# jdeschut/tunempc

Hardware: AMD Instinct MI355X
Metric: stage-Hessian convexifications/sec at (nx+nu)=32, p=64 (higher is better)
Workload: dtype f64

## Files before the change

### include/tunempc_hip.h

```cpp
#ifndef TUNEMPC_HIP_H
#define TUNEMPC_HIP_H

#include <stdint.h>

#ifdef __cplusplus
extern "C" {
#endif

#define TMPC_OK 0
#define TMPC_E_ARG (-1)
#define TMPC_E_UNSUPPORTED (-2)
#define TMPC_E_NOMEM (-3)
#define TMPC_E_HIP (-4)
#define TMPC_E_NODEVICE (-5)
#define TMPC_E_NOCONV (-6)

#define TMPC_STATUS_OPTIMAL 0
#define TMPC_STATUS_FEASIBLE 1
#define TMPC_STATUS_INFEASIBLE 2

#define TMPC_FLAG_NO_MFMA 1
#define TMPC_FLAG_PROFILE 2
#define TMPC_FLAG_FAST_EXIT 4

#define TMPC_INFO_STRIDE 16

typedef struct tmpc_handle tmpc_handle;

int tmpc_device_count(void);

uint64_t tmpc_workspace_bytes(int chunk, int p, int nx, int mb);

int tmpc_create(tmpc_handle** out, int chunk, int p, int nx, int mb);
#define TMPC_MAX_ROWS 31
#define TMPC_ARROW_LD 32
uint64_t tmpc_workspace_bytes_eq(int chunk, int p, int nx, int mb, int ng);
int tmpc_create_eq(tmpc_handle** out, int chunk, int p, int nx, int mb, int ng);
uint64_t tmpc_workspace_bytes_con(int chunk, int p, int nx, int mb, int ng, int nc);
int tmpc_create_con(tmpc_handle** out, int chunk, int p, int nx, int mb, int ng, int nc);
int tmpc_destroy(tmpc_handle* h);
int tmpc_get_chunk(tmpc_handle* h);

int tmpc_set_options(tmpc_handle* h, double tol, double center_tol, int max_iter, int center_iter, int flags);

#define TMPC_TUNE_CHORD_STEP 1
#define TMPC_TUNE_SMALL_BLOCKS 2
#define TMPC_TUNE_EIG_PRETEST 3
#define TMPC_TUNE_FUSE_FWD 4
#define TMPC_TUNE_GRAPH 5
#define TMPC_TUNE_PERSISTENT 7
#define TMPC_TUNE_LOWP_SWITCH 8
#define TMPC_LOWP_SWITCH_DEFAULT 1e-5
#define TMPC_TUNE_LOWP_TRSM 9
int tmpc_set_tuning(tmpc_handle* h, int key, double value);
int tmpc_create_ex(tmpc_handle** out, int chunk, int p, int nx, int mb, int ng, int nc, int step3, int lanes);

int tmpc_set_tight(tmpc_handle* h, int enable, double tight_tol);

int tmpc_convexify_batch_host(tmpc_handle* h, int nb, const double* A, const double* B, const double* H,
                              double* Hc, double* dHc, double* P, double* alpha, double* beta, double* kappa,
                              int32_t* status, int32_t* iters, double* info);
int tmpc_convexify_batch_device(tmpc_handle* h, int nb, const double* dA, const double* dB, const double* dH,
                                double* dHc_out, double* ddHc_out, double* dP_out, double* d_alpha, double* d_beta,
                                double* d_kappa, int32_t* d_status, int32_t* d_iters, double* d_info, void* stream);

int tmpc_convexify_eq_batch_host(tmpc_handle* h, int nb, const double* A, const double* B, const double* H, const double* G,
                                 double* Hc, double* dHc, double* P, double* Fg, double* alpha, double* beta, double* kappa,
                                 int32_t* status, int32_t* iters, double* info);

int tmpc_convexify_step2_batch_host(tmpc_handle* h, int nb, const double* A, const double* B, const double* H, const double* J,
                                    const int32_t* ncnt, double rho, double* Hc, double* dHc, double* P, double* FgF, double* alpha,
                                    double* beta, double* kappa, int32_t* status, int32_t* iters, double* info);

uint64_t tmpc_workspace_bytes_step3(int chunk, int p, int nx, int mb);
int tmpc_create_step3(tmpc_handle** out, int chunk, int p, int nx, int mb);
int tmpc_convexify_step3_batch_host(tmpc_handle* h, int nb, const double* A, const double* B, const double* H, double rho,
                                    double* Hc, double* dHc, double* P, double* T, double* alpha, double* beta, double* kappa,
                                    int32_t* status, int32_t* iters, double* info);

uint64_t tmpc_workspace_bytes_step3_con(int chunk, int p, int nx, int mb, int ng, int nc);
int tmpc_create_step3_con(tmpc_handle** out, int chunk, int p, int nx, int mb, int ng, int nc);
int tmpc_convexify_step3_con_batch_host(tmpc_handle* h, int nb, const double* A, const double* B, const double* H, const double* J,
                                        const int32_t* ncnt, double rho, double* Hc, double* dHc, double* P, double* FgF, double* T,
                                        double* alpha, double* beta, double* kappa, int32_t* status, int32_t* iters, double* info);
int tmpc_convexify_step3_batch_device(tmpc_handle* h, int nb, const double* dA, const double* dB, const double* dH, double rho, double* Hc, double* dHc,
                                      double* P, double* T, double* alpha, double* beta, double* kappa, int32_t* status, int32_t* iters, double* info, void* stream);
int tmpc_convexify_step3_con_batch_device(tmpc_handle* h, int nb, const double* dA, const double* dB, const double* dH, const double* dJ, const int32_t* d_ncnt,
                                          double rho, double* Hc, double* dHc, double* P, double* FgF, double* T, double* alpha, double* beta, double* kappa,
                                          int32_t* status, int32_t* iters, double* info, void* stream);

int tmpc_convexify_con_batch_device(tmpc_handle* h, int nb, const double* dA, const double* dB, const double* dH, const double* dJ,
                                    const int32_t* d_ncnt, double rho, double* dHc_out, double* ddHc_out, double* dP_out, double* dFgF,
                                    double* d_alpha, double* d_beta, double* d_kappa, int32_t* d_status, int32_t* d_iters,
                                    double* d_info, void* stream);

int tmpc_supplement_batch_host(tmpc_handle* h, int nb, const double* A, const double* B, const double* P, double* dHc);
int tmpc_supplement_terms_batch_host(tmpc_handle* h, int nb, const double* A, const double* B, const double* P, int nr,
                                     const double* J, const double* wts, const double* T, double* dHc);

int tmpc_pack_sensitivities_host(tmpc_handle* h, int nb, int nh, const double* C, const double* mu, const double* Hbig, double thr, int ncmax,
                                 double* C_As, int32_t* ncnt, int32_t* idx, double* q, double* Hst);

int tmpc_tracking_reference_host(tmpc_handle* h, int nstage, const double* Hc, const double* q, const double* wref,
                                 double ts, double* W, double* yref, int32_t* info);

int tmpc_eig_scan_host(tmpc_handle* h, int nb, const double* H, double* out);

int tmpc_eig_clip_host(int nb, int n, const double* A, double tol, double* out, double* evals, double* reg, int32_t* sweeps);

#define TMPC_LQR_NMAX 64
int tmpc_periodic_lqr_batch_host(int nb, int p, int nx, int mb, const double* A, const double* B, const double* H, const double* Pi0, double tol,
                                 int max_sweeps, double* K, double* Pi, double* Phi, double* info);
int tmpc_periodic_lqr_batch_device(int nb, int p, int nx, int mb, const double* A, const double* B, const double* H, const double* Pi0, double tol,
                                   int max_sweeps, double* K, double* Pi, double* Phi, double* info);

int tmpc_periodic_lqr_rows_batch_host(int nb, int p, int nx, int mb, int nr, int ng, const double* A, const double* B, const double* H, const double* J,
                                      const int32_t* ncnt, const double* Pi0, double tol, int max_sweeps, double* K, double* Pi, double* Phi, double* Lam,
                                      double* info);
int tmpc_periodic_lqr_rows_batch_device(int nb, int p, int nx, int mb, int nr, int ng, const double* A, const double* B, const double* H, const double* J,
                                        const int32_t* ncnt, const double* Pi0, double tol, int max_sweeps, double* K, double* Pi, double* Phi, double* Lam,
                                        double* info);

#define TMPC_LQR_CTG_INFO 12
int tmpc_periodic_lqr_ctg_batch_host(int nb, int p, int nx, int mb, int nr, int ng, const double* A, const double* B, const double* H, const double* J,
                                     const int32_t* ncnt, const double* Pi0, double tol, double rank_tol, int max_sweeps, double* K, double* Pi, double* Phi,
                                     double* Hn, int32_t* cnt, double* info);
int tmpc_periodic_lqr_ctg_batch_device(int nb, int p, int nx, int mb, int nr, int ng, const double* A, const double* B, const double* H, const double* J,
                                       const int32_t* ncnt, const double* Pi0, double tol, double rank_tol, int max_sweeps, double* K, double* Pi, double* Phi,
                                       double* Hn, int32_t* cnt, double* info);

int tmpc_horizon_lqr_batch_host(int nb, int p, int nx, int mb, int nr, int ng, int N, int nph, const int32_t* phases, int terminal, const double* A,
                                const double* B, const double* H, const double* J, const int32_t* ncnt, const double* Pf, double rank_tol, double* K0,
                                double* Pi0, double* Hn0, int32_t* cnt0, double* Kall, int32_t* cntall, double* info);
int tmpc_horizon_lqr_batch_device(int nb, int p, int nx, int mb, int nr, int ng, int N, int nph, const int32_t* phases, int terminal, const double* A,
                                  const double* B, const double* H, const double* J, const int32_t* ncnt, const double* Pf, double rank_tol, double* K0,
                                  double* Pi0, double* Hn0, int32_t* cnt0, double* Kall, int32_t* cntall, double* info);
// ... 67 lines not shown
```

### include/tunempc_hip_debug.h

```cpp
#ifndef TUNEMPC_HIP_DEBUG_H
#define TUNEMPC_HIP_DEBUG_H

#include "tunempc_hip.h"

#ifdef __cplusplus
extern "C" {
#endif

#define TMPC_DEBUG_FLAG_STOP_ASSEMBLED 8
#define TMPC_DEBUG_FLAG_NO_LIFT 16
#define TMPC_DEBUG_FLAG_NO_DMA 32
#define TMPC_DEBUG_FLAG_GENERIC_STAGE 64

int tmpc_debug_gemm_nt(tmpc_handle* h, double* C, const double* A, const double* B, int M, int N, int K, int mode, int lower);

int tmpc_debug_block_solve(tmpc_handle* h, int p, int d, const double* D, const double* Ccpl, const double* rhs, double* x, int32_t* nshift);

#define TMPC_DEBUG_FACTOR_PASS1 1
#define TMPC_DEBUG_FACTOR_FUSE_FWD1 2
#define TMPC_DEBUG_FACTOR_LOWP_TRSM 4
#define TMPC_DEBUG_FACTOR_DD 8
typedef struct {
  const double *D, *Ccpl, *Dlo, *Clo, *rhs;
  const int32_t *list, *lowp;
  double *oD, *oO, *oF, *oDdiag, *oX;
  float* oO32;
  double *oDl, *oOl, *oFl, *oXl;
  int32_t *nshift, *dims, *orient;
} tmpc_debug_factor_io;
int tmpc_debug_block_factor(tmpc_handle* h, int nb, int p, int d, int count, int mode, const tmpc_debug_factor_io* io);

int tmpc_debug_cr_schedule(int p, int32_t* out, int cap);

int tmpc_debug_get_multipliers(tmpc_handle* h, int nb, int nr, double* phi, double* z, double* dphi, double* dz);

int tmpc_debug_get_array(tmpc_handle* h, int which, uint64_t offset, uint64_t count, double* out);

int tmpc_debug_min_eig(tmpc_handle* h, int nmat, int n, const double* W, double* out);
int tmpc_debug_min_eig_lane(tmpc_handle* h, int nmat, int n, const double* W, double* out);

int tmpc_debug_factor_bench(tmpc_handle* h, int nb, int p, int d, int reps, double* ms_out2);

#ifdef __cplusplus
}
#endif
#endif
```

### tunempc_amd/_lib.py

```python
import ctypes as C
import os

import numpy as np

_HERE = os.path.dirname(os.path.abspath(__file__))
_LIB = None

INFO_STRIDE = 16
FLAG_NO_MFMA = 1
FLAG_PROFILE = 2
FLAG_FAST_EXIT = 4
STATUS_NAMES = {0: 'Optimal', 1: 'Feasible', 2: 'Infeasible'}

ARROW_LD = 32
EXPORTS = [
    'tmpc_device_count', 'tmpc_workspace_bytes', 'tmpc_workspace_bytes_eq', 'tmpc_workspace_bytes_con',
    'tmpc_create', 'tmpc_create_eq', 'tmpc_create_con', 'tmpc_destroy', 'tmpc_get_chunk', 'tmpc_set_options', 'tmpc_set_tight', 'tmpc_set_tuning', 'tmpc_create_ex',
    'tmpc_convexify_batch_host', 'tmpc_convexify_batch_device', 'tmpc_convexify_eq_batch_host', 'tmpc_convexify_step2_batch_host',
    'tmpc_convexify_con_batch_device', 'tmpc_workspace_bytes_step3', 'tmpc_create_step3', 'tmpc_convexify_step3_batch_host', 'tmpc_workspace_bytes_step3_con', 'tmpc_create_step3_con', 'tmpc_convexify_step3_con_batch_host', 'tmpc_convexify_step3_batch_device', 'tmpc_convexify_step3_con_batch_device', 'tmpc_supplement_batch_host', 'tmpc_supplement_terms_batch_host',
    'tmpc_tracking_reference_host', 'tmpc_eig_scan_host', 'tmpc_get_profile', 'tmpc_get_trace', 'tmpc_get_dual_host', 'tmpc_get_dual_con_host', 'tmpc_pack_sensitivities_host', 'tmpc_eig_clip_host',
    'tmpc_periodic_lqr_batch_host', 'tmpc_periodic_lqr_batch_device', 'tmpc_periodic_lqr_rows_batch_host', 'tmpc_periodic_lqr_rows_batch_device',
    'tmpc_periodic_lqr_ctg_batch_host', 'tmpc_periodic_lqr_ctg_batch_device', 'tmpc_horizon_lqr_batch_host', 'tmpc_horizon_lqr_batch_device',
    'tmpc_closed_loop_batch_host', 'tmpc_closed_loop_batch_device', 'tmpc_mpc_qp_batch_host', 'tmpc_mpc_qp_batch_device',
    'tmpc_mpc_qp_soft_batch_host', 'tmpc_mpc_qp_soft_batch_device', 'tmpc_mpc_qp_eq_batch_host', 'tmpc_mpc_qp_eq_batch_device',
    'tmpc_mpc_qp_aff_batch_host', 'tmpc_mpc_qp_aff_batch_device',
    'tmpc_last_error', 'tmpc_version',
]
DEBUG_EXPORTS = [
    'tmpc_debug_gemm_nt', 'tmpc_debug_block_solve', 'tmpc_debug_cr_schedule', 'tmpc_debug_get_multipliers', 'tmpc_debug_get_array',
    'tmpc_debug_min_eig', 'tmpc_debug_min_eig_lane', 'tmpc_debug_factor_bench', 'tmpc_debug_block_factor',
]
FLAG_DEBUG_NO_DMA = 32
FACTOR_PASS1, FACTOR_FUSE_FWD1, FACTOR_LOWP_TRSM, FACTOR_DD = 1, 2, 4, 8


class _FactorIO(C.Structure):
    _fields_ = ([(n, C.POINTER(C.c_double)) for n in ('D', 'Ccpl', 'Dlo', 'Clo', 'rhs')] + [(n, C.POINTER(C.c_int32)) for n in ('list', 'lowp')] +
                [(n, C.POINTER(C.c_double)) for n in ('oD', 'oO', 'oF', 'oDdiag', 'oX')] + [('oO32', C.POINTER(C.c_float))] +
                [(n, C.POINTER(C.c_double)) for n in ('oDl', 'oOl', 'oFl', 'oXl')] + [(n, C.POINTER(C.c_int32)) for n in ('nshift', 'dims', 'orient')])


def library_path():
    return os.environ.get('TMPC_LIB') or os.path.join(_HERE, 'lib', 'libtunempc_hip.so')


def load_library():
    global _LIB
    if _LIB is not None:
        return _LIB
    path = library_path()
    if not os.path.exists(path):
        raise RuntimeError(
            f"tunempc_amd: HIP library not built ({path}); run `python -c 'import __graft_entry__ as g; g.build()'`"
            " -- there is no CPU fallback for the convexify hot path")
    lib = C.CDLL(path)
    dp = C.POINTER(C.c_double)
    ip = C.POINTER(C.c_int32)
    vp = C.c_void_p
    lib.tmpc_device_count.restype = C.c_int
    lib.tmpc_workspace_bytes.restype = C.c_uint64
    lib.tmpc_workspace_bytes.argtypes = [C.c_int] * 4
    lib.tmpc_workspace_bytes_eq.restype = C.c_uint64
    lib.tmpc_workspace_bytes_eq.argtypes = [C.c_int] * 5
    lib.tmpc_create_eq.restype = C.c_int
    lib.tmpc_create_eq.argtypes = [C.POINTER(vp), C.c_int, C.c_int, C.c_int, C.c_int, C.c_int]
    lib.tmpc_convexify_eq_batch_host.restype = C.c_int
    lib.tmpc_convexify_eq_batch_host.argtypes = [vp, C.c_int, dp, dp, dp, dp, dp, dp, dp, dp, dp, dp, dp, ip, ip, dp]
    lib.tmpc_workspace_bytes_con.restype = C.c_uint64
    lib.tmpc_workspace_bytes_con.argtypes = [C.c_int] * 6
    lib.tmpc_create_con.restype = C.c_int
    lib.tmpc_create_con.argtypes = [C.POINTER(vp), C.c_int, C.c_int, C.c_int, C.c_int, C.c_int, C.c_int]
    lib.tmpc_convexify_step2_batch_host.restype = C.c_int
    lib.tmpc_convexify_step2_batch_host.argtypes = [vp, C.c_int, dp, dp, dp, dp, ip, C.c_double, dp, dp, dp, dp, dp, dp, dp, ip, ip, dp]
    lib.tmpc_workspace_bytes_step3.restype = C.c_uint64
    lib.tmpc_workspace_bytes_step3.argtypes = [C.c_int] * 4
    lib.tmpc_create_step3.restype = C.c_int
    lib.tmpc_create_step3.argtypes = [C.POINTER(vp), C.c_int, C.c_int, C.c_int, C.c_int]
    lib.tmpc_workspace_bytes_step3_con.restype = C.c_uint64
    lib.tmpc_workspace_bytes_step3_con.argtypes = [C.c_int] * 6
    lib.tmpc_create_step3_con.restype = C.c_int
    lib.tmpc_create_step3_con.argtypes = [C.POINTER(vp), C.c_int, C.c_int, C.c_int, C.c_int, C.c_int, C.c_int]
    lib.tmpc_convexify_step3_con_batch_host.restype = C.c_int
    lib.tmpc_convexify_step3_con_batch_host.argtypes = [vp, C.c_int, dp, dp, dp, dp, ip, C.c_double, dp, dp, dp, dp, dp, dp, dp, dp, ip, ip, dp]
    lib.tmpc_convexify_step3_batch_host.restype = C.c_int
    lib.tmpc_convexify_step3_batch_host.argtypes = [vp, C.c_int, dp, dp, dp, C.c_double, dp, dp, dp, dp, dp, dp, dp, ip, ip, dp]
    lib.tmpc_debug_get_multipliers.restype = C.c_int
    lib.tmpc_debug_get_multipliers.argtypes = [vp, C.c_int, C.c_int, dp, dp, dp, dp]
    lib.tmpc_debug_get_array.restype = C.c_int
    lib.tmpc_debug_get_array.argtypes = [vp, C.c_int, C.c_uint64, C.c_uint64, dp]
    lib.tmpc_convexify_con_batch_device.restype = C.c_int
    lib.tmpc_convexify_con_batch_device.argtypes = [vp, C.c_int, vp, vp, vp, vp, vp, C.c_double] + [vp] * 10 + [vp]
    lib.tmpc_convexify_step3_batch_device.restype = C.c_int
    lib.tmpc_convexify_step3_batch_device.argtypes = [vp, C.c_int, vp, vp, vp, C.c_double] + [vp] * 10 + [vp]
    lib.tmpc_convexify_step3_con_batch_device.restype = C.c_int
    lib.tmpc_convexify_step3_con_batch_device.argtypes = [vp, C.c_int, vp, vp, vp, vp, vp, C.c_double] + [vp] * 11 + [vp]
    lib.tmpc_get_dual_con_host.restype = C.c_int
    lib.tmpc_get_dual_con_host.argtypes = [vp, C.c_int, dp, dp, dp, dp]
    lib.tmpc_create.restype = C.c_int
    lib.tmpc_create.argtypes = [C.POINTER(vp), C.c_int, C.c_int, C.c_int, C.c_int]
    lib.tmpc_destroy.restype = C.c_int
    lib.tmpc_destroy.argtypes = [vp]
    lib.tmpc_get_chunk.restype = C.c_int
    lib.tmpc_get_chunk.argtypes = [vp]
    lib.tmpc_set_tuning.restype = C.c_int
    lib.tmpc_set_tuning.argtypes = [vp, C.c_int, C.c_double]
    lib.tmpc_create_ex.restype = C.c_int
    lib.tmpc_create_ex.argtypes = [C.POINTER(C.c_void_p)] + [C.c_int] * 8
    lib.tmpc_set_tight.restype = C.c_int
    lib.tmpc_set_tight.argtypes = [vp, C.c_int, C.c_double]
    lib.tmpc_set_options.restype = C.c_int
    lib.tmpc_set_options.argtypes = [vp, C.c_double, C.c_double, C.c_int, C.c_int, C.c_int]
    lib.tmpc_convexify_batch_host.restype = C.c_int
    lib.tmpc_convexify_batch_host.argtypes = [vp, C.c_int, dp, dp, dp, dp, dp, dp, dp, dp, dp, ip, ip, dp]
    lib.tmpc_convexify_batch_device.restype = C.c_int
    lib.tmpc_convexify_batch_device.argtypes = [vp, C.c_int] + [vp] * 12 + [vp]
    lib.tmpc_supplement_batch_host.restype = C.c_int
    lib.tmpc_supplement_batch_host.argtypes = [vp, C.c_int, dp, dp, dp, dp]
    lib.tmpc_eig_scan_host.restype = C.c_int
    lib.tmpc_eig_scan_host.argtypes = [vp, C.c_int, dp, dp]
    lib.tmpc_eig_clip_host.restype = C.c_int
    lib.tmpc_eig_clip_host.argtypes = [C.c_int, C.c_int, dp, C.c_double, dp, dp, dp, C.POINTER(C.c_int32)]
    lib.tmpc_periodic_lqr_batch_host.restype = C.c_int
    lib.tmpc_periodic_lqr_batch_host.argtypes = [C.c_int] * 4 + [dp] * 4 + [C.c_double, C.c_int] + [dp] * 4
    lib.tmpc_periodic_lqr_batch_device.restype = C.c_int
    lib.tmpc_periodic_lqr_batch_device.argtypes = [C.c_int] * 4 + [vp] * 4 + [C.c_double, C.c_int] + [vp] * 4
    lib.tmpc_periodic_lqr_rows_batch_host.restype = C.c_int
    lib.tmpc_periodic_lqr_rows_batch_host.argtypes = [C.c_int] * 6 + [dp] * 4 + [ip, dp, C.c_double, C.c_int] + [dp] * 5
    lib.tmpc_periodic_lqr_rows_batch_device.restype = C.c_int
    lib.tmpc_periodic_lqr_rows_batch_device.argtypes = [C.c_int] * 6 + [vp] * 6 + [C.c_double, C.c_int] + [vp] * 5
    lib.tmpc_periodic_lqr_ctg_batch_host.restype = C.c_int
    lib.tmpc_periodic_lqr_ctg_batch_host.argtypes = [C.c_int] * 6 + [dp] * 4 + [ip, dp, C.c_double, C.c_double, C.c_int] + [dp] * 4 + [ip, dp]
    lib.tmpc_periodic_lqr_ctg_batch_device.restype = C.c_int
    lib.tmpc_periodic_lqr_ctg_batch_device.argtypes = [C.c_int] * 6 + [vp] * 6 + [C.c_double, C.c_double, C.c_int] + [vp] * 6
    lib.tmpc_horizon_lqr_batch_host.restype = C.c_int
    lib.tmpc_horizon_lqr_batch_host.argtypes = [C.c_int] * 8 + [ip, C.c_int] + [dp] * 4 + [ip, dp, C.c_double] + [dp] * 3 + [ip, dp, ip, dp]
    lib.tmpc_horizon_lqr_batch_device.restype = C.c_int
    lib.tmpc_horizon_lqr_batch_device.argtypes = [C.c_int] * 8 + [ip, C.c_int] + [vp] * 6 + [C.c_double] + [vp] * 7
    lib.tmpc_closed_loop_batch_host.restype = C.c_int
    lib.tmpc_closed_loop_batch_host.argtypes = [C.c_int] * 9 + [dp] * 7 + [ip] + [dp] * 10
    lib.tmpc_closed_loop_batch_device.restype = C.c_int
    lib.tmpc_closed_loop_batch_device.argtypes = [C.c_int] * 9 + [vp] * 18
    lib.tmpc_mpc_qp_batch_host.restype = C.c_int
    lib.tmpc_mpc_qp_batch_host.argtypes = [C.c_int] * 9 + [dp] * 6 + [ip, dp, dp, C.c_double, C.c_int] + [dp] * 5 + [ip, ip] + [dp] * 4
    lib.tmpc_mpc_qp_batch_device.restype = C.c_int
    lib.tmpc_mpc_qp_batch_device.argtypes = [C.c_int] * 9 + [vp] * 9 + [C.c_double, C.c_int] + [vp] * 11
    lib.tmpc_mpc_qp_soft_batch_host.restype = C.c_int
    lib.tmpc_mpc_qp_soft_batch_host.argtypes = lib.tmpc_mpc_qp_batch_host.argtypes + [dp, dp, ip]
    lib.tmpc_mpc_qp_soft_batch_device.restype = C.c_int
    lib.tmpc_mpc_qp_soft_batch_device.argtypes = lib.tmpc_mpc_qp_batch_device.argtypes + [vp] * 3
    lib.tmpc_mpc_qp_eq_batch_host.restype = C.c_int
    lib.tmpc_mpc_qp_eq_batch_host.argtypes = lib.tmpc_mpc_qp_soft_batch_host.argtypes + [C.c_int, dp, dp, ip, C.c_int, dp, dp, dp, dp]
    lib.tmpc_mpc_qp_eq_batch_device.restype = C.c_int
    lib.tmpc_mpc_qp_eq_batch_device.argtypes = lib.tmpc_mpc_qp_soft_batch_device.argtypes + [C.c_int, vp, vp, vp, C.c_int, vp, vp, vp, vp]
    lib.tmpc_mpc_qp_aff_batch_host.restype = C.c_int
    lib.tmpc_mpc_qp_aff_batch_host.argtypes = lib.tmpc_mpc_qp_eq_batch_host.argtypes + [dp] * 7
    lib.tmpc_mpc_qp_aff_batch_device.restype = C.c_int
    lib.tmpc_mpc_qp_aff_batch_device.argtypes = lib.tmpc_mpc_qp_eq_batch_device.argtypes + [vp] * 7
    lib.tmpc_get_profile.restype = C.c_int
    lib.tmpc_get_profile.argtypes = [vp, dp]
    lib.tmpc_get_trace.restype = C.c_int
    lib.tmpc_get_trace.argtypes = [vp, C.c_int, dp]
    lib.tmpc_pack_sensitivities_host.restype = C.c_int
    lib.tmpc_pack_sensitivities_host.argtypes = [vp, C.c_int, C.c_int, dp, dp, dp, C.c_double, C.c_int, dp, ip, ip, dp, dp]
    lib.tmpc_get_dual_host.restype = C.c_int
    lib.tmpc_get_dual_host.argtypes = [vp, C.c_int, dp, dp, dp]
    lib.tmpc_debug_gemm_nt.restype = C.c_int
    lib.tmpc_debug_gemm_nt.argtypes = [vp, dp, dp, dp, C.c_int, C.c_int, C.c_int, C.c_int, C.c_int]
    lib.tmpc_debug_block_solve.restype = C.c_int
    lib.tmpc_debug_block_solve.argtypes = [vp, C.c_int, C.c_int, dp, dp, dp, dp, ip]
    lib.tmpc_supplement_terms_batch_host.restype = C.c_int
    lib.tmpc_supplement_terms_batch_host.argtypes = [vp, C.c_int, dp, dp, dp, C.c_int, dp, dp, dp, dp]
    lib.tmpc_tracking_reference_host.restype = C.c_int
    lib.tmpc_tracking_reference_host.argtypes = [vp, C.c_int, dp, dp, dp, C.c_double, dp, dp, ip]
    lib.tmpc_debug_cr_schedule.restype = C.c_int
    lib.tmpc_debug_cr_schedule.argtypes = [C.c_int, ip, C.c_int]
    lib.tmpc_debug_block_factor.restype = C.c_int
    lib.tmpc_debug_block_factor.argtypes = [vp, C.c_int, C.c_int, C.c_int, C.c_int, C.c_int, C.POINTER(_FactorIO)]
    lib.tmpc_debug_factor_bench.restype = C.c_int
    lib.tmpc_debug_factor_bench.argtypes = [vp, C.c_int, C.c_int, C.c_int, C.c_int, dp]
    lib.tmpc_debug_min_eig.restype = C.c_int
    lib.tmpc_debug_min_eig.argtypes = [vp, C.c_int, C.c_int, dp, dp]
    lib.tmpc_debug_min_eig_lane.restype = C.c_int
    lib.tmpc_debug_min_eig_lane.argtypes = [vp, C.c_int, C.c_int, dp, dp]
    lib.tmpc_last_error.restype = C.c_char_p
    lib.tmpc_version.restype = C.c_char_p
    _LIB = lib
    return lib


def _dptr(a):
    return a.ctypes.data_as(C.POINTER(C.c_double)) if a is not None else None


def _iptr(a):
    return a.ctypes.data_as(C.POINTER(C.c_int32)) if a is not None else None


class EigNotConverged(RuntimeError):
    """tmpc_eig_clip_host returned TMPC_E_NOCONV: the Jacobi sweeps were exhausted; `.partial` holds the last iterate."""


E_NOCONV = -6
E_UNSUPPORTED = -2
LQR_INFO_STRIDE = 8
LQR_CTG_INFO_STRIDE = 12
CLOSED_LOOP_INFO_STRIDE = 4
MPC_QP_INFO_STRIDE = 8


def _check(lib, rc, what):
    if rc != 0:
        raise RuntimeError(f"tunempc_amd: {what} failed with code {rc}: {lib.tmpc_last_error().decode()}")


class HipConvexifier:

    def __init__(self, p, nx, mb, chunk=0, tol=None, center_tol=None, max_iter=None, center_iter=None, flags=0, ng=0, nc=0, step3=False, lanes=0):
        self.lib = load_library()
        if self.lib.tmpc_device_count() < 1:
            raise RuntimeError("tunempc_amd: no HIP device visible; the convexify hot path has no CPU fallback")
        self.p, self.nx, self.mb, self.n = int(p), int(nx), int(mb), int(nx) + int(mb)
        self._h = C.c_void_p()
        self.ng = int(ng)
        self.nc = int(nc)
        self.step3 = bool(step3)
        if lanes:
            _check(self.lib, self.lib.tmpc_create_ex(C.byref(self._h), int(chunk), self.p, self.nx, self.mb, self.ng, self.nc, int(self.step3), int(lanes)), 'tmpc_create_ex')
        elif self.step3 and (self.ng or self.nc):
            _check(self.lib, self.lib.tmpc_create_step3_con(C.byref(self._h), int(chunk), self.p, self.nx, self.mb, self.ng, self.nc), 'tmpc_create_step3_con')
        elif self.step3:
            _check(self.lib, self.lib.tmpc_create_step3(C.byref(self._h), int(chunk), self.p, self.nx, self.mb), 'tmpc_create_step3')
        else:
            _check(self.lib, self.lib.tmpc_create_con(C.byref(self._h), int(chunk), self.p, self.nx, self.mb, self.ng, self.nc), 'tmpc_create_con')
        self.chunk = int(self.lib.tmpc_get_chunk(self._h))
        self.flags = int(flags)
        self.set_options(tol, center_tol, max_iter, center_iter, flags)

    def set_options(self, tol=None, center_tol=None, max_iter=None, center_iter=None, flags=None):
        if flags is not None:
            self.flags = int(flags)
        _check(self.lib, self.lib.tmpc_set_options(self._h, float(tol or 0.0), float(center_tol or 0.0),
                                                   int(max_iter or 0), int(center_iter or 0), self.flags), 'tmpc_set_options')

    def set_tuning(self, chord_step=None, small_blocks=None, eig_pretest=None, fuse_fwd=None, graph=None, persistent=None, lowp_switch=None, lowp_trsm=None):
        for key, v in ((1, chord_step), (2, small_blocks), (3, eig_pretest), (4, fuse_fwd), (5, graph), (7, persistent), (8, lowp_switch), (9, lowp_trsm)):
            if v is not None:
                _check(self.lib, self.lib.tmpc_set_tuning(self._h, key, float(v)), 'tmpc_set_tuning')

    def set_tight(self, enable=True, tight_tol=None):
        _check(self.lib, self.lib.tmpc_set_tight(self._h, 1 if enable else 0, float(tight_tol or 0.0)), 'tmpc_set_tight')

    def close(self):
        if getattr(self, '_h', None) is not None and self._h.value:
            self.lib.tmpc_destroy(self._h)
            self._h = C.c_void_p()

    def __del__(self):
        try:
            self.close()
        except Exception:
            pass

    def convexify_batch(self, A, B, H):
        A = np.ascontiguousarray(A, dtype=np.float64); B = np.ascontiguousarray(B, dtype=np.float64)
        H = np.ascontiguousarray(H, dtype=np.float64)
        nb = A.shape[0]
        assert A.shape == (nb, self.p, self.nx, self.nx), A.shape
        assert B.shape == (nb, self.p, self.nx, self.mb), B.shape
        assert H.shape == (nb, self.p, self.n, self.n), H.shape
        out = dict(Hc=np.empty_like(H), dHc=np.empty_like(H), P=np.empty_like(A), alpha=np.empty(nb), beta=np.empty(nb),
                   kappa=np.empty(nb), status=np.empty(nb, np.int32), iters=np.empty(nb, np.int32),
                   info=np.empty((nb, INFO_STRIDE)))
        if nb == 0:
            return out
        rc = self.lib.tmpc_convexify_batch_host(self._h, nb, _dptr(A), _dptr(B), _dptr(H), _dptr(out['Hc']), _dptr(out['dHc']),
                                                _dptr(out['P']), _dptr(out['alpha']), _dptr(out['beta']), _dptr(out['kappa']),
                                                _iptr(out['status']), _iptr(out['iters']), _dptr(out['info']))
        _check(self.lib, rc, 'tmpc_convexify_batch_host')
        return out

    def convexify_eq_batch(self, A, B, H, G):
        A = np.ascontiguousarray(A, dtype=np.float64); B = np.ascontiguousarray(B, dtype=np.float64)
        H = np.ascontiguousarray(H, dtype=np.float64); G = np.ascontiguousarray(G, dtype=np.float64)
        nb = A.shape[0]
        assert A.shape == (nb, self.p, self.nx, self.nx), A.shape
        assert B.shape == (nb, self.p, self.nx, self.mb), B.shape
        assert H.shape == (nb, self.p, self.n, self.n), H.shape
        assert self.ng > 0 and G.shape == (nb, self.p, self.ng, self.n), (G.shape, self.ng)
        out = dict(Hc=np.empty_like(H), dHc=np.empty_like(H), P=np.empty_like(A), Fg=np.empty((nb, self.p, self.ng)),
                   alpha=np.empty(nb), beta=np.empty(nb), kappa=np.empty(nb), status=np.empty(nb, np.int32),
                   iters=np.empty(nb, np.int32), info=np.empty((nb, INFO_STRIDE)))
        if nb == 0:
            return out
        rc = self.lib.tmpc_convexify_eq_batch_host(self._h, nb, _dptr(A), _dptr(B), _dptr(H), _dptr(G), _dptr(out['Hc']),
                                                   _dptr(out['dHc']), _dptr(out['P']), _dptr(out['Fg']), _dptr(out['alpha']),
                                                   _dptr(out['beta']), _dptr(out['kappa']), _iptr(out['status']),
                                                   _iptr(out['iters']), _dptr(out['info']))
        _check(self.lib, rc, 'tmpc_convexify_eq_batch_host')
        return out

    def debug_array(self, which, offset, count):
        out = np.empty(int(count))
        _check(self.lib, self.lib.tmpc_debug_get_array(self._h, int(which), int(offset), int(count), _dptr(out)), 'tmpc_debug_get_array')
        return out

    def debug_multipliers(self, nb, nr):
        out = [np.empty((nb, self.p, nr)) for _ in range(4)]
        _check(self.lib, self.lib.tmpc_debug_get_multipliers(self._h, nb, nr, *[_dptr(o) for o in out]), 'tmpc_debug_get_multipliers')
        return dict(phi=out[0], z=out[1], dphi=out[2], dz=out[3])

    def convexify_step2_batch(self, A, B, H, J, ncnt, rho):
        A = np.ascontiguousarray(A, dtype=np.float64); B = np.ascontiguousarray(B, dtype=np.float64)
        H = np.ascontiguousarray(H, dtype=np.float64); J = np.ascontiguousarray(J, dtype=np.float64)
        ncnt = np.ascontiguousarray(ncnt, dtype=np.int32)
        nb = A.shape[0]
        nr = self.ng + self.nc
        assert A.shape == (nb, self.p, self.nx, self.nx), A.shape
        assert B.shape == (nb, self.p, self.nx, self.mb), B.shape
        assert H.shape == (nb, self.p, self.n, self.n), H.shape
        assert self.nc > 0 and J.shape == (nb, self.p, nr, self.n) and ncnt.shape == (nb, self.p), (J.shape, ncnt.shape, nr)
        out = dict(Hc=np.empty_like(H), dHc=np.empty_like(H), P=np.empty_like(A), FgF=np.empty((nb, self.p, nr)),
                   alpha=np.empty(nb), beta=np.empty(nb), kappa=np.empty(nb), status=np.empty(nb, np.int32),
                   iters=np.empty(nb, np.int32), info=np.empty((nb, INFO_STRIDE)))
        if nb == 0:
            return out
        rc = self.lib.tmpc_convexify_step2_batch_host(self._h, nb, _dptr(A), _dptr(B), _dptr(H), _dptr(J), _iptr(ncnt), float(rho),
                                                      _dptr(out['Hc']), _dptr(out['dHc']), _dptr(out['P']), _dptr(out['FgF']),
                                                      _dptr(out['alpha']), _dptr(out['beta']), _dptr(out['kappa']),
# ... 141 lines not shown

    def profile(self):
        out = np.zeros(16)
        _check(self.lib, self.lib.tmpc_get_profile(self._h, _dptr(out)), 'tmpc_get_profile')
        keys = ['pre_ms', 'schur_ms', 'factor_ms', 'pass1_ms', 'pass2_ms', 'factor_launches', 'total_ms', 'ipm_iters',
                'problem_factorisations', 'potrf_ms', 'trsm_ms', 'update_ms', 'lanes', 'lowp_factorisations', 'update_f32_ms', 'persistent_problems']
        return dict(zip(keys, out.tolist()))

    def pack_sensitivities(self, C=None, mu=None, Hbig=None, thr=1e-15, ncmax=None, nb=None):
        out = {}
        p, n = self.p, self.n
        if C is not None:
            C = np.ascontiguousarray(C, dtype=np.float64); mu = np.ascontiguousarray(mu, dtype=np.float64)
            nb, nh = C.shape[0], C.shape[2]
            assert C.shape == (nb, p, nh, n) and mu.shape == (nb, p, nh), (C.shape, mu.shape)
            ncmax = int(ncmax or nh)
            out.update(C_As=np.empty((nb, p, ncmax, n)), nc=np.empty((nb, p), np.int32), idx=np.empty((nb, p, nh), np.int32))
        else:
            nh, ncmax = 0, 0
            nb = int(nb if nb is not None else Hbig.shape[0])
        out['q'] = np.empty((nb, p, n))
        if Hbig is not None:
            Hbig = np.ascontiguousarray(Hbig, dtype=np.float64)
            assert Hbig.shape == (nb, p * n, p * n), Hbig.shape
            out['H'] = np.empty((nb, p, n, n))
        _check(self.lib, self.lib.tmpc_pack_sensitivities_host(self._h, nb, nh, _dptr(C), _dptr(mu), _dptr(Hbig), float(thr), ncmax,
                                                               _dptr(out.get('C_As')), _iptr(out.get('nc')), _iptr(out.get('idx')),
                                                               _dptr(out['q']), _dptr(out.get('H'))), 'tmpc_pack_sensitivities_host')
        if 'nc' in out and (out['nc'] > ncmax).any():
            raise ValueError('pack_sensitivities: a stage has %d active rows, more than ncmax = %d' % (int(out['nc'].max()), ncmax))
        return out

    def dual(self, nb):
        X1 = np.empty((nb, self.p, self.n, self.n)); X2 = np.empty_like(X1); sc = np.empty((nb, 4))
        _check(self.lib, self.lib.tmpc_get_dual_host(self._h, int(nb), _dptr(X1), _dptr(X2), _dptr(sc)), 'tmpc_get_dual_host')
        return dict(X1=X1, X2=X2, x0=sc[:, 0].copy(), tau=sc[:, 1].copy(), alpha=sc[:, 2].copy(), mu_target=sc[:, 3].copy())

    def dual_con(self, nb, arrows=False):
        nr = self.ng + self.nc
        phi = np.zeros((nb, self.p, nr)); z = np.zeros_like(phi)
        aX = np.zeros((nb, self.p, 2, ARROW_LD, ARROW_LD)) if arrows else None; at = np.zeros((nb, self.p, 2)) if arrows else None
        _check(self.lib, self.lib.tmpc_get_dual_con_host(self._h, int(nb), _dptr(phi), _dptr(z), _dptr(aX) if arrows else None, _dptr(at) if arrows else None), 'tmpc_get_dual_con_host')
        out = dict(phi=phi, z=z)
        if arrows:
            out.update(aX=aX, at=at)
        return out

    def trace(self, nb):
        out = np.zeros((nb, 80, 10))
        _check(self.lib, self.lib.tmpc_get_trace(self._h, nb, _dptr(out)), 'tmpc_get_trace')
        return out

    def debug_gemm_nt(self, Cm, A, B, mode=0, lower=False):
        Cm = np.ascontiguousarray(Cm, dtype=np.float64).copy(); A = np.ascontiguousarray(A, dtype=np.float64)
        B = np.ascontiguousarray(B, dtype=np.float64)
        M, N = Cm.shape; K = A.shape[1]
        _check(self.lib, self.lib.tmpc_debug_gemm_nt(self._h, _dptr(Cm), _dptr(A), _dptr(B), M, N, K, int(mode), int(lower)), 'tmpc_debug_gemm_nt')
        return Cm

    def debug_min_eig(self, W, lane=False):
        W = np.ascontiguousarray(W, dtype=np.float64)
        nmat, n, _ = W.shape
        out = np.empty(nmat)
        fn = self.lib.tmpc_debug_min_eig_lane if lane else self.lib.tmpc_debug_min_eig
        _check(self.lib, fn(self._h, nmat, n, _dptr(W), _dptr(out)), 'tmpc_debug_min_eig')
        return out

    def tracking_reference(self, Hc, q, wref, ts):
        Hc = np.ascontiguousarray(Hc, dtype=np.float64); q = np.ascontiguousarray(q, dtype=np.float64)
        wref = np.ascontiguousarray(wref, dtype=np.float64)
        n = self.nx + self.mb
        if Hc.shape[-2:] != (n, n) or q.shape != Hc.shape[:-1] or wref.shape != q.shape:
            raise ValueError('tracking_reference: expected Hc [..., %d, %d] and q, wref [..., %d]' % (n, n, n))
        ns = int(np.prod(Hc.shape[:-2], dtype=np.int64))
        W = np.empty_like(Hc); yref = np.empty_like(q); info = np.zeros(Hc.shape[:-2], dtype=np.int32)
        _check(self.lib, self.lib.tmpc_tracking_reference_host(self._h, ns, _dptr(Hc), _dptr(q), _dptr(wref), float(ts), _dptr(W), _dptr(yref),
                                                              info.ctypes.data_as(C.POINTER(C.c_int32))), 'tmpc_tracking_reference_host')
        return W, yref, info

    def debug_factor_bench(self, nb, p, d, reps=3):
        out = np.zeros(2)
        _check(self.lib, self.lib.tmpc_debug_factor_bench(self._h, nb, p, d, reps, _dptr(out)), 'tmpc_debug_factor_bench')
        return out

    def debug_block_solve(self, D, Ccpl, rhs):
        D = np.ascontiguousarray(D, dtype=np.float64); Ccpl = np.ascontiguousarray(Ccpl, dtype=np.float64)
        rhs = np.ascontiguousarray(rhs, dtype=np.float64)
        p, d, _ = D.shape
        x = np.empty((p, d)); ns = np.zeros(1, np.int32)
        _check(self.lib, self.lib.tmpc_debug_block_solve(self._h, p, d, _dptr(D), _dptr(Ccpl), _dptr(rhs), _dptr(x), _iptr(ns)), 'tmpc_debug_block_solve')
        return x, int(ns[0])

    def debug_block_factor(self, D, Ccpl, rhs, plist=None, lowp=None, pass1=False, fuse_fwd1=False, lowp_trsm=False, dd=False, Dlo=None, Clo=None):
        f64 = lambda a: None if a is None else np.ascontiguousarray(a, dtype=np.float64)
        D, Ccpl, rhs, Dlo, Clo = f64(D), f64(Ccpl), f64(rhs), f64(Dlo), f64(Clo)
        nb, p, d, _ = D.shape
        nc = 3 if pass1 else 1
        if Ccpl.shape != D.shape or rhs.shape != ((nb, p, d, 3) if pass1 else (nb, p, d)):
            raise ValueError('debug_block_factor: D, Ccpl [nb, p, d, d] and rhs [nb, p, d] (pass 2) / [nb, p, d, 3] (pass 1) expected')
        plist = np.ascontiguousarray(np.arange(nb) if plist is None else plist, dtype=np.int32)
        lowp = None if lowp is None else np.ascontiguousarray(lowp, dtype=np.int32)
        if lowp is not None and lowp.shape != (nb,):
            raise ValueError('debug_block_factor: lowp [nb] expected')
        mode = (FACTOR_PASS1 if pass1 else 0) | (FACTOR_FUSE_FWD1 if fuse_fwd1 else 0) | (FACTOR_LOWP_TRSM if lowp_trsm else 0) | (FACTOR_DD if dd else 0)
        dp = (d + 15) // 16 * 16; ld32 = (dp + 31) // 32 * 32
        has32 = bool(lowp_trsm or (lowp is not None and lowp.any()))
        raw = dict(D=np.empty((nb, p, dp, dp)), O=np.empty((nb, p, dp, dp)), F=np.empty((nb, p, dp, dp)), Ddiag=np.empty((nb, p, dp)), X=np.empty((nb, p, dp, nc)),
                   O32=np.empty((nb, 2 * p, dp, ld32), np.float32) if has32 else None)
        if dd:
            raw.update(Dl=np.empty((nb, p, dp, dp)), Ol=np.empty((nb, p, dp, dp)), Fl=np.empty((nb, p, dp, dp)), Xl=np.empty((nb, p, dp, nc)))
        nshift = np.zeros(nb, np.int32); dims = np.zeros(4, np.int32); orient = np.zeros(p, np.int32)
        io = _FactorIO(D=_dptr(D), Ccpl=_dptr(Ccpl), Dlo=_dptr(Dlo), Clo=_dptr(Clo), rhs=_dptr(rhs), list=_iptr(plist), lowp=_iptr(lowp),
                       oD=_dptr(raw['D']), oO=_dptr(raw['O']), oF=_dptr(raw['F']), oDdiag=_dptr(raw['Ddiag']), oX=_dptr(raw['X']),
                       oO32=raw['O32'].ctypes.data_as(C.POINTER(C.c_float)) if has32 else None,
                       oDl=_dptr(raw.get('Dl')), oOl=_dptr(raw.get('Ol')), oFl=_dptr(raw.get('Fl')), oXl=_dptr(raw.get('Xl')),
                       nshift=_iptr(nshift), dims=_iptr(dims), orient=_iptr(orient))
        _check(self.lib, self.lib.tmpc_debug_block_factor(self._h, nb, p, d, len(plist), mode, C.byref(io)), 'tmpc_debug_block_factor')
        assert (int(dims[0]), int(dims[1]), int(dims[2]), bool(dims[3])) == (dp, ld32, nc, has32), dims
        raw.update(dp=dp, ld32=ld32)
        cut = lambda a: None if a is None else a[:, :, :d, :d].copy()
        vec = lambda a: None if a is None else (a[:, :, :d, :].copy() if pass1 else a[:, :, :d, 0].copy())
        out = dict(raw=raw, orient=orient, nshift=nshift, D=cut(raw['D']), L=np.tril(cut(raw['D'])), O=cut(raw['O']), F=cut(raw['F']), O32=cut(raw['O32']),
                   Ddiag=raw['Ddiag'][:, :, :d].copy(), x=vec(raw['X']))
        if dd:
            out.update(Dl=cut(raw['Dl']), Ll=np.tril(cut(raw['Dl'])), Ol=cut(raw['Ol']), Fl=cut(raw['Fl']), xl=vec(raw['Xl']))
        return out


def eig_clip(A, tol):
    lib = load_library()
    A = np.ascontiguousarray(A, dtype=np.float64)
    single = A.ndim == 2
    A3 = A[None] if single else A
    nb, n, n2 = A3.shape
    if n != n2:
        raise ValueError('square matrices expected')
    out = np.empty_like(A3); ev = np.empty((nb, n)); reg = np.empty(nb); sw = np.zeros(nb, dtype=np.int32)
    rc = lib.tmpc_eig_clip_host(nb, n, _dptr(A3), float(tol), _dptr(out), _dptr(ev), _dptr(reg), _iptr(sw))
    if rc == E_NOCONV:
        err = EigNotConverged(f"tunempc_amd: tmpc_eig_clip_host did not converge: {lib.tmpc_last_error().decode()}")
        err.partial = dict(out=out, evals=ev, reg=reg, sweeps=sw)
        raise err
    _check(lib, rc, 'tmpc_eig_clip_host')
    if single:
        return dict(out=out[0], evals=ev[0], reg=float(reg[0]), sweeps=int(sw[0]))
    return dict(out=out, evals=ev, reg=reg, sweeps=sw)


def _check_lqr(lib, rc, what):
    if rc == E_UNSUPPORTED:
        raise NotImplementedError(lib.tmpc_last_error().decode())
    _check(lib, rc, what)


def periodic_lqr_batch_host(A, B, H, Pi0, tol, max_sweeps):
    lib = load_library()
    nb, p, nx, mb = B.shape
    K = np.empty((nb, p, mb, nx)); Pi = np.empty((nb, p, nx, nx)); Phi = np.empty((nb, nx, nx)); info = np.zeros((nb, LQR_INFO_STRIDE))
    rc = lib.tmpc_periodic_lqr_batch_host(nb, p, nx, mb, _dptr(A), _dptr(B), _dptr(H), _dptr(Pi0), float(tol), int(max_sweeps),
                                          _dptr(K), _dptr(Pi), _dptr(Phi), _dptr(info))
    _check_lqr(lib, rc, 'tmpc_periodic_lqr_batch_host')
    return K, Pi, Phi, info


def periodic_lqr_batch_device(A, B, H, Pi0, tol, max_sweeps):
    import torch
# ... 335 lines not shown
```

### tunempc_amd/csrc/tmpc_api.hip

```cpp
#include <hip/hip_runtime.h>
#include <stdio.h>
#include <stdlib.h>
#include <new>
#include <string.h>
#include <algorithm>
#include <chrono>
#include <thread>
#include <mutex>
#include <condition_variable>
#include <functional>
#include <unistd.h>
#include <vector>

#include <string>
#include <unordered_map>

#include "../../include/tunempc_hip.h"
#include "../../include/tunempc_hip_debug.h"
#include "tmpc_common.h"
#include "tmpc_small.h"
#include "tmpc_stage.h"
#include "tmpc_schur.h"
#include "tmpc_factor.h"
#include "tmpc_cr.h"
// ... 27 lines not shown
struct DevBuf {
  void* p = nullptr;
  ~DevBuf() { if (p) hipFree(p); }
  hipError_t alloc(size_t bytes) { return hipMalloc(&p, bytes ? bytes : 8); }
  template <typename T> T* as() const { return (T*)p; }
};

constexpr int MAXL = 4;
struct LaneWorker {
  std::thread th;
  std::mutex m;
  std::condition_variable cv;
  std::function<void()> job;
  bool has_job = false, done = true, stop = false;
  pid_t pid = 0;
  void start() {
    pid = getpid();
    th = std::thread([this] {
      std::unique_lock<std::mutex> lk(m);
      for (;;) {
        cv.wait(lk, [&] { return has_job || stop; });
        if (stop) return;
        std::function<void()> j = std::move(job);
        has_job = false;
        lk.unlock();
        j();
        lk.lock();
        done = true;
        cv.notify_all();
      }
    });
  }
  void submit(std::function<void()> j) {
    { std::lock_guard<std::mutex> lk(m); job = std::move(j); has_job = true; done = false; }
    cv.notify_all();
  }
  void wait() { std::unique_lock<std::mutex> lk(m); cv.wait(lk, [&] { return done; }); }
  void shutdown() {
    { std::lock_guard<std::mutex> lk(m); stop = true; }
    cv.notify_all();
    if (th.joinable()) th.join();
  }
  static void retire(LaneWorker*& wk) {
    if (!wk) return;
    if (wk->pid == getpid()) { wk->shutdown(); delete wk; }
    wk = nullptr;
  }
};

struct Lane {
  LaneWorker* worker;
  WS ws;
  double *dA, *dB, *dH;
  double* dG;
  int32_t* dncnt;
  double* d_info;
  double* d_abk;
  void* big_scr;
  int32_t* d_si;
  hipStream_t st;
  hipEvent_t ev[8];
  double prof[16];
  std::vector<hipEvent_t> kev;
  int last_nb;
  int o32_dp;
  std::unordered_map<std::string, hipGraphExec_t>* graphs;
  char err[512];
};

struct tmpc_handle {
  Dims dm;
  int chunk;
  int nlanes;
  Opts opt;
  int flags;
  Lane lane[MAXL];
  void* slab;
  size_t slab_bytes;
  hipEvent_t ev_in;
  int device;
  CrSched sched;
  int* d_sched;
  int rs, mt;
  int tune_small, tune_pretest, tune_fuse, tune_graph, tune_persist, tune_lowp_trsm;
  void* dd_slab;
  size_t dd_bytes;
  int tight;
  double tight_tol;
};

static int cr_upload(const CrSched& sc, int** out) {
  std::vector<int> flat(sc.elim);
  flat.insert(flat.end(), sc.upd.begin(), sc.upd.end());
  flat.insert(flat.end(), sc.orient.begin(), sc.orient.end());
  *out = nullptr;
  if (hipMalloc(out, flat.size() * sizeof(int)) != hipSuccess) return TMPC_E_NOMEM;
  if (hipMemcpy(*out, flat.data(), flat.size() * sizeof(int), hipMemcpyHostToDevice) != hipSuccess) { hipFree(*out); *out = nullptr; return TMPC_E_HIP; }
  return TMPC_OK;
}
static CrDev cr_dev(const CrSched& sc, const int* d_sched, const int* alist) {
  CrDev c; c.elim = d_sched; c.upd = d_sched + sc.elim.size(); c.orient = d_sched + sc.elim.size() + sc.upd.size(); c.alist = alist;
  return c;
}

static bool dims_ok(int p, int nx, int mb) { return p >= 1 && nx >= 1 && mb >= 0 && nx + mb <= NB && nx + mb >= 1; }

static Dims make_dims(int chunk, int p, int nx, int mb, int ng = 0, int nc = 0, int step3 = 0) {
  Dims d;
  d.ng = ng; d.nr = ng + nc; d.constr = 0;
  d.nT = step3 ? (nx + mb) * (nx + mb + 1) / 2 : 0;
  d.nz = d.nr + (nc > 0 ? 2 : 0);
  d.B = chunk; d.p = p; d.nx = nx; d.mb = mb; d.n = nx + mb;
  d.d = nx * (nx + 1) / 2;
  d.dp = (d.d + d.nz + (d.nT ? d.nT + 1 : 0) + 15) / 16 * 16;
  d.nt = (d.dp + TB - 1) / TB;
  d.flags = 0;
  return d;
}

static bool schur_in_lds(const Dims& dm) { return (size_t)sch_rec<0>() * dm.nx * dm.nx * sizeof(double) + (size_t)dm.d * sizeof(unsigned) + 64 <= 158 * 1024; }
struct Carver {
  char* base; size_t off;
  template <typename T> T* take(size_t count) {
    off = (off + 255) & ~(size_t)255;
    T* p = base ? (T*)(base + off) : nullptr;
    off += count * sizeof(T);
    return p;
  }
};

static size_t carve(WS& w, const Dims& dm, char* base, Lane* h) {
  Carver c{base, 0};
  const size_t BP = (size_t)dm.B * dm.p, nn = (size_t)dm.n * dm.n, nxx = (size_t)dm.nx * dm.nx;
  const size_t bs = (size_t)dm.dp * dm.dp;
  w.Hb = c.take<double>(BP * nn); w.V = c.take<double>(BP * dm.nx * dm.n);
  w.P = c.take<double>(BP * nxx);
  w.X1 = c.take<double>(BP * nn); w.X2 = c.take<double>(BP * nn); w.S1 = c.take<double>(BP * nn); w.S2 = c.take<double>(BP * nn);
  w.S1i = c.take<double>(BP * nn); w.S2i = c.take<double>(BP * nn); w.L1i = c.take<double>(BP * nn); w.L2i = c.take<double>(BP * nn);
  w.LX1i = c.take<double>(BP * nn); w.LX2i = c.take<double>(BP * nn);
  w.Rd1 = c.take<double>(BP * nn); w.Rd2 = c.take<double>(BP * nn); w.T1 = c.take<double>(BP * nn); w.T2 = c.take<double>(BP * nn);
  w.dS1 = c.take<double>(BP * nn); w.dS2 = c.take<double>(BP * nn); w.dX1 = c.take<double>(BP * nn); w.dX2 = c.take<double>(BP * nn);
  w.c1 = c.take<double>(BP * nn); w.c2 = c.take<double>(BP * nn);
  w.dP = c.take<double>(BP * nxx);
  w.Wm = c.take<double>(BP * 4 * nn); w.eigmin = c.take<double>(BP * 4);
  w.KF = c.take<double>(BP * 12 * nxx); w.adjV = c.take<double>(BP * NADJ * nxx); w.adjE = c.take<double>(BP * NADJ * nxx);
  w.part = c.take<double>(BP * NPART); w.prob = c.take<double>((size_t)dm.B * PS); w.iprob = c.take<int>((size_t)dm.B * IS);
  w.D = c.take<double>(BP * bs); w.O = c.take<double>(BP * bs); w.F = c.take<double>(BP * bs);
  w.O32 = (dm.nT == 0 && dm.n <= NMAX && dm.dp > 64 && dm.nt <= TRR_NT) ? c.take<float>(2 * BP * (size_t)dm.dp * ((dm.dp + 31) & ~31)) : nullptr;
  w.Linv = c.take<double>(BP * dm.nt * TB * TB); w.Ddiag = c.take<double>(BP * dm.dp);
  w.W3 = c.take<double>(BP * dm.dp * 3); w.U = c.take<double>(BP * dm.dp * 2); w.TU = c.take<double>(BP * dm.dp * 2);
  w.Z = c.take<double>(BP * dm.dp);
  w.active = c.take<int>(64);
  w.alist = c.take<int>((size_t)dm.B);
  w.flist = c.take<int>((size_t)dm.B);
  w.cr_orient = nullptr;
  w.trace = c.take<double>((size_t)dm.B * TRACE_LEN * TRACE_W);
  w.Hc = c.take<double>(BP * nn); w.dHc = c.take<double>(BP * nn); w.Pout = c.take<double>(BP * nxx);
  w.bscr = (dm.n > NMAX) ? c.take<double>(BP * BIG_SCR * nn) : nullptr;
  w.sscr = schur_in_lds(dm) ? nullptr : c.take<double>(BP * 10 * nxx);
  w.Dl = w.Ol = w.Fl = w.Linvl = w.KFl = w.adjVl = w.adjEl = w.W3l = w.Zl = w.Pprev = w.Pdef = w.phidef = w.Zdd = w.TUl = w.atdef = w.ddscr = nullptr; w.plist = w.pnext = nullptr;
  w.G = nullptr; w.ncnt = nullptr; w.rho = 0.0;
  w.phi = w.zph = w.dphi = w.dzph = w.corrp = w.pvec = w.psm = w.prs = w.Fg = nullptr;
  w.at = w.adt = w.aX = w.adX = w.acor = w.aSi = w.aLi = w.aLXi = w.asum = nullptr;
  if (dm.nr > 0) {
    const size_t g = dm.nr, z = dm.nz;
    w.phi = c.take<double>(BP * g); w.zph = c.take<double>(BP * g); w.dphi = c.take<double>(BP * g); w.dzph = c.take<double>(BP * g);
    w.corrp = c.take<double>(BP * g); w.Fg = c.take<double>(BP * g);
// ... 208 lines not shown
  const double* A0 = A + (size_t)m0 * K; const double* B0 = B + (size_t)n0 * K;
  if (k1 > 0 && k1 < K && 2 * k1 == K)
    wg_tile_dma<UPD_DMA_DEPTH>(C + (size_t)m0 * N + n0, N, A0, B0, A0 + k1, B0 + k1, K, Mt, Nt, k1, mode, (lower && tm == tn) ? 0 : GM_NOTRI, blockIdx.x, lds);
  else
    wg_tile_dma<UPD_DMA_DEPTH>(C + (size_t)m0 * N + n0, N, A0, B0, nullptr, nullptr, K, Mt, Nt, K, mode, (lower && tm == tn) ? 0 : GM_NOTRI, blockIdx.x, lds);
}
static size_t slots_bytes(int s) { return (size_t)s * MS * sizeof(double); }
template <int PART> static size_t schur_lds(const Dims& dm) {
  if (!schur_in_lds(dm)) return (size_t)dm.d * sizeof(unsigned) + 64;
 return (size_t)sch_rec<PART>() * dm.nx * dm.nx * sizeof(double) + (size_t)dm.d * sizeof(unsigned) + 64; }
static size_t factor_lds() { return (size_t)FACT_LDS_DOUBLES * sizeof(double); }
static size_t solve_lds(const Dims& dm) { return (size_t)cr_solve_lds_doubles(dm.dp) * sizeof(double); }

static int set_lds_attrs(int device) {
  static bool done[64] = {false};
  if (device >= 0 && device < 64 && done[device]) return TMPC_OK;
  const int big = 160 * 1024;
  HIPCHK(hipFuncSetAttribute((const void*)k_stage_pre<256>, hipFuncAttributeMaxDynamicSharedMemorySize, big - 4096));
  HIPCHK(hipFuncSetAttribute((const void*)k_stage_rhs<256>, hipFuncAttributeMaxDynamicSharedMemorySize, big - 4096));
  HIPCHK(hipFuncSetAttribute((const void*)k_stage_dir<256>, hipFuncAttributeMaxDynamicSharedMemorySize, big - 4096));
  HIPCHK(hipFuncSetAttribute((const void*)k_final_stage, hipFuncAttributeMaxDynamicSharedMemorySize, big));
  HIPCHK(hipFuncSetAttribute((const void*)k_schur<0>, hipFuncAttributeMaxDynamicSharedMemorySize, big));
  HIPCHK(hipFuncSetAttribute((const void*)k_schur<1>, hipFuncAttributeMaxDynamicSharedMemorySize, big));
  HIPCHK(hipFuncSetAttribute((const void*)k_cr_potrf<true>, hipFuncAttributeMaxDynamicSharedMemorySize, big));
  HIPCHK(hipFuncSetAttribute((const void*)k_cr_potrf<false>, hipFuncAttributeMaxDynamicSharedMemorySize, big));
  HIPCHK(hipFuncSetAttribute((const void*)k_cr_trsm<true, 2>, hipFuncAttributeMaxDynamicSharedMemorySize, big));
  HIPCHK(hipFuncSetAttribute((const void*)k_cr_trsm<false, 2>, hipFuncAttributeMaxDynamicSharedMemorySize, big));
  HIPCHK(hipFuncSetAttribute((const void*)k_cr_trsm_dma, hipFuncAttributeMaxDynamicSharedMemorySize, big));
  HIPCHK(hipFuncSetAttribute((const void*)k_cr_trsm_dma_f32, hipFuncAttributeMaxDynamicSharedMemorySize, big));
  HIPCHK(hipFuncSetAttribute((const void*)k_cr_potrf_dma, hipFuncAttributeMaxDynamicSharedMemorySize, big));
  HIPCHK(hipFuncSetAttribute((const void*)k_cr_update<true, 2>, hipFuncAttributeMaxDynamicSharedMemorySize, big));
  HIPCHK(hipFuncSetAttribute((const void*)k_cr_update<false, 2>, hipFuncAttributeMaxDynamicSharedMemorySize, big));
  HIPCHK(hipFuncSetAttribute((const void*)k_cr_fwd_diag, hipFuncAttributeMaxDynamicSharedMemorySize, big));
  HIPCHK(hipFuncSetAttribute((const void*)k_cr_fwd_off, hipFuncAttributeMaxDynamicSharedMemorySize, big));
  HIPCHK(hipFuncSetAttribute((const void*)k_cr_bwd, hipFuncAttributeMaxDynamicSharedMemorySize, big));
  HIPCHK(hipFuncSetAttribute((const void*)k_cr_small_solve, hipFuncAttributeMaxDynamicSharedMemorySize, big));
  HIPCHK(hipFuncSetAttribute((const void*)k_cr_small_factor, hipFuncAttributeMaxDynamicSharedMemorySize, big));
  HIPCHK(hipFuncSetAttribute((const void*)k_ipm_small, hipFuncAttributeMaxDynamicSharedMemorySize, big));
  HIPCHK(hipFuncSetAttribute((const void*)k_debug_gemm<true>, hipFuncAttributeMaxDynamicSharedMemorySize, big));
  HIPCHK(hipFuncSetAttribute((const void*)k_debug_gemm<false>, hipFuncAttributeMaxDynamicSharedMemorySize, big));
  HIPCHK(hipFuncSetAttribute((const void*)k_supplement, hipFuncAttributeMaxDynamicSharedMemorySize, big));
  HIPCHK(hipFuncSetAttribute((const void*)k_phi_pre<false, false>, hipFuncAttributeMaxDynamicSharedMemorySize, big));
  HIPCHK(hipFuncSetAttribute((const void*)k_phi_pre<false, true>, hipFuncAttributeMaxDynamicSharedMemorySize, big));
  HIPCHK(hipFuncSetAttribute((const void*)k_phi_pre<true, false>, hipFuncAttributeMaxDynamicSharedMemorySize, big));
  HIPCHK(hipFuncSetAttribute((const void*)k_phi_pre<true, true>, hipFuncAttributeMaxDynamicSharedMemorySize, big));
  HIPCHK(hipFuncSetAttribute((const void*)k_phi_rhs<false>, hipFuncAttributeMaxDynamicSharedMemorySize, big));
  HIPCHK(hipFuncSetAttribute((const void*)k_phi_dir<false>, hipFuncAttributeMaxDynamicSharedMemorySize, big));
  HIPCHK(hipFuncSetAttribute((const void*)k_phi_rhs<true>, hipFuncAttributeMaxDynamicSharedMemorySize, big));
  HIPCHK(hipFuncSetAttribute((const void*)k_phi_dir<true>, hipFuncAttributeMaxDynamicSharedMemorySize, big));
  HIPCHK(hipFuncSetAttribute((const void*)k_t3_schur<false>, hipFuncAttributeMaxDynamicSharedMemorySize, big));
  HIPCHK(hipFuncSetAttribute((const void*)k_t3_schur<true>, hipFuncAttributeMaxDynamicSharedMemorySize, big));
  HIPCHK(hipFuncSetAttribute((const void*)k_dd_potrf, hipFuncAttributeMaxDynamicSharedMemorySize, big));
  HIPCHK(hipFuncSetAttribute((const void*)k_dd_aug_fill, hipFuncAttributeMaxDynamicSharedMemorySize, big));
  HIPCHK(hipFuncSetAttribute((const void*)k_dd_trsm, hipFuncAttributeMaxDynamicSharedMemorySize, big));
  HIPCHK(hipFuncSetAttribute((const void*)k_dd_update, hipFuncAttributeMaxDynamicSharedMemorySize, big));
  HIPCHK(hipFuncSetAttribute((const void*)k_dd_fwd_diag, hipFuncAttributeMaxDynamicSharedMemorySize, big));
  HIPCHK(hipFuncSetAttribute((const void*)k_dd_fwd_off, hipFuncAttributeMaxDynamicSharedMemorySize, big));
  HIPCHK(hipFuncSetAttribute((const void*)k_dd_bwd, hipFuncAttributeMaxDynamicSharedMemorySize, big));
  HIPCHK(hipFuncSetAttribute((const void*)k_dd_images, hipFuncAttributeMaxDynamicSharedMemorySize, big));
  HIPCHK(hipFuncSetAttribute((const void*)k_dd_schur<0>, hipFuncAttributeMaxDynamicSharedMemorySize, big));
  HIPCHK(hipFuncSetAttribute((const void*)k_dd_schur<1>, hipFuncAttributeMaxDynamicSharedMemorySize, big));
  HIPCHK(hipFuncSetAttribute((const void*)k_dd_schur<0, true>, hipFuncAttributeMaxDynamicSharedMemorySize, big));
  HIPCHK(hipFuncSetAttribute((const void*)k_dd_schur<1, true>, hipFuncAttributeMaxDynamicSharedMemorySize, big));
  HIPCHK(hipFuncSetAttribute((const void*)k_dd_polish_pre, hipFuncAttributeMaxDynamicSharedMemorySize, big - 4096));
  HIPCHK(hipFuncSetAttribute((const void*)k_polish_step, hipFuncAttributeMaxDynamicSharedMemorySize, big - 4096));
  if (device >= 0 && device < 64) done[device] = true;
  return TMPC_OK;
}

static unsigned cr_grid(long items) { return (unsigned)((items + 7) / 8 * 8); }
constexpr int DF_NO_SMALL = 2;
constexpr int DF_NO_DMA = 4;

static bool cr_small_levels(const Dims& dm, const CrSched& sc, CrLevs* out) {
  if ((dm.flags & DF_NO_SMALL) || dm.dp != 16 || (dm.flags & 1) || dm.p > CRS_PMAX || (int)sc.lev.size() > CRS_MAXLEV) return false;
  if (out) {
    out->n = (int)sc.lev.size();
    for (int l = 0; l < out->n; ++l) { out->v[4 * l] = sc.lev[l].eoff; out->v[4 * l + 1] = sc.lev[l].nelim; out->v[4 * l + 2] = sc.lev[l].uoff; out->v[4 * l + 3] = sc.lev[l].nupd; }
  }
  return true;
}

static void cr_factor(const WS& w, const Dims& dm, const CrSched& sc, const int* d_sched, const int* alist, int count, hipStream_t st,
                      int rs_opt, int mt_opt, std::vector<hipEvent_t>* kev = nullptr, int* nkev = nullptr, int fuse_fwd1 = 0, int nlowp = 0) {
  const CrDev cd = cr_dev(sc, d_sched, alist);
  int ke = 0;
  auto mark = [&](int cls) {
#ifdef TMPC_CYCLE_PROF
    { static int cls_ids[4] = {0, 1, 2, 3}; hipMemcpyToSymbolAsync(HIP_SYMBOL(tmpc::g_prof_cls), &cls_ids[cls + 1], sizeof(int), 0, hipMemcpyHostToDevice, st); }
#endif
    if (!kev) return;
    while ((int)kev->size() <= ke) { hipEvent_t e; if (hipEventCreate(&e) != hipSuccess) return; kev->push_back(e); }
    (void)cls;
    hipEventRecord((*kev)[ke++], st);
  };
  const bool mf = !(dm.flags & 1);
  if (sc.prep) hipLaunchKernelGGL(k_cr_prep, dim3(count), dim3(256), 0, st, w, dm, cd, sc.prep);
  {
    CrLevs lv;
    if (!fuse_fwd1 && cr_small_levels(dm, sc, &lv)) {
      mark(0);
      hipLaunchKernelGGL(k_cr_small_factor, dim3(count), dim3(CRS_NT), (size_t)crs_factor_lds_doubles() * sizeof(double), st, w, dm, cd, lv);
      mark(0);
      if (nkev) *nkev = ke;
      return;
    }
  }
  const int nt64 = (dm.dp + 63) / 64;
  for (const CrLevel& lv : sc.lev) {
    const bool use_dma = !(dm.flags & DF_NO_DMA), potrf_dma = use_dma;
    mark(0);
    if (mf && use_dma && potrf_dma && dm.nt <= TRR_NT)
      hipLaunchKernelGGL(k_cr_potrf_dma, dim3(cr_grid((long)count * lv.nelim)), dim3(256), (size_t)potrf_dma_lds_doubles() * sizeof(double), st, w, dm, cd, lv.eoff, lv.nelim, count);
    else if (mf) hipLaunchKernelGGL(k_cr_potrf<true>, dim3(cr_grid((long)count * lv.nelim)), dim3(256), factor_lds(), st, w, dm, cd, lv.eoff, lv.nelim, count);
    else hipLaunchKernelGGL(k_cr_potrf<false>, dim3(cr_grid((long)count * lv.nelim)), dim3(256), factor_lds(), st, w, dm, cd, lv.eoff, lv.nelim, count);
    mark(0);
    if (fuse_fwd1) hipLaunchKernelGGL(k_cr_fwd_diag, dim3(cr_grid((long)count * lv.nelim)), dim3(256), solve_lds(dm), st, w, dm, cd, lv.eoff, lv.nelim, count, 1);
    if (lv.nupd == 0) { mark(1); mark(1); mark(2); mark(2); mark(3); mark(3); continue; }
    const long work64 = (long)count * lv.nelim * 2 * nt64;
    const int rs = rs_opt > 0 ? rs_opt : (work64 >= 16384 ? 128 : 64);
    const int mt = mt_opt > 0 ? mt_opt : 64;
    const int nstrip = (dm.dp + rs - 1) / rs, nm = (dm.dp + mt - 1) / mt;
    const long it_trsm = (long)count * lv.nelim * 2 * nstrip;
    const long it_upd = (long)count * ((long)lv.nupd * (nm * (nm + 1) / 2) + (long)lv.nelim * nm * nm);
    mark(1);
    if (mf && use_dma && dm.nt <= TRR_NT) {
      const size_t trsm_lds = (size_t)trd_lds_doubles() * sizeof(double);
      const bool trsm32 = (dm.flags & DF_LOWP_TRSM) != 0;
      if (!trsm32 || nlowp < count)
        hipLaunchKernelGGL(k_cr_trsm_dma, dim3(cr_grid((long)count * lv.nelim * 2 * nt64)), dim3(256), trsm_lds, st, w, dm, cd, lv.eoff, lv.nelim, count);
      if (trsm32 && nlowp > 0)
        hipLaunchKernelGGL(k_cr_trsm_dma_f32, dim3(cr_grid((long)count * lv.nelim * 2 * nt64)), dim3(256), (size_t)trf_lds_doubles() * sizeof(double), st, w, dm, cd, lv.eoff, lv.nelim, count);
    }
    else if (mf) hipLaunchKernelGGL((k_cr_trsm<true, 2>), dim3(cr_grid(it_trsm)), dim3(256), factor_lds(), st, w, dm, cd, lv.eoff, lv.nelim, count, rs);
    else hipLaunchKernelGGL((k_cr_trsm<false, 2>), dim3(cr_grid(it_trsm)), dim3(256), factor_lds(), st, w, dm, cd, lv.eoff, lv.nelim, count, rs);
    mark(1); mark(2);
    if (mf && use_dma) {
      const int nm64 = (dm.dp + 63) / 64;
      const long it_dma = (long)count * ((long)lv.nupd * (nm64 * (nm64 + 1) / 2) + (long)lv.nelim * nm64 * nm64);
      if (nlowp < count)
        hipLaunchKernelGGL(k_cr_update_dma, dim3(cr_grid(it_dma)), dim3(256), (size_t)dma_lds_doubles<UPD_DMA_DEPTH>() * sizeof(double), st, w, dm, cd, lv.eoff, lv.nelim, lv.uoff, lv.nupd, count, fuse_fwd1);
      mark(2); mark(3);
      if (nlowp > 0)
        hipLaunchKernelGGL(k_cr_update_dma_f32, dim3(cr_grid(it_dma)), dim3(256), (size_t)UPD_DMA_DEPTH * DMA_SLAB * sizeof(double), st, w, dm, cd, lv.eoff, lv.nelim, lv.uoff, lv.nupd, count);
      mark(3);
    }
    else if (mf) { hipLaunchKernelGGL((k_cr_update<true, 2>), dim3(cr_grid(it_upd)), dim3(256), factor_lds(), st, w, dm, cd, lv.eoff, lv.nelim, lv.uoff, lv.nupd, count, mt); mark(2); mark(3); mark(3); }
    else { hipLaunchKernelGGL((k_cr_update<false, 2>), dim3(cr_grid(it_upd)), dim3(256), factor_lds(), st, w, dm, cd, lv.eoff, lv.nelim, lv.uoff, lv.nupd, count, mt); mark(2); mark(3); mark(3); }
    if (fuse_fwd1 && nlowp > 0 && mf && use_dma && lv.nupd)
      hipLaunchKernelGGL(k_cr_fwd_off, dim3(cr_grid((long)count * lv.nupd)), dim3(256), solve_lds(dm), st, w, dm, cd, lv.uoff, lv.nupd, count, 1, 1);
  }
  if (nkev) *nkev = ke;
}

static void cr_solve(const WS& w, const Dims& dm, const CrSched& sc, const int* d_sched, const int* alist, int count, hipStream_t st, int pass, bool skip_fwd = false) {
  const CrDev cd = cr_dev(sc, d_sched, alist);
  {
    CrLevs lv;
    if (!skip_fwd && cr_small_levels(dm, sc, &lv)) {
      hipLaunchKernelGGL(k_cr_small_solve, dim3(count), dim3(CRS_NT), (size_t)crs_solve_lds_doubles(dm.p) * sizeof(double), st, w, dm, cd, lv, pass);
      return;
    }
  }
  const size_t lds = solve_lds(dm);
  for (const CrLevel& lv : sc.lev) {
    if (skip_fwd) break;
    hipLaunchKernelGGL(k_cr_fwd_diag, dim3(cr_grid((long)count * lv.nelim)), dim3(256), lds, st, w, dm, cd, lv.eoff, lv.nelim, count, pass);
    if (lv.nupd) hipLaunchKernelGGL(k_cr_fwd_off, dim3(cr_grid((long)count * lv.nupd)), dim3(256), lds, st, w, dm, cd, lv.uoff, lv.nupd, count, pass, 0);
  }
  for (size_t l = sc.lev.size(); l-- > 0;) {
    const CrLevel& lv = sc.lev[l];
    hipLaunchKernelGGL(k_cr_bwd, dim3(cr_grid((long)count * lv.nelim)), dim3(256), lds, st, w, dm, cd, lv.eoff, lv.nelim, count, pass);
  }
}

static bool ddschur_in_lds(const Dims& dm) { return (size_t)2 * ddsch_mats<0>() * dm.nx * dm.nx * sizeof(double) + (size_t)dm.d * sizeof(unsigned) + 64 <= 158 * 1024; }
template <int PART> static size_t ddschur_lds(const Dims& dm) {
  if (!ddschur_in_lds(dm)) return (size_t)dm.d * sizeof(unsigned) + 64;
  return (size_t)2 * ddsch_mats<PART>() * dm.nx * dm.nx * sizeof(double) + (size_t)dm.d * sizeof(unsigned) + 64;
}
static void dd_schur_launch(const WS& w, const Dims& dm, int grid_stages, hipStream_t st) {
  if (ddschur_in_lds(dm)) {
    hipLaunchKernelGGL(k_dd_schur<0>, dim3(grid_stages), dim3(256), ddschur_lds<0>(dm), st, w, dm);
    hipLaunchKernelGGL(k_dd_schur<1>, dim3(grid_stages), dim3(256), ddschur_lds<1>(dm), st, w, dm);
  } else {
    hipLaunchKernelGGL((k_dd_schur<0, true>), dim3(grid_stages), dim3(256), ddschur_lds<0>(dm), st, w, dm);
    hipLaunchKernelGGL((k_dd_schur<1, true>), dim3(grid_stages), dim3(256), ddschur_lds<1>(dm), st, w, dm);
  }
}
static size_t dd_stage_lds(const Dims& dm, int slots) { return dm.n > NMAX ? 64 : slots_bytes(slots); }
static void dd_factor(const WS& w, const Dims& dm, const CrSched& sc, const int* d_sched, const int* alist, int count, hipStream_t st) {
  const CrDev cd = cr_dev(sc, d_sched, alist);
  const size_t lds = (size_t)DD_FACT_LDS * sizeof(double);
  if (sc.prep) hipLaunchKernelGGL(k_dd_prep, dim3(count), dim3(256), 0, st, w, dm, cd, sc.prep);
  const int nm = (dm.dp + 63) / 64;
  for (const CrLevel& lv : sc.lev) {
    hipLaunchKernelGGL(k_dd_potrf, dim3(cr_grid((long)count * lv.nelim)), dim3(256), lds, st, w, dm, cd, lv.eoff, lv.nelim, count);
    if (lv.nupd == 0) continue;
    hipLaunchKernelGGL(k_dd_trsm, dim3(cr_grid((long)count * lv.nelim * 2 * nm)), dim3(256), lds, st, w, dm, cd, lv.eoff, lv.nelim, count);
    const long items = (long)count * ((long)lv.nupd * (nm * (nm + 1) / 2) + (long)lv.nelim * nm * nm);
    hipLaunchKernelGGL(k_dd_update, dim3(cr_grid(items)), dim3(256), lds, st, w, dm, cd, lv.eoff, lv.nelim, lv.uoff, lv.nupd, count);
  }
}
static int dd_solve(const WS& w, const Dims& dm, const CrSched& sc, const int* d_sched, const int* alist, int count, hipStream_t st, int pass, int nb_all) {
  const CrDev cd = cr_dev(sc, d_sched, alist);
  const size_t lds = (size_t)dd_solve_lds_doubles(dm.dp) * sizeof(double);
  HIPCHK(hipMemsetAsync(w.W3l, 0, (size_t)nb_all * dm.p * dm.dp * 3 * sizeof(double), st));
  HIPCHK(hipMemsetAsync(w.Zl, 0, (size_t)nb_all * dm.p * dm.dp * sizeof(double), st));
  for (const CrLevel& lv : sc.lev) {
    hipLaunchKernelGGL(k_dd_fwd_diag, dim3(cr_grid((long)count * lv.nelim)), dim3(256), lds, st, w, dm, cd, lv.eoff, lv.nelim, count, pass);
    if (lv.nupd) hipLaunchKernelGGL(k_dd_fwd_off, dim3(cr_grid((long)count * lv.nupd)), dim3(256), lds, st, w, dm, cd, lv.uoff, lv.nupd, count, pass);
  }
  for (size_t l = sc.lev.size(); l-- > 0;) {
    const CrLevel& lv = sc.lev[l];
    hipLaunchKernelGGL(k_dd_bwd, dim3(cr_grid((long)count * lv.nelim)), dim3(256), lds, st, w, dm, cd, lv.eoff, lv.nelim, count, pass);
  }
  return TMPC_OK;
}

#define TMPC_STAGE_LAUNCH(K, LDSB, ST, ...)                                                          \
  do {                                                                                               \
    hipLaunchKernelGGL((K<256>), dim3(BP), dim3(256), LDSB, ST, __VA_ARGS__);                        \
  } while (0)

static int run_chunk(tmpc_handle* h, Lane* ln, int nb, const double* dA, const double* dB, const double* dH, hipStream_t st,
                     const double* dG = nullptr, const int32_t* dncnt = nullptr, double rho = 0.0, bool step3 = false) {
  Dims dm = h->dm;
  dm.B = nb;
  if (!step3) dm.nT = 0;
  if (!dG) { dm.ng = 0; dm.nr = 0; dm.nz = 0; }
  dm.constr = (dG && dncnt && rho > 0.0) ? 1 : 0;
  if (dG && !dncnt) { dm.nr = dm.ng; dm.nz = dm.ng; }
  if (dG && dncnt && !dm.constr) dm.nz = dm.nr;
  const bool eq = dm.nr > 0;
  const bool t3 = dm.nT > 0;
  dm.dp = (dm.d + (eq ? dm.nz : 0) + (t3 ? dm.nT + 1 : 0) + 15) / 16 * 16;
  dm.nt = (dm.dp + TB - 1) / TB;
  dm.flags = (h->flags & TMPC_FLAG_NO_MFMA) | (h->tune_small ? 0 : DF_NO_SMALL) | ((h->flags & TMPC_DEBUG_FLAG_NO_DMA) ? DF_NO_DMA : 0);
  const size_t t3_lds = (size_t)(3 * (dm.nT + 1) + 8) * sizeof(double);
  const bool big = dm.n > NMAX || (h->flags & TMPC_DEBUG_FLAG_GENERIC_STAGE);
  const size_t t3_schur_lds = (size_t)((big ? 0 : 9 * 32 * T3_LD) + 2 * (dm.nT + 1)) * sizeof(double) + (size_t)(2 * (dm.nT + 1) + 2 * (dm.d + 1)) * sizeof(short) + 64;
  if (big && !ln->ws.bscr) {
    if (hipMalloc(&ln->big_scr, (size_t)h->dm.B * dm.p * BIG_SCR * dm.n * dm.n * sizeof(double)) != hipSuccess) { snprintf(g_err, sizeof(g_err), "hipMalloc of the generic-stage scratch failed"); return TMPC_E_NOMEM; }
    ln->ws.bscr = (double*)ln->big_scr;
  }
  WS wall = ln->ws;
  wall.A = dA; wall.Bm = dB; wall.H = dH; wall.G = dG; wall.ncnt = dncnt; wall.rho = rho;
  wall.cr_orient = h->d_sched + h->sched.elim.size() + h->sched.upd.size();
  WS w = wall;
  w.A = nullptr; w.Bm = nullptr; w.H = nullptr;
  int* alist = wall.alist;
  int* flist = wall.flist;
  wall.alist = nullptr;
  Opts o = h->opt;
  o.tight = 0; o.tight_tol = 0.0;
  o.fast_exit = (h->flags & TMPC_FLAG_FAST_EXIT) ? 1 : 0;
  if ((h->flags & (TMPC_FLAG_NO_MFMA | TMPC_DEBUG_FLAG_NO_DMA)) || !w.O32 || t3 || dm.dp <= 64 || dm.nt > TRR_NT) o.lowp_switch = 0.0;
  if (o.lowp_switch > 0.0) o.lowp_switch = fmax(o.lowp_switch, 16.0 * o.tol);
  if (o.lowp_switch > 0.0) {
    dm.flags |= DF_LOWP | (h->tune_lowp_trsm ? DF_LOWP_TRSM : 0);
    if (ln->o32_dp != 0 && ln->o32_dp != dm.dp) HIPCHK(hipMemsetAsync(w.O32, 0, 2 * (size_t)h->dm.B * h->dm.p * h->dm.dp * ((h->dm.dp + 31) & ~31) * sizeof(float), st));
    ln->o32_dp = dm.dp;
  }
  WS wf = w; wf.alist = flist;
  const int BPall = nb * dm.p;
  const bool prof = (h->flags & TMPC_FLAG_PROFILE) != 0;
  bool use_graph = h->tune_graph && dm.dp <= 64 && !(h->flags & (TMPC_FLAG_PROFILE | TMPC_DEBUG_FLAG_STOP_ASSEMBLED)) && st == ln->st;
  const int reg_max = (h->flags & TMPC_DEBUG_FLAG_NO_LIFT) ? 0 : REG_MAX;
  HIPCHK(hipMemsetAsync(w.active, 0, 5 * sizeof(int), st));
  HIPCHK(hipMemsetAsync(w.trace, 0, (size_t)nb * TRACE_LEN * TRACE_W * sizeof(double), st));
  const size_t big_lds = (size_t)BIG_EIG_LDS * sizeof(double);
  if (big) hipLaunchKernelGGL(kb_init_stage, dim3(BPall), dim3(256), big_lds, st, wall, dm);
  else hipLaunchKernelGGL(k_init_stage, dim3(BPall), dim3(64), slots_bytes(2), st, wall, dm);
  {
    WS wi = wall; wi.alist = alist;
    hipLaunchKernelGGL(k_init_prob, dim3(nb), dim3(64), 0, st, wi, dm, o.lowp_switch);
  }
  hipLaunchKernelGGL(k_init_state, dim3(BPall), dim3(64), 0, st, wall, dm);
  if (eq) hipLaunchKernelGGL(k_phi_init, dim3(BPall), dim3(64), 0, st, wall, dm);
  if (t3) hipLaunchKernelGGL(k_t3_init, dim3(BPall), dim3(64), 0, st, wall, dm);
  int cnt[5] = {0, 0, 0, 0, 0};
  HIPCHK(hipMemcpyAsync(cnt, w.active, 5 * sizeof(int), hipMemcpyDeviceToHost, st));
  HIPCHK(hipStreamSynchronize(st));
  int active = cnt[0], nfac = cnt[0], nlowp = cnt[4];
  const int cap = o.max_iter + o.center_iter * (MUT_BACKOFF_MAX + 1) + 2;
  int it = 0;
  {
    CrLevs plv;
    const bool pays = h->tune_persist >= 2 || dm.p <= 8 || active * h->nlanes >= 96;
    const bool persist = h->tune_persist && pays && !eq && !t3 && !big && dm.dp == 16 && dm.n <= PK_NMAX && !h->tight && !prof &&
                         !(h->flags & TMPC_DEBUG_FLAG_STOP_ASSEMBLED) && cr_small_levels(dm, h->sched, &plv);
    if (persist && active > 0) {
      const CrDev cd = cr_dev(h->sched, h->d_sched, alist);
      hipLaunchKernelGGL(k_ipm_small, dim3(active), dim3(CRS_NT), (size_t)pk_lds_doubles(dm.p) * sizeof(double), st, w, dm, o, cd, plv, h->sched.prep, reg_max,
                         h->tune_pretest ? o.chord_step : -1.0, cap);
      HIPCHK(hipGetLastError());
      ln->prof[15] += (double)active;
      active = 0; nfac = 0;
    }
  }
  auto ipm_loop = [&](const Opts& o, bool ddm, int cap) -> int {
  while (active > 0 && it < cap) {
    const int BP = active * dm.p;
    hipGraphExec_t gexec = nullptr;
    std::string gkey;
    bool capturing = false;
    struct CaptureGuard {
      hipStream_t st; bool* on;
      ~CaptureGuard() { if (*on) { hipGraph_t g_ = nullptr; (void)hipStreamEndCapture(st, &g_); if (g_) hipGraphDestroy(g_); (void)hipGetLastError(); } }
    } capture_guard{st, &capturing};
    int nkev = 0;
    if (use_graph && !ddm) {
      gkey.assign((const char*)&w, sizeof(WS)); gkey.append((const char*)&dm, sizeof(Dims)); gkey.append((const char*)&o, sizeof(Opts));
      const int ks[6] = {active, nfac, nb, reg_max, (int)h->flags, h->tune_pretest | (h->tune_fuse << 1) | (h->tune_small << 2)};
      gkey.append((const char*)ks, sizeof(ks));
      if (!ln->graphs) ln->graphs = new std::unordered_map<std::string, hipGraphExec_t>();
      auto f = ln->graphs->find(gkey);
      if (f == ln->graphs->end()) {
        if (ln->graphs->size() >= 256) { for (auto& kv : *ln->graphs) if (kv.second) hipGraphExecDestroy(kv.second); ln->graphs->clear(); }
        (*ln->graphs)[gkey] = nullptr;
      } else if (f->second) gexec = f->second;
      else if (hipStreamBeginCapture(st, hipStreamCaptureModeThreadLocal) == hipSuccess) capturing = true;
    }
    if (!gexec) {
    if (prof) HIPCHK(hipEventRecord(ln->ev[0], st));
    if (big) hipLaunchKernelGGL(kb_stage_pre, dim3(BP), dim3(256), 0, st, w, dm);
    else TMPC_STAGE_LAUNCH(k_stage_pre, slots_bytes(PRE_SLOTS), st, w, dm);
    if (eq) {
      const bool bigr = dm.nr > NRS;
      if (big && bigr) hipLaunchKernelGGL((k_phi_pre<true, true>), dim3(BP), dim3(64), (size_t)phi_pre_lds(true, true) * sizeof(double), st, w, dm, 1);
      else if (big) hipLaunchKernelGGL((k_phi_pre<true, false>), dim3(BP), dim3(64), (size_t)phi_pre_lds(true, false) * sizeof(double), st, w, dm, 1);
      else if (bigr) hipLaunchKernelGGL((k_phi_pre<false, true>), dim3(BP), dim3(64), (size_t)phi_pre_lds(false, true) * sizeof(double), st, w, dm, 1);
      else hipLaunchKernelGGL((k_phi_pre<false, false>), dim3(BP), dim3(64), (size_t)phi_pre_lds(false, false) * sizeof(double), st, w, dm, 1);
    }
    if (t3) hipLaunchKernelGGL(k_t3_pre, dim3(BP), dim3(64), t3_lds, st, w, dm);
    hipLaunchKernelGGL(k_ctrl_a, dim3(active), dim3(64), 0, st, w, dm, o);
    if (prof) HIPCHK(hipEventRecord(ln->ev[1], st));
    if (ddm) {
      if (nfac > 0) {
        hipLaunchKernelGGL(k_dd_images, dim3(nfac * dm.p), dim3(256), dd_stage_lds(dm, DD_IMG_SLOTS), st, wf, dm);
        dd_schur_launch(wf, dm, nfac * dm.p, st);
      }
    } else if (nfac > 0) {
// ... 189 lines not shown
const char* tmpc_version(void) { return "tunempc_amd 0.2 (gfx950, fp64 MFMA, cyclic-reduction block factorisation)"; }

int tmpc_device_count(void) {
  int n = 0;
  if (hipGetDeviceCount(&n) != hipSuccess) return 0;
  return n;
}

static bool rows_ok(int nx, int ng, int nc) {
  (void)nx;
  return ng >= 0 && ng <= NGM && nc >= 0 && nc <= NCM;
}
static bool model_dims_ok(int nx, int mb, int ng, int nc, int step3) { return nx + mb <= NBM || (ng == 0 && nc == 0 && !step3); }
static_assert(AEL == TMPC_ARROW_LD, "tunempc_hip.h: leading dimension of the exported arrow blocks");
static_assert(LQR_NMAX == TMPC_LQR_NMAX, "tunempc_hip.h: largest stage block of the periodic LQR recursion");
static_assert(NGM == TMPC_MAX_ROWS && NCM == TMPC_MAX_ROWS, "tunempc_hip.h: row limits");
static uint64_t workspace_bytes(int chunk, int p, int nx, int mb, int ng, int nc, int step3) {
  if (chunk < 1 || !dims_ok(p, nx, mb) || !rows_ok(nx, ng, nc) || !model_dims_ok(nx, mb, ng, nc, step3)) return 0;
  WS w;
  Dims dm = make_dims(chunk, p, nx, mb, ng, nc, step3);
  if (solve_lds(dm) > 160 * 1024) return 0;
  return (uint64_t)carve(w, dm, nullptr, nullptr);
}
uint64_t tmpc_workspace_bytes_con(int chunk, int p, int nx, int mb, int ng, int nc) { return workspace_bytes(chunk, p, nx, mb, ng, nc, 0); }
uint64_t tmpc_workspace_bytes_step3(int chunk, int p, int nx, int mb) { return workspace_bytes(chunk, p, nx, mb, 0, 0, 1); }
uint64_t tmpc_workspace_bytes_step3_con(int chunk, int p, int nx, int mb, int ng, int nc) { return workspace_bytes(chunk, p, nx, mb, ng, nc, 1); }
uint64_t tmpc_workspace_bytes_eq(int chunk, int p, int nx, int mb, int ng) { return tmpc_workspace_bytes_con(chunk, p, nx, mb, ng, 0); }
uint64_t tmpc_workspace_bytes(int chunk, int p, int nx, int mb) { return tmpc_workspace_bytes_eq(chunk, p, nx, mb, 0); }

int tmpc_create(tmpc_handle** out, int chunk, int p, int nx, int mb) { return tmpc_create_eq(out, chunk, p, nx, mb, 0); }

int tmpc_create_eq(tmpc_handle** out, int chunk, int p, int nx, int mb, int ng) { return tmpc_create_con(out, chunk, p, nx, mb, ng, 0); }

static int create_handle(tmpc_handle** out, int chunk, int p, int nx, int mb, int ng, int nc, int step3, int lanes = 0);
int tmpc_create_con(tmpc_handle** out, int chunk, int p, int nx, int mb, int ng, int nc) { return create_handle(out, chunk, p, nx, mb, ng, nc, 0); }
int tmpc_create_step3(tmpc_handle** out, int chunk, int p, int nx, int mb) { return create_handle(out, chunk, p, nx, mb, 0, 0, 1); }
int tmpc_create_step3_con(tmpc_handle** out, int chunk, int p, int nx, int mb, int ng, int nc) { return create_handle(out, chunk, p, nx, mb, ng, nc, 1); }
int tmpc_create_ex(tmpc_handle** out, int chunk, int p, int nx, int mb, int ng, int nc, int step3, int lanes) {
  if (lanes < 0 || lanes > MAXL) { snprintf(g_err, sizeof(g_err), "tmpc_create_ex: lanes = %d outside 0..%d", lanes, MAXL); return TMPC_E_ARG; }
  return create_handle(out, chunk, p, nx, mb, ng, nc, step3 ? 1 : 0, lanes);
}

static int create_handle(tmpc_handle** out, int chunk, int p, int nx, int mb, int ng, int nc, int step3, int lanes) {
  if (!out) return TMPC_E_ARG;
  *out = nullptr;
  if (!dims_ok(p, nx, mb)) { snprintf(g_err, sizeof(g_err), "unsupported dims p=%d nx=%d mb=%d (need nx+mb<=%d)", p, nx, mb, NB); return TMPC_E_UNSUPPORTED; }
  if (!rows_ok(nx, ng, nc)) {
    snprintf(g_err, sizeof(g_err), "unsupported constraint rows ng=%d nc=%d (need 0<=ng<=%d, 0<=nc<=%d)", ng, nc, NGM, NCM);
    return TMPC_E_UNSUPPORTED;
  }
  if (!model_dims_ok(nx, mb, ng, nc, step3)) {
    snprintf(g_err, sizeof(g_err), "nx+mb = %d > %d is supported for the plain model only (no G / C rows, no Step 3)", nx + mb, NBM);
    return TMPC_E_UNSUPPORTED;
  }
  {
    const Dims db = make_dims(1, p, nx, mb, ng, nc, step3);
    if (solve_lds(db) > 160 * 1024) {
      snprintf(g_err, sizeof(g_err), "nx=%d ng=%d nc=%d step3=%d: Schur blocks of %d (svec(P) + multipliers + entries of T_k) do not fit the LDS image of the substitution kernels (limit 3168)", nx, ng, nc, step3, db.dp);
      return TMPC_E_UNSUPPORTED;
    }
  }
  int ndev = 0;
  if (hipGetDeviceCount(&ndev) != hipSuccess || ndev < 1) { snprintf(g_err, sizeof(g_err), "no HIP device"); return TMPC_E_NODEVICE; }
  if (chunk <= 0) {
    size_t fr = 0, tot = 0;
    HIPCHK(hipMemGetInfo(&fr, &tot));
    const uint64_t per = workspace_bytes(1, p, nx, mb, ng, nc, step3);
    uint64_t fit = (uint64_t)(0.6 * (double)fr) / std::max<uint64_t>(per, 1);
    chunk = (int)std::max<uint64_t>(1, std::min<uint64_t>(512, fit));
  }
  tmpc_handle* h = new (std::nothrow) tmpc_handle();
  if (!h) return TMPC_E_NOMEM;
  h->slab = nullptr; h->d_sched = nullptr; h->ev_in = nullptr; h->dd_slab = nullptr; h->dd_bytes = 0; h->tight = 0; h->tight_tol = 0x1p-37;
  if (hipGetDevice(&h->device) != hipSuccess) { delete h; return TMPC_E_HIP; }
  int nl = (make_dims(1, p, nx, mb, ng, nc, step3).dp <= 64 && chunk >= 2) ? 2 : 1;
  if (lanes >= 1) nl = std::min(lanes, MAXL);
  nl = std::max(1, std::min(nl, chunk));
  h->nlanes = nl;
  const int cap = (chunk + nl - 1) / nl;
  h->chunk = cap * nl;
  h->dm = make_dims(cap, p, nx, mb, ng, nc, step3);
  h->sched = cr_build(p);
  h->rs = 0; h->mt = 0;
  h->tune_small = 1; h->tune_pretest = 1; h->tune_fuse = 1; h->tune_graph = 1; h->tune_persist = 1; h->tune_lowp_trsm = 1;
  h->opt.tol = 0x1p-25; h->opt.center_tol = 1e-9; h->opt.max_iter = 50; h->opt.center_iter = 12;
  h->opt.fast_exit = 0;
  h->opt.lowp_switch = TMPC_LOWP_SWITCH_DEFAULT;
  h->opt.chord_step = 10.0;
  h->flags = 0;
  WS tmp;
  const size_t lane_bytes = carve(tmp, h->dm, nullptr, nullptr);
  h->slab_bytes = lane_bytes * nl;
  if (hipMalloc(&h->slab, h->slab_bytes) != hipSuccess) {
    snprintf(g_err, sizeof(g_err), "hipMalloc(%zu bytes) failed", h->slab_bytes);
    delete h;
    return TMPC_E_NOMEM;
  }
  int rc = cr_upload(h->sched, &h->d_sched);
  bool ok = (rc == TMPC_OK) && hipEventCreateWithFlags(&h->ev_in, hipEventDisableTiming) == hipSuccess;
  for (int l = 0; l < MAXL; ++l) { Lane& ln = h->lane[l]; ln.big_scr = nullptr; ln.o32_dp = 0; ln.graphs = nullptr; ln.st = nullptr; for (int i = 0; i < 8; ++i) ln.ev[i] = nullptr; memset(ln.prof, 0, sizeof(ln.prof)); ln.last_nb = 0; ln.err[0] = 0; }
  for (int l = 0; l < nl && ok; ++l) {
    Lane& ln = h->lane[l];
    carve(ln.ws, h->dm, (char*)h->slab + (size_t)l * lane_bytes, &ln);
    if (ln.ws.O32) ok = hipMemset(ln.ws.O32, 0, 2 * (size_t)h->dm.B * h->dm.p * h->dm.dp * ((h->dm.dp + 31) & ~31) * sizeof(float)) == hipSuccess;
    ok = ok && hipStreamCreateWithFlags(&ln.st, hipStreamNonBlocking) == hipSuccess;
    for (int i = 0; i < 8 && ok; ++i) ok = hipEventCreate(&ln.ev[i]) == hipSuccess;
  }
  if (ok) { rc = set_lds_attrs(h->device); ok = (rc == TMPC_OK); }
  if (!ok) { tmpc_destroy(h); return rc != TMPC_OK ? rc : TMPC_E_HIP; }
  *out = h;
  return TMPC_OK;
}

int tmpc_destroy(tmpc_handle* h) {
  if (!h) return TMPC_E_ARG;
#ifdef TMPC_EIG_DEBUG
  { int c[4]; double v[8]; hipDeviceSynchronize(); hipMemcpyFromSymbol(c, HIP_SYMBOL(g_eig_dbg), sizeof c); hipMemcpyFromSymbol(v, HIP_SYMBOL(g_eig_dbgv), sizeof v);
    fprintf(stderr, "eig pretest: passed %d (wrong %d: lambda %.6e theta %.6f pass %g phase %g)  failed %d (wrong %d: lambda %.6e theta %.6f pass %g phase %g)\n",
            c[0], c[1], v[0], v[1], v[2], v[3], c[2], c[3], v[4], v[5], v[6], v[7]); }
#endif
  for (int l = 0; l < MAXL; ++l) {
    Lane& ln = h->lane[l];
    for (int i = 0; i < 8; ++i) if (ln.ev[i]) hipEventDestroy(ln.ev[i]);
    for (hipEvent_t e : ln.kev) hipEventDestroy(e);
    if (ln.st) hipStreamDestroy(ln.st);
    if (ln.big_scr) hipFree(ln.big_scr);
    if (ln.graphs) { for (auto& kv : *ln.graphs) if (kv.second) hipGraphExecDestroy(kv.second); delete ln.graphs; }
    LaneWorker::retire(ln.worker);
  }
  if (h->ev_in) hipEventDestroy(h->ev_in);
  if (h->slab) hipFree(h->slab);
  if (h->dd_slab) hipFree(h->dd_slab);
  if (h->d_sched) hipFree(h->d_sched);
  delete h;
  return TMPC_OK;
}

int tmpc_get_chunk(tmpc_handle* h) { return h ? h->chunk : TMPC_E_ARG; }

int tmpc_set_options(tmpc_handle* h, double tol, double center_tol, int max_iter, int center_iter, int flags) {
  if (!h) return TMPC_E_ARG;
  if (flags & ~(TMPC_FLAG_NO_MFMA | TMPC_FLAG_PROFILE | TMPC_FLAG_FAST_EXIT | TMPC_DEBUG_FLAG_STOP_ASSEMBLED | TMPC_DEBUG_FLAG_NO_LIFT | TMPC_DEBUG_FLAG_NO_DMA | TMPC_DEBUG_FLAG_GENERIC_STAGE)) {
    snprintf(g_err, sizeof(g_err), "tmpc_set_options: unknown flag bits 0x%x (TMPC_FLAG_NO_MFMA = 1, TMPC_FLAG_PROFILE = 2, TMPC_FLAG_FAST_EXIT = 4)", flags);
    return TMPC_E_ARG;
  }
  if (tol > 0) h->opt.tol = tol;
  if (center_tol > 0) h->opt.center_tol = center_tol;
  if (max_iter > 0) h->opt.max_iter = max_iter;
  if (center_iter > 0) h->opt.center_iter = center_iter;
  h->flags = flags;
  return TMPC_OK;
}


int tmpc_set_tuning(tmpc_handle* h, int key, double value) {
  if (!h) return TMPC_E_ARG;
  switch (key) {
    case TMPC_TUNE_CHORD_STEP: if (!(value >= 0.0)) return TMPC_E_ARG; h->opt.chord_step = value; return TMPC_OK;
    case TMPC_TUNE_LOWP_SWITCH: if (!(value >= 0.0)) return TMPC_E_ARG; h->opt.lowp_switch = value; return TMPC_OK;
    case TMPC_TUNE_SMALL_BLOCKS: h->tune_small = value != 0.0; return TMPC_OK;
    case TMPC_TUNE_EIG_PRETEST: h->tune_pretest = value != 0.0; return TMPC_OK;
    case TMPC_TUNE_FUSE_FWD: h->tune_fuse = value != 0.0; return TMPC_OK;
    case TMPC_TUNE_GRAPH: h->tune_graph = value != 0.0; return TMPC_OK;
    case TMPC_TUNE_PERSISTENT: if (!(value >= 0.0 && value <= 2.0)) return TMPC_E_ARG; h->tune_persist = (int)value; return TMPC_OK;
    case TMPC_TUNE_LOWP_TRSM: h->tune_lowp_trsm = value != 0.0; return TMPC_OK;
    default: snprintf(g_err, sizeof(g_err), "tmpc_set_tuning: unknown key %d", key); return TMPC_E_ARG;
  }
}

int tmpc_set_tight(tmpc_handle* h, int enable, double tight_tol) {
  if (!h) return TMPC_E_ARG;
  if (!enable) { h->tight = 0; return TMPC_OK; }
  if (h->dm.nT > 0) { snprintf(g_err, sizeof(g_err), "tmpc_set_tight: Steps 1 and 2 only (no Step 3 handles)"); return TMPC_E_UNSUPPORTED; }
  if (h->dm.nr > 0 && (size_t)dd_aug_lds_doubles(h->dm.nr, h->dm.n, h->dm.nx) * sizeof(double) > 160 * 1024) {
    snprintf(g_err, sizeof(g_err), "tmpc_set_tight: %d rows per stage at nx = %d, nx + mb = %d: their double-double vectors do not fit the LDS (rows * (2 n + 2 nx) <= 4040)", h->dm.nr, h->dm.nx, h->dm.n);
    return TMPC_E_UNSUPPORTED;
  }
  if ((size_t)dd_solve_lds_doubles(h->dm.dp) * sizeof(double) > 160 * 1024) {
    snprintf(g_err, sizeof(g_err), "tmpc_set_tight: Schur blocks of %d do not fit the LDS image of the double-double substitution kernels (nx <= 51)", h->dm.dp);
    return TMPC_E_UNSUPPORTED;
  }
  if (tight_tol > 0.0 && !(tight_tol >= 0x1p-42 && tight_tol < 1.0)) { snprintf(g_err, sizeof(g_err), "tmpc_set_tight: tolerance %g outside [2^-42, 1)", tight_tol); return TMPC_E_ARG; }
  ON_DEVICE(h);
  if (!h->dd_slab) {
    WS tmp;
    const size_t lane_bytes = carve_dd(tmp, h->dm, nullptr);
    if (hipMalloc(&h->dd_slab, lane_bytes * h->nlanes) != hipSuccess) {
      h->dd_slab = nullptr;
      snprintf(g_err, sizeof(g_err), "tmpc_set_tight: hipMalloc(%zu bytes) failed", lane_bytes * h->nlanes);
      return TMPC_E_NOMEM;
    }
    h->dd_bytes = lane_bytes * h->nlanes;
    for (int l = 0; l < h->nlanes; ++l) carve_dd(h->lane[l].ws, h->dm, (char*)h->dd_slab + (size_t)l * lane_bytes);
  }
  if (tight_tol > 0.0) h->tight_tol = tight_tol;
  h->tight = 1;
  return TMPC_OK;
}

}

template <typename F> static int for_last_wave(tmpc_handle* h, int nb, F&& f) {
  int done = 0;
  for (int l = 0; l < h->nlanes && done < nb; ++l) {
    const int m = std::min(h->lane[l].last_nb, nb - done);
    if (m > 0) { int rc = f(h->lane[l], done, m); if (rc != TMPC_OK) return rc; }
    done += m;
  }
  return done == nb ? TMPC_OK : TMPC_E_ARG;
}

extern "C" {

int tmpc_get_trace(tmpc_handle* h, int nb, double* out) {
  if (!h || !out || nb < 1 || nb > h->chunk) return TMPC_E_ARG;
  ON_DEVICE(h);
  const size_t row = (size_t)TRACE_LEN * TRACE_W;
  return for_last_wave(h, nb, [&](Lane& ln, int o, int m) {
    HIPCHK(hipMemcpy(out + (size_t)o * row, ln.ws.trace, (size_t)m * row * sizeof(double), hipMemcpyDeviceToHost));
    return TMPC_OK;
  });
}

__global__ void k_dual_scalars(WS w, int nb, double* out) {
  const int b = blockIdx.x * blockDim.x + threadIdx.x;
  if (b >= nb) return;
  const double* pr = w.prob + (size_t)b * PS;
  double* o = out + (size_t)b * 4;
  o[0] = pr[P_X0]; o[1] = pr[P_TAU]; o[2] = pr[P_ALPHA]; o[3] = pr[P_MUT];
}

int tmpc_get_dual_host(tmpc_handle* h, int nb, double* X1, double* X2, double* scal) {
  if (!h || nb < 1 || nb > h->chunk) return TMPC_E_ARG;
  ON_DEVICE(h);
  const size_t row = (size_t)h->dm.p * h->dm.n * h->dm.n;
  return for_last_wave(h, nb, [&](Lane& ln, int o, int m) {
    if (X1) HIPCHK(hipMemcpy(X1 + (size_t)o * row, ln.ws.X1, (size_t)m * row * sizeof(double), hipMemcpyDeviceToHost));
    if (X2) HIPCHK(hipMemcpy(X2 + (size_t)o * row, ln.ws.X2, (size_t)m * row * sizeof(double), hipMemcpyDeviceToHost));
    if (scal) {
      hipLaunchKernelGGL(k_dual_scalars, dim3((m + 63) / 64), dim3(64), 0, 0, ln.ws, m, ln.d_info);
      HIPCHK(hipMemcpy(scal + (size_t)o * 4, ln.d_info, (size_t)m * 4 * sizeof(double), hipMemcpyDeviceToHost));
    }
    return TMPC_OK;
  });
}

int tmpc_get_dual_con_host(tmpc_handle* h, int nb, double* phi, double* z, double* aX, double* at) {
  if (!h || nb < 1 || nb > h->chunk || h->dm.nr < 1 || !h->lane[0].ws.phi) return TMPC_E_ARG;
// ... 1197 lines not shown

struct CrBench {
  WS w; Dims dm; CrSched sc; int* d_sched = nullptr; DevBuf D, O, F, Li, dd, Z, W3, ip, pr, al;
  DevBuf O32b; int ablate = 0;
  int init(int nb, int p, int d, int flags, bool lowp = false) {
    memset(&w, 0, sizeof(w)); memset(&dm, 0, sizeof(dm));
    dm.B = nb; dm.p = p; dm.d = d; dm.dp = (d + 15) / 16 * 16; dm.nt = (dm.dp + TB - 1) / TB; dm.flags = flags & TMPC_FLAG_NO_MFMA;
    const size_t bs = (size_t)dm.dp * dm.dp, per = (size_t)p * bs;
    sc = cr_build(p);
    int rc = cr_upload(sc, &d_sched);
    if (rc != TMPC_OK) return rc;
    if (D.alloc(nb * per * 8) != hipSuccess || O.alloc(nb * per * 8) != hipSuccess || F.alloc(nb * per * 8) != hipSuccess ||
        Li.alloc((size_t)nb * p * dm.nt * TB * TB * 8) != hipSuccess || dd.alloc((size_t)nb * p * dm.dp * 8) != hipSuccess ||
        Z.alloc((size_t)nb * p * dm.dp * 8) != hipSuccess || W3.alloc((size_t)nb * p * dm.dp * 3 * 8) != hipSuccess ||
        ip.alloc((size_t)nb * IS * sizeof(int)) != hipSuccess || pr.alloc((size_t)nb * PS * 8) != hipSuccess || al.alloc((size_t)nb * sizeof(int)) != hipSuccess)
      return TMPC_E_NOMEM;
    w.D = D.as<double>(); w.O = O.as<double>(); w.F = F.as<double>(); w.Linv = Li.as<double>(); w.Ddiag = dd.as<double>();
    w.Z = Z.as<double>(); w.W3 = W3.as<double>(); w.iprob = ip.as<int>(); w.prob = pr.as<double>(); w.alist = al.as<int>();
    std::vector<int> ids(nb); for (int i = 0; i < nb; ++i) ids[i] = i;
    std::vector<double> one((size_t)nb * PS, 1.0);
    if (hipMemcpy(w.alist, ids.data(), nb * sizeof(int), hipMemcpyHostToDevice) != hipSuccess) return TMPC_E_HIP;
    if (hipMemset(w.iprob, 0, (size_t)nb * IS * sizeof(int)) != hipSuccess) return TMPC_E_HIP;
    if (hipMemcpy(w.prob, one.data(), one.size() * 8, hipMemcpyHostToDevice) != hipSuccess) return TMPC_E_HIP;
    if (lowp && dm.dp > 64 && dm.nt <= TRR_NT) {
      dm.flags |= DF_LOWP;
      const size_t n32 = 2 * (size_t)nb * p * dm.dp * ((dm.dp + 31) & ~31);
      if (O32b.alloc(n32 * sizeof(float)) != hipSuccess || hipMemset(O32b.as<float>(), 0, n32 * sizeof(float)) != hipSuccess) return TMPC_E_NOMEM;
      w.O32 = O32b.as<float>();
#ifdef TMPC_ABLATE
      dm.flags |= ablate << 24;
#endif
      std::vector<int> hi((size_t)nb * IS, 0);
      for (int b = 0; b < nb; ++b) hi[(size_t)b * IS + I_LOWP] = 1;
      if (hipMemcpy(w.iprob, hi.data(), hi.size() * sizeof(int), hipMemcpyHostToDevice) != hipSuccess) return TMPC_E_HIP;
    }
    return TMPC_OK;
  }
  ~CrBench() { if (d_sched) hipFree(d_sched); }
};

static void cr_pack(const CrSched& sc, int p, int d, int dp, const double* D, const double* Ccpl, std::vector<double>& hD, std::vector<double>& hO,
                    std::vector<double>& hdd) {
  const size_t bs = (size_t)dp * dp;
  hD.assign(p * bs, 0.0); hO.assign(p * bs, 0.0); hdd.assign((size_t)p * dp, 1.0);
  for (int k = 0; k < p; ++k) {
    for (int i = 0; i < dp; ++i)
      for (int j = 0; j < dp; ++j) {
        double dv = (i == j) ? 1.0 : 0.0, cv = 0.0;
        if (i < d && j < d) { dv = D[((size_t)k * d + i) * d + j]; cv = Ccpl[((size_t)k * d + i) * d + j]; }
        hD[k * bs + (size_t)i * dp + j] = dv;
        if (sc.orient[k]) hO[k * bs + (size_t)i * dp + j] = cv; else hO[k * bs + (size_t)j * dp + i] = cv;
      }
    for (int i = 0; i < d; ++i) hdd[(size_t)k * dp + i] = D[((size_t)k * d + i) * d + i];
  }
}

int tmpc_debug_block_solve(tmpc_handle* h, int p, int d, const double* D, const double* Ccpl, const double* rhs, double* x, int32_t* nshift) {
  if (!h || p < 1 || d < 1 || !D || !Ccpl || !rhs || !x) return TMPC_E_ARG;
  ON_DEVICE(h);
  CrBench cb;
  int rc = cb.init(1, p, d, h->flags, h->opt.lowp_switch >= 1.0);
  if (rc != TMPC_OK) return rc;
  const int dp = cb.dm.dp;
  const size_t bs = (size_t)dp * dp;
  std::vector<double> hD, hO, hdd, hz((size_t)p * dp, 0.0);
  cr_pack(cb.sc, p, d, dp, D, Ccpl, hD, hO, hdd);
  for (int k = 0; k < p; ++k) for (int i = 0; i < d; ++i) hz[(size_t)k * dp + i] = rhs[(size_t)k * d + i];
  HIPCHK(hipMemcpy(cb.w.D, hD.data(), p * bs * 8, hipMemcpyHostToDevice));
  HIPCHK(hipMemcpy(cb.w.O, hO.data(), p * bs * 8, hipMemcpyHostToDevice));
  HIPCHK(hipMemcpy(cb.w.Ddiag, hdd.data(), (size_t)p * dp * 8, hipMemcpyHostToDevice));
  HIPCHK(hipMemcpy(cb.w.Z, hz.data(), (size_t)p * dp * 8, hipMemcpyHostToDevice));
  cr_factor(cb.w, cb.dm, cb.sc, cb.d_sched, cb.w.alist, 1, 0, h->rs, h->mt, nullptr, nullptr, 0, cb.w.O32 ? 1 : 0);
  cr_solve(cb.w, cb.dm, cb.sc, cb.d_sched, cb.w.alist, 1, 0, 2);
  HIPCHK(hipDeviceSynchronize());
  HIPCHK(hipGetLastError());
  int hip_[IS];
  HIPCHK(hipMemcpy(hz.data(), cb.w.Z, (size_t)p * dp * 8, hipMemcpyDeviceToHost));
  HIPCHK(hipMemcpy(hip_, cb.w.iprob, sizeof(hip_), hipMemcpyDeviceToHost));
  for (int k = 0; k < p; ++k) for (int i = 0; i < d; ++i) x[(size_t)k * d + i] = hz[(size_t)k * dp + i];
  if (nshift) *nshift = hip_[I_NSHIFT];
  return TMPC_OK;
}

int tmpc_debug_block_factor(tmpc_handle* h, int nb, int p, int d, int count, int mode, const tmpc_debug_factor_io* io) {
  if (!h || !io || nb < 1 || p < 1 || d < 1 || count < 0 || count > nb || !io->D || !io->Ccpl || !io->rhs || (count > 0 && !io->list)) return TMPC_E_ARG;
  if (mode & ~(TMPC_DEBUG_FACTOR_PASS1 | TMPC_DEBUG_FACTOR_FUSE_FWD1 | TMPC_DEBUG_FACTOR_LOWP_TRSM | TMPC_DEBUG_FACTOR_DD)) return TMPC_E_ARG;
  const bool pass1 = (mode & TMPC_DEBUG_FACTOR_PASS1) != 0, fuse = (mode & TMPC_DEBUG_FACTOR_FUSE_FWD1) != 0, ddm = (mode & TMPC_DEBUG_FACTOR_DD) != 0;
  std::vector<char> seen(nb, 0);
  int nlowp = 0, anylowp = 0;
  for (int i = 0; i < count; ++i) {
    const int b = io->list[i];
    if (b < 0 || b >= nb || seen[b]) { snprintf(g_err, sizeof(g_err), "tmpc_debug_block_factor: list entry %d is out of range or repeated", i); return TMPC_E_ARG; }
    seen[b] = 1;
    if (io->lowp && io->lowp[b]) ++nlowp;
  }
  for (int b = 0; b < nb && io->lowp; ++b) anylowp |= io->lowp[b] != 0;
  ON_DEVICE(h);
  CrBench cb;
  int rc = cb.init(nb, p, d, h->flags, false);
  if (rc != TMPC_OK) return rc;
  Dims& dm = cb.dm; WS& w = cb.w;
  if (h->flags & TMPC_DEBUG_FLAG_NO_DMA) dm.flags |= DF_NO_DMA;
  if (!h->tune_small) dm.flags |= DF_NO_SMALL;
  const int dp = dm.dp, ld32 = (dp + 31) & ~31, nc = pass1 ? 3 : 1;
  const size_t bs = (size_t)dp * dp, per = (size_t)p * bs, vl = (size_t)p * dp;
  if (solve_lds(dm) > 160 * 1024) return TMPC_E_UNSUPPORTED;
  const bool lowp_ok = !(dm.flags & (1 | DF_NO_DMA)) && dp > 64 && dm.nt <= TRR_NT;
  const bool fuse_ok = pass1 && !(dm.flags & (1 | DF_NO_DMA)) && p > 1 && dm.nt <= TRR_NT && !cr_small_levels(dm, cb.sc, nullptr);
  if ((anylowp || (mode & TMPC_DEBUG_FACTOR_LOWP_TRSM)) && (!lowp_ok || ddm)) { snprintf(g_err, sizeof(g_err), "tmpc_debug_block_factor: no float32 path at dp = %d with these flags", dp); return TMPC_E_ARG; }
  if (fuse && (!fuse_ok || ddm)) { snprintf(g_err, sizeof(g_err), "tmpc_debug_block_factor: no fused forward sweep at p = %d, dp = %d with these flags", p, dp); return TMPC_E_ARG; }
  DevBuf O32b, Dlb, Olb, Flb, Lilb, W3lb, Zlb;
  const size_t n32 = 2 * (size_t)nb * p * dp * ld32;
  if (anylowp || (mode & TMPC_DEBUG_FACTOR_LOWP_TRSM)) {
    if (O32b.alloc(n32 * sizeof(float)) != hipSuccess) return TMPC_E_NOMEM;
    HIPCHK(hipMemset(O32b.p, 0, n32 * sizeof(float)));
    w.O32 = O32b.as<float>();
    dm.flags |= DF_LOWP | ((mode & TMPC_DEBUG_FACTOR_LOWP_TRSM) ? DF_LOWP_TRSM : 0);
  }
  if (ddm) {
    if (Dlb.alloc(nb * per * 8) != hipSuccess || Olb.alloc(nb * per * 8) != hipSuccess || Flb.alloc(nb * per * 8) != hipSuccess ||
        Lilb.alloc((size_t)nb * p * dm.nt * TB * TB * 8) != hipSuccess || W3lb.alloc((size_t)nb * vl * 3 * 8) != hipSuccess || Zlb.alloc((size_t)nb * vl * 8) != hipSuccess)
      return TMPC_E_NOMEM;
    w.Dl = Dlb.as<double>(); w.Ol = Olb.as<double>(); w.Fl = Flb.as<double>(); w.Linvl = Lilb.as<double>(); w.W3l = W3lb.as<double>(); w.Zl = Zlb.as<double>();
    HIPCHK(hipMemset(w.Fl, 0, nb * per * 8)); HIPCHK(hipMemset(w.Linvl, 0, (size_t)nb * p * dm.nt * TB * TB * 8));
    HIPCHK(hipMemset(w.W3l, 0, (size_t)nb * vl * 3 * 8)); HIPCHK(hipMemset(w.Zl, 0, (size_t)nb * vl * 8));
  }
  HIPCHK(hipMemset(w.F, 0, nb * per * 8)); HIPCHK(hipMemset(w.Linv, 0, (size_t)nb * p * dm.nt * TB * TB * 8));
  HIPCHK(hipMemset(w.Z, 0, (size_t)nb * vl * 8)); HIPCHK(hipMemset(w.W3, 0, (size_t)nb * vl * 3 * 8));
  double* X = pass1 ? w.W3 : w.Z; double* Xl = pass1 ? w.W3l : w.Zl;
  {
    std::vector<double> hD, hO, hdd, hz(vl * nc), hDl, hOl, hdl;
    const size_t dd_ = (size_t)p * d * d;
    const std::vector<double> zero(ddm && (!io->Dlo || !io->Clo) ? dd_ : 0, 0.0);
    for (int b = 0; b < nb; ++b) {
      cr_pack(cb.sc, p, d, dp, io->D + b * dd_, io->Ccpl + b * dd_, hD, hO, hdd);
      std::fill(hz.begin(), hz.end(), 0.0);
      for (int k = 0; k < p; ++k) for (int i = 0; i < d; ++i) for (int q = 0; q < nc; ++q) hz[((size_t)k * dp + i) * nc + q] = io->rhs[(((size_t)b * p + k) * d + i) * nc + q];
      HIPCHK(hipMemcpy(w.D + b * per, hD.data(), per * 8, hipMemcpyHostToDevice));
      HIPCHK(hipMemcpy(w.O + b * per, hO.data(), per * 8, hipMemcpyHostToDevice));
      HIPCHK(hipMemcpy(w.Ddiag + b * vl, hdd.data(), vl * 8, hipMemcpyHostToDevice));
      HIPCHK(hipMemcpy(X + b * vl * nc, hz.data(), vl * nc * 8, hipMemcpyHostToDevice));
      if (ddm) {
        cr_pack(cb.sc, p, d, dp, io->Dlo ? io->Dlo + b * dd_ : zero.data(), io->Clo ? io->Clo + b * dd_ : zero.data(), hDl, hOl, hdl);
        for (int k = 0; k < p; ++k) for (int i = d; i < dp; ++i) hDl[k * bs + (size_t)i * dp + i] = 0.0;
        HIPCHK(hipMemcpy(w.Dl + b * per, hDl.data(), per * 8, hipMemcpyHostToDevice));
        HIPCHK(hipMemcpy(w.Ol + b * per, hOl.data(), per * 8, hipMemcpyHostToDevice));
      }
    }
  }
  if (count > 0) HIPCHK(hipMemcpy(w.alist, io->list, (size_t)count * sizeof(int), hipMemcpyHostToDevice));
  if (anylowp) {
    std::vector<int> hi((size_t)nb * IS, 0);
    for (int b = 0; b < nb; ++b) hi[(size_t)b * IS + I_LOWP] = io->lowp[b] ? 1 : 0;
    HIPCHK(hipMemcpy(w.iprob, hi.data(), hi.size() * sizeof(int), hipMemcpyHostToDevice));
  }
  if (count > 0) {
    const int pass = pass1 ? 1 : 2;
    if (ddm) {
      dd_factor(w, dm, cb.sc, cb.d_sched, w.alist, count, 0);
      rc = dd_solve(w, dm, cb.sc, cb.d_sched, w.alist, count, 0, pass, nb);
      if (rc != TMPC_OK) return rc;
    } else {
      cr_factor(w, dm, cb.sc, cb.d_sched, w.alist, count, 0, h->rs, h->mt, nullptr, nullptr, fuse ? 1 : 0, nlowp);
      cr_solve(w, dm, cb.sc, cb.d_sched, w.alist, count, 0, pass, fuse);
    }
  }
  HIPCHK(hipDeviceSynchronize());
  HIPCHK(hipGetLastError());
  if (io->oD) HIPCHK(hipMemcpy(io->oD, w.D, nb * per * 8, hipMemcpyDeviceToHost));
  if (io->oO) HIPCHK(hipMemcpy(io->oO, w.O, nb * per * 8, hipMemcpyDeviceToHost));
  if (io->oF) HIPCHK(hipMemcpy(io->oF, w.F, nb * per * 8, hipMemcpyDeviceToHost));
  if (io->oDdiag) HIPCHK(hipMemcpy(io->oDdiag, w.Ddiag, nb * vl * 8, hipMemcpyDeviceToHost));
  if (io->oX) HIPCHK(hipMemcpy(io->oX, X, nb * vl * nc * 8, hipMemcpyDeviceToHost));
  if (io->oO32 && w.O32) HIPCHK(hipMemcpy(io->oO32, w.O32, n32 * sizeof(float), hipMemcpyDeviceToHost));
  if (ddm) {
    if (io->oDl) HIPCHK(hipMemcpy(io->oDl, w.Dl, nb * per * 8, hipMemcpyDeviceToHost));
    if (io->oOl) HIPCHK(hipMemcpy(io->oOl, w.Ol, nb * per * 8, hipMemcpyDeviceToHost));
    if (io->oFl) HIPCHK(hipMemcpy(io->oFl, w.Fl, nb * per * 8, hipMemcpyDeviceToHost));
    if (io->oXl) HIPCHK(hipMemcpy(io->oXl, Xl, nb * vl * nc * 8, hipMemcpyDeviceToHost));
  }
  if (io->nshift) {
    std::vector<int> hi((size_t)nb * IS);
    HIPCHK(hipMemcpy(hi.data(), w.iprob, hi.size() * sizeof(int), hipMemcpyDeviceToHost));
    for (int b = 0; b < nb; ++b) io->nshift[b] = hi[(size_t)b * IS + I_NSHIFT];
  }
  if (io->dims) { io->dims[0] = dp; io->dims[1] = ld32; io->dims[2] = nc; io->dims[3] = w.O32 ? 1 : 0; }
  if (io->orient) for (int k = 0; k < p; ++k) io->orient[k] = cb.sc.orient[k];
  return TMPC_OK;
}

int tmpc_debug_factor_bench(tmpc_handle* h, int nb, int p, int d, int reps, double* ms_out2) {
  if (!h || nb < 1 || p < 1 || d < 1 || reps < 1 || !ms_out2) return TMPC_E_ARG;
  ON_DEVICE(h);
  CrBench cb;
  cb.ablate = (int)h->opt.lowp_switch - 2;
  int rc = cb.init(nb, p, d, h->flags, h->opt.lowp_switch >= 1.0);
  if (rc != TMPC_OK) return rc;
  const int dp = cb.dm.dp;
  const size_t bs = (size_t)dp * dp, per = (size_t)p * bs;
  std::vector<double> E((size_t)p * d * d), G((size_t)p * d * d), Dd((size_t)p * d * d, 0.0), Cc((size_t)p * d * d, 0.0);
  unsigned long long st = 88172645463325252ull;
  auto rnd = [&]() { st ^= st << 13; st ^= st >> 7; st ^= st << 17; return ((double)(st % 2000001) / 1000000.0 - 1.0) / sqrt((double)d); };
  for (auto& v : E) v = rnd();
  for (auto& v : G) v = rnd();
  for (int k = 0; k < p; ++k) {
    const int kn = (k + 1) % p;
    const double* Ek = &E[(size_t)k * d * d]; const double* Gk = &G[(size_t)k * d * d];
    for (int i = 0; i < d; ++i)
      for (int j = 0; j < d; ++j) {
        double ee = 0, gg = 0, eg = 0;
        for (int r = 0; r < d; ++r) { ee += Ek[r * d + i] * Ek[r * d + j]; gg += Gk[r * d + i] * Gk[r * d + j]; eg += Ek[r * d + i] * Gk[r * d + j]; }
        Dd[((size_t)k * d + i) * d + j] += ee + (i == j ? 1.0 : 0.0); Dd[((size_t)kn * d + i) * d + j] += gg;
        Cc[((size_t)k * d + i) * d + j] = eg;
      }
  }
  std::vector<double> hD, hO, hdd;
  cr_pack(cb.sc, p, d, dp, Dd.data(), Cc.data(), hD, hO, hdd);
  DevBuf pD, pO;
  HIPCHK(pD.alloc(per * 8)); HIPCHK(pO.alloc(per * 8));
  HIPCHK(hipMemcpy(pD.p, hD.data(), per * 8, hipMemcpyHostToDevice));
  HIPCHK(hipMemcpy(pO.p, hO.data(), per * 8, hipMemcpyHostToDevice));
  for (int b = 0; b < nb; ++b) HIPCHK(hipMemcpy(cb.w.Ddiag + (size_t)b * p * dp, hdd.data(), (size_t)p * dp * 8, hipMemcpyHostToDevice));
  HIPCHK(hipMemset(cb.w.Z, 0, (size_t)nb * p * dp * 8));
  hipEvent_t e0, e1, e2; HIPCHK(hipEventCreate(&e0)); HIPCHK(hipEventCreate(&e1)); HIPCHK(hipEventCreate(&e2));
  ms_out2[0] = ms_out2[1] = 0.0;
  for (int r = 0; r < reps + 1; ++r) {
    for (int b = 0; b < nb; ++b) {
      HIPCHK(hipMemcpyAsync(cb.w.D + b * per, pD.p, per * 8, hipMemcpyDeviceToDevice, 0));
      HIPCHK(hipMemcpyAsync(cb.w.O + b * per, pO.p, per * 8, hipMemcpyDeviceToDevice, 0));
    }
    HIPCHK(hipEventRecord(e0, 0));
    cr_factor(cb.w, cb.dm, cb.sc, cb.d_sched, cb.w.alist, nb, 0, h->rs, h->mt, nullptr, nullptr, 0, cb.w.O32 ? nb : 0);
    HIPCHK(hipEventRecord(e1, 0));
    cr_solve(cb.w, cb.dm, cb.sc, cb.d_sched, cb.w.alist, nb, 0, 2);
    HIPCHK(hipEventRecord(e2, 0));
    HIPCHK(hipEventSynchronize(e2));
    float ms0, ms1; HIPCHK(hipEventElapsedTime(&ms0, e0, e1)); HIPCHK(hipEventElapsedTime(&ms1, e1, e2));
    if (r > 0) { ms_out2[0] += ms0 / reps; ms_out2[1] += ms1 / reps; }
  }
  HIPCHK(hipGetLastError());
  int nsh = 0; HIPCHK(hipMemcpy(&nsh, cb.w.iprob + I_NSHIFT, sizeof(int), hipMemcpyDeviceToHost));
  if (nsh) { snprintf(g_err, sizeof(g_err), "factor bench: %d shifted pivots", nsh); }
  hipEventDestroy(e0); hipEventDestroy(e1); hipEventDestroy(e2);
  return TMPC_OK;
}

#ifdef TMPC_CYCLE_PROF
int tmpc_debug_cycle_prof(double* out64) {
  unsigned long long hh[64];
  HIPCHK(hipMemcpyFromSymbol(hh, HIP_SYMBOL(tmpc::g_prof), sizeof(hh)));
  for (int i = 0; i < 64; ++i) out64[i] = (double)hh[i];
  unsigned long long z[64] = {0};
  HIPCHK(hipMemcpyToSymbol(HIP_SYMBOL(tmpc::g_prof), z, sizeof(z)));
  return 0;
}
#endif

}
```

### tunempc_amd/csrc/tmpc_common.h

```cpp
#pragma once
#include <hip/hip_runtime.h>
#include <stdint.h>

namespace tmpc {

#ifdef TMPC_CYCLE_PROF
__device__ unsigned long long g_prof[64];
__device__ int g_prof_cls;
#define TMPC_T(i) { if (blockIdx.x == 0 && threadIdx.x == 0) { const unsigned long long t_ = __builtin_readcyclecounter(); g_prof[(g_prof_cls & 7) * 8 + (i)] += t_ - tprev_; tprev_ = t_; } }
#define TMPC_T0() unsigned long long tprev_ = __builtin_readcyclecounter();
#define TMPC_TC(c, i) { if (blockIdx.x == 0 && threadIdx.x == 0) { const unsigned long long t_ = __builtin_readcyclecounter(); g_prof[(c) * 8 + (i)] += t_ - tprevc_; tprevc_ = t_; } }
#define TMPC_TC0() unsigned long long tprevc_ = __builtin_readcyclecounter();
#else
#define TMPC_TC(c, i)
#define TMPC_TC0()
#define TMPC_T(i)
#define TMPC_T0()
#endif



constexpr double ALPHA_MIN = 1e-8;
constexpr int TRACE_LEN = 80, TRACE_W = 10;
constexpr int TB = 64;
#ifndef TMPC_CENTER_DAMP
#define TMPC_CENTER_DAMP 0.95
#endif
constexpr int REG_MAX = 3;
constexpr int EIG_MAX_SWEEPS = 40;

enum {
  P_TAU = 0, P_ALPHA, P_S0, P_X0, P_MU, P_MUT, P_SIGMU, P_AP, P_AD, P_S, P_SBETA, P_PINF, P_DINF, P_RELGAP,
  P_STEPN, P_PREVSTEPN, P_DTAU, P_DALPHA, P_DS0, P_DX0, P_RD0, P_CORR0, P_MINEIG_H, P_BTT, P_BTA, P_BAA,
  P_SB00, P_SB01, P_SB11, P_RHS_TAU, P_RHS_ALPHA, P_SXS, P_MINEIG_HC, P_MAXCOND, P_KAPPA, P_BETA, P_ALPHA_OUT,
  P_MAXEIG_HC, P_MU0, P_MINPIV, P_RAWSTEP, P_TAU_PREV, P_ALPHA_PREV, P_MUT1, P_TAU_DEF, P_ALPHA_DEF, PS = 48
};
enum { I_PHASE = 0, I_ITERS, I_NCENT, I_IPMSTATUS, I_EARLY, I_NSHIFT, I_STATUS, I_BOSTEP, I_CHOLBAD, I_SHIFT0, I_JAM, I_SHIFTRUN, I_REG, I_CHORD, I_NCHORD, I_BACKOFF,
       I_DD, I_NDD, I_NPOLISH, I_LOWP, I_LOWPOFF, I_NLOWP, IS = 24 };
enum { PH_MAIN = 0, PH_CENTER = 1, PH_DONE = 2, PH_POLISH = 3 };
enum { IPM_OPTIMAL = 0, IPM_INACCURATE = 1, IPM_MAXITER = 2, IPM_FAST_EXIT = 3, IPM_TIGHT_FALLBACK = 4 };
enum { ST_OPTIMAL = 0, ST_FEASIBLE = 1, ST_INFEASIBLE = 2 };

enum {
  Q_XS = 0, Q_RD2, Q_S2, Q_TRX2, Q_HBY, Q_TRPSI, Q_TRPHI2, Q_HBPHI,
  Q_TRT2, Q_HBG,
  Q_MINX, Q_MINS, Q_DXS, Q_XDS, Q_DXDS, Q_DP2, Q_P2,
  Q_MINEIG, Q_MINABS, Q_MAXABS, Q_MAXEIG, Q_CHOLBAD, Q_DH2, Q_M2,
  Q_RPHI2, Q_NCONE,
  NPART = 26
};

typedef double double2_t __attribute__((ext_vector_type(2)));
typedef double double4_t __attribute__((ext_vector_type(4)));
typedef float float4_t __attribute__((ext_vector_type(4)));
typedef float float2_t __attribute__((ext_vector_type(2)));
enum { KF_XXX = 0, KF_SIXX, KF_KX, KF_KS, KF_FX, KF_FS, KF_PER_LMI = 6 };
enum { ADJ_G = 0, ADJ_PSI, ADJ_PHI, NADJ = 3 };

struct Dims {
  int B;
  int p;
  int nx, mb;
  int n;
  int d;
  int dp;
  int nt;
  int flags;
  int ng;
  int nr;
  int nz;
  int constr;
  int nT;
};
constexpr int DF_LOWP = 8;
constexpr int DF_LOWP_TRSM = 16;
constexpr int NGM = 31;
constexpr int NCM = 31;
constexpr int NRM = NGM + NCM, NZM = NRM + 2;
constexpr int NRS = 32, NZS = NRS + 2;
constexpr int NAM = 31;
constexpr int AEL = NAM + 1, AE = AEL * AEL;

struct Opts {
  double tol;
  double center_tol;
  int max_iter;
  int center_iter;
  double chord_step;
  int tight;
  double tight_tol;
  double lowp_switch;
  int fast_exit;
};

struct WS {
  const double* A; const double* Bm; const double* H;
  double* Hb;
  double* V;
  double* P;
  double* X1; double* X2; double* S1; double* S2;
  double* S1i; double* S2i; double* L1i; double* L2i; double* LX1i; double* LX2i;
  double* Rd1; double* Rd2; double* T1; double* T2;
  double* dS1; double* dS2; double* dX1; double* dX2; double* c1; double* c2;
  double* dP;
  double* Wm;
  double* eigmin;
  double* KF;
  double* adjV;
  double* adjE;
  double* part;
  double* prob;
  int* iprob;
  double* D;
  double* O;
  double* F;
  float* O32;
  double* Linv;
  double* Ddiag;
  double* W3;
  double* U;
  double* TU;
  double* Z;
  int* active;
  int* flist;
  int* alist;
  const int* cr_orient;
  double* trace;
  double* Hc;
  double* dHc;
  double* Pout;
  const double* G;
  const int* ncnt;
  double rho;
  double* phi; double* zph; double* dphi; double* dzph; double* corrp;
  double* pvec;
  double* psm;
  double* prs;
  double* Fg;
  double* at; double* adt;
  double* aX; double* adX; double* acor;
  double* aSi; double* aLi; double* aLXi;
  double* asum;
  double* t3th; double* t3z; double* t3dth; double* t3dz; double* t3cth;
  double* t3x; double* t3dx; double* t3cq; double* t3g; double* t3v; double* t3lam;
  double* t3t; double* t3dt; double* t3beta;
  double* t3psi; double* t3phi;
  double* Tout;
  double* Dl; double* Ol; double* Fl; double* Linvl; double* KFl; double* adjVl; double* adjEl; double* W3l; double* Zl;
  double* ddscr;
  double* Pprev;
  double* Pdef;
  double* phidef;
  double* atdef;
  double* TUl;
  double* Zdd;
  double* sscr;
  double* bscr;
  int* plist;
// ... 12 lines not shown
```

### tunempc_amd/csrc/tmpc_cr.h

```cpp
#pragma once
#include <climits>
#include <vector>

#include "tmpc_common.h"
#include "tmpc_factor.h"
#include "tmpc_gemm_dma.h"

namespace tmpc {

constexpr int CR_EW = 8;
constexpr int CR_UW = 8;
enum { CE_NODE = 0, CE_NA, CE_NB, CE_EA, CE_EB, CE_FILL, CE_FX, CE_FACC };
enum { CU_NODE = 0, CU_E0, CU_S0, CU_E1, CU_S1 };

struct CrLevel { int eoff, nelim, uoff, nupd; };
struct CrSched {
  int p = 0;
  int prep = 0;
  std::vector<int> orient;
  std::vector<int> elim, upd;
  std::vector<CrLevel> lev;
};

static inline CrSched cr_build(int p) {
// ... 413 lines not shown
      for (int cs = 0; cs < ((nci + 1) >> 1); ++cs) {
        TRD_STEP_BEGIN()
        const double* A0 = At + 2 * cs * ASL;
        if (rw) {
          TRD_MMA_R(acc0, A0, Bc, 2 * cs, nci)
          if (2 * cs + 1 < nci) TRD_MMA_R(acc0, A0 + ASL, Bc + 1024, 2 * cs + 1, nci)
        }
        TMPC_TC(2, 3)
      }
      TRD_STORE_R(ci, nci, acc0, +)
    }
    if (ci == 0 && nt > 1) TRD_LOAD_R(nlast, ncl, acc0)
    if (ci + 1 >= nt) break;
    if (ci < 1 && 1 < nlast) TRD_PAIR_C(acc1)
    if (ci < 2 && 2 < nlast) TRD_PAIR_C(acc2)
    if (ci < 3 && 3 < nlast) TRD_PAIR_C(acc3)
    if (ncl == 3) TRD_PAIR_RL(3) else if (ncl == 4) TRD_PAIR_RL(4) else if (ncl == 2) TRD_PAIR_RL(2) else TRD_PAIR_RL(1)
    const int t = ci + 1;
    __builtin_amdgcn_s_barrier();
    if (POTRF && t == nlast) break;
    if (t == nlast) { TRD_PARK_R(ncl, acc0, -) TRD_ZERO(acc0) }
    else if (t == 1) { TRD_PARK_C(acc1) TRD_ZERO(acc1) }
    else if (t == 2) { TRD_PARK_C(acc2) TRD_ZERO(acc2) }
    else { TRD_PARK_C(acc3) TRD_ZERO(acc3) }
    TMPC_TC(2, 4)
  }
  if (POTRF) {
    if (rw) {
      double* Simg = lds;
      const int row = wc0 + 4 * fq + fk;
#pragma unroll
      for (int c = 0; c < 4; ++c) {
        if (c < ncl) {
#pragma unroll
          for (int e = 0; e < 4; ++e) Simg[row * LDP + 16 * c + 4 * fj + e] = -acc0[c][e];
        }
      }
    }
  }
#undef TRD_DIAG
#undef TRD_PAIR_RL
#undef TRD_PAIR_C
#undef TRD_STEP_BEGIN
#undef TRD_STEP_RL
#undef TRD_STEP_D1
#undef TRD_STEP_D0
#undef TRD_STEP_C
#undef TRD_MMA_R
#undef TRD_MMA_C
#undef TRD_ISSUE
#undef TRD_ZERO
#undef TRD_PARK_R
#undef TRD_PARK_C
#undef TRD_STORE_R
#undef TRD_LOAD_R
#undef TRD_LOAD_C
#undef TRD_NB
}

__global__ void __launch_bounds__(256, 2) k_cr_trsm_dma(WS w, Dims dm, CrDev cr, int eoff, int nelim, int count) {
  const int dp = dm.dp;
  const int nst = (dp + 63) / 64;
  const int per = 2 * nst;
  const int it = cr_item(count * nelim * per);
  if (it < 0) return;
  extern __shared__ __attribute__((aligned(16))) double lds[];
  const int g = it / per, r = it - g * per;
  const int b = cr.alist[g / nelim];
  const int* er = cr.elim + (size_t)(eoff + g % nelim) * CR_EW;
  const int which = r / nst, strip = r - which * nst;
  const int slot = which ? er[CE_EB] : er[CE_EA];
  if (slot < 0) return;
  const int node = er[CE_NODE];
  const double* Dk = w.D + ((size_t)b * dm.p + node) * (size_t)dp * dp;
  const double* Li = w.Linv + ((size_t)b * dm.p + node) * dm.nt * TB * TB;
  const int r0 = strip * 64;
  const bool lp = cr_lowp(w, b);
  if (lp && (dm.flags & DF_LOWP_TRSM)) return;
  const int ld32 = cr_ld32(dm);
  trd_strip<false>(cr_edge(w, dm, b, slot) + (size_t)r0 * dp, Dk, Li, (dp - r0 < 64) ? dp - r0 : 64, dm.nt, dp, it, lds,
                   lp ? cr_edge32(w, dm, b, slot) + (size_t)r0 * ld32 : nullptr, ld32);
}

constexpr int trf_lds_doubles() { return 2048 + TRD_DEPTH * 2048; }
__device__ __forceinline__ void trf_strip(const double* X, const double* Dk, const double* Li, int rows, int nt, int dp, int it, double* lds, float* X32, int ld32) {
  constexpr int ASL = 64 * 16, DP = TRD_DEPTH;
  const int tid = threadIdx.x;
  const int lane = tid & 63, wv = __builtin_amdgcn_readfirstlane(tid >> 6);
  const int ws = (wv + it) & 3, wc0 = ws * 16;
  const int fk = lane >> 4, fr = lane & 15;
  const int i1 = (rows + 15) >> 4;
  const int nlast = nt - 1, nbl = (dp - 64 * nlast < 64) ? dp - 64 * nlast : 64, ncl = nbl >> 4;
  const int ntd = nt;
  const bool rw = ws < i1;
  float* At = (float*)lds;
  double* Bs = lds + 2048;
  unsigned voT[2], voL[2];
#pragma unroll
  for (int h = 0; h < 2; ++h) {
    const int row = wv * 16 + 8 * h + (lane >> 3), c = lane & 7;
    voT[h] = (unsigned)(row * TB + 2 * (c ^ dma_sw(row))) * 8u;
    voL[h] = (unsigned)(row * dp + 2 * (c ^ dma_sw(row))) * 8u;
  }
  int of[2];
#pragma unroll
  for (int hh = 0; hh < 2; ++hh) of[hh] = fr * 16 + 2 * ((4 * hh + fk) ^ dma_sw(fr));
  const int asw = (fr >> 1) & 3, ofa = fr * 16 + 4 * (fk ^ asw);
  const int opa0 = 4 * ((2 * fk) & 3 ^ asw) + 2 * (fk >> 1), opa1 = 4 * ((2 * fk + 1) & 3 ^ asw) + 2 * (fk >> 1);
  float4_t acc0[4], acc1[4], acc2[4], acc3[4];
  int vmtot = 0, vmk0 = 0, vmk1 = 0, vmk2 = 0;
#define TRF_NB(T) ((dp - 64 * (T) < 64) ? dp - 64 * (T) : 64)
#define TRF_LOAD_C(I, SET)                                                                                  \
  {                                                                                                         \
    const bool on_ = wc0 < TRF_NB(I);                                                                       \
    _Pragma("unroll") for (int i = 0; i < 4; ++i) {                                                          \
      double2_t u0 = (double2_t){0.0, 0.0}, u1 = u0;                                                        \
      if (on_ && i < i1) {                                                                                  \
        gcptr2 cp = (gcptr2)(X + (size_t)(16 * i + fr) * dp + 64 * (I) + wc0 + 4 * fk);                     \
        u0 = cp[0]; u1 = cp[1];                                                                             \
      }                                                                                                     \
      SET[i] = (float4_t){(float)-u0[0], (float)-u0[1], (float)-u1[0], (float)-u1[1]};                      \
    }                                                                                                       \
    if (on_) vmtot += 2 * i1;                                                                               \
  }
#define TRF_LOAD_R(I, NC, SET)                                                                              \
  {                                                                                                         \
    _Pragma("unroll") for (int c = 0; c < 4; ++c) {                                                          \
      double2_t u0 = (double2_t){0.0, 0.0}, u1 = u0;                                                        \
      if (rw && c < (NC)) {                                                                                 \
        gcptr2 cp = (gcptr2)(X + (size_t)(wc0 + fr) * dp + 64 * (I) + 16 * c + 4 * fk);                     \
        u0 = cp[0]; u1 = cp[1];                                                                             \
      }                                                                                                     \
      SET[c] = (float4_t){(float)-u0[0], (float)-u0[1], (float)-u1[0], (float)-u1[1]};                      \
    }                                                                                                       \
    if (rw) vmtot += 2 * (NC);                                                                              \
  }
#define TRF_STORE_R(I, NC, SET)                                                                             \
  if (rw) {                                                                                                 \
    typedef float4_t __attribute__((address_space(1)))* gptr4;                                              \
    _Pragma("unroll") for (int c = 0; c < 4; ++c)                                                            \
      if (c < (NC)) *(gptr4)(X32 + (size_t)(wc0 + fr) * ld32 + 64 * (I) + 16 * c + 4 * fk) = SET[c];        \
    vmtot += (NC);                                                                                          \
  }
#define TRF_PARK_C(SET)                                                                        \
  {                                                                                                         \
    _Pragma("unroll") for (int i = 0; i < 4; ++i) {                                                          \
      float* q = At + ws * ASL + (16 * i + fr) * 16;                                                        \
      *(float2_t*)(q + opa0) = (float2_t){-SET[i][0], -SET[i][1]};                                           \
      *(float2_t*)(q + opa1) = (float2_t){-SET[i][2], -SET[i][3]};                                           \
    }                                                                                                       \
  }
#define TRF_PARK_R(NC, SET, SG)                                                                             \
  if (rw) {                                                                                                 \
    _Pragma("unroll") for (int c = 0; c < 4; ++c) {                                                          \
      if (c < (NC)) {                                                                                       \
        float* q = At + c * ASL + (wc0 + fr) * 16;                                                          \
        *(float2_t*)(q + opa0) = (float2_t){SG SET[c][0], SG SET[c][1]};                                     \
        *(float2_t*)(q + opa1) = (float2_t){SG SET[c][2], SG SET[c][3]};                                     \
      }                                                                                                     \
    }                                                                                                       \
  }
#define TRF_ZERO(SET) { _Pragma("unroll") for (int i = 0; i < 4; ++i) SET[i] = (float4_t){0.f, 0.f, 0.f, 0.f}; }
  int ii = 0, ij = 0, is = 0, nissued = 0, ndone = 0;
#define TRF_ISSUE()                                                       \
  {                                                                                                         \
    if (ii < ntd) {                                                                                         \
      double* dst_ = Bs + (nissued % DP) * 2048 + wv * 256;                                                 \
      const int nsl_ = (ij == ii) ? (TRF_NB(ii) >> 4) : 4;                                                  \
      const bool two_ = 2 * is + 1 < nsl_;                                                                  \
      if (ij == ii) {                                                                                       \
        const int nb_ = TRF_NB(ii);                                                                         \
        const __amdgpu_buffer_rsrc_t rs_ = __builtin_amdgcn_make_buffer_rsrc((void*)(Li + (size_t)ii * TB * TB), 0, (int)(((unsigned)(nb_ - 1) * TB + (unsigned)nb_) * 8u), 0x00020000); \
        __builtin_amdgcn_raw_ptr_buffer_load_lds(rs_, (lds_vptr)(dst_), 16, voT[0], is * 256, 0, 0);        \
        __builtin_amdgcn_raw_ptr_buffer_load_lds(rs_, (lds_vptr)(dst_ + 128), 16, voT[1], is * 256, 0, 0);  \
        if (two_) {                                                                                         \
          __builtin_amdgcn_raw_ptr_buffer_load_lds(rs_, (lds_vptr)(dst_ + 1024), 16, voT[0], is * 256 + 128, 0, 0);       \
          __builtin_amdgcn_raw_ptr_buffer_load_lds(rs_, (lds_vptr)(dst_ + 1024 + 128), 16, voT[1], is * 256 + 128, 0, 0); \
        }                                                                                                   \
      } else {                                                                                              \
        const int nb_ = TRF_NB(ij);                                                                         \
        const __amdgpu_buffer_rsrc_t rs_ = __builtin_amdgcn_make_buffer_rsrc((void*)(Dk + (size_t)(64 * ij) * dp + 64 * ii), 0, (int)(((unsigned)(nb_ - 1) * (unsigned)dp + 64u) * 8u), 0x00020000); \
        __builtin_amdgcn_raw_ptr_buffer_load_lds(rs_, (lds_vptr)(dst_), 16, voL[0], is * 256, 0, 0);        \
        __builtin_amdgcn_raw_ptr_buffer_load_lds(rs_, (lds_vptr)(dst_ + 128), 16, voL[1], is * 256, 0, 0);  \
        __builtin_amdgcn_raw_ptr_buffer_load_lds(rs_, (lds_vptr)(dst_ + 1024), 16, voL[0], is * 256 + 128, 0, 0);         \
        __builtin_amdgcn_raw_ptr_buffer_load_lds(rs_, (lds_vptr)(dst_ + 1024 + 128), 16, voL[1], is * 256 + 128, 0, 0);   \
      }                                                                                                     \
      vmtot += (ij == ii && !two_) ? 2 : 4;                                                                 \
      { const int k_ = nissued % DP; if (k_ == 0) vmk0 = vmtot; else if (k_ == 1) vmk1 = vmtot; else vmk2 = vmtot; }  \
      ++nissued;                                                                                            \
      if (++is == ((nsl_ + 1) >> 1)) { is = 0; if (++ij >= ntd) { ++ii; ij = ii; } }                        \
    }                                                                                                       \
  }
#define TRF_MMA_C(TGT, AS, BS)                                                                              \
  {                                                                                                         \
    float4_t a_[4];                                                                                          \
    _Pragma("unroll") for (int i = 0; i < 4; ++i) a_[i] = *(const float4_t*)((AS) + i * 256 + ofa);         \
    _Pragma("unroll") for (int hh = 0; hh < 2; ++hh) {                                                      \
      const double2_t b_ = *(const double2_t*)((BS) + wc0 * 16 + of[hh]);                                   \
      _Pragma("unroll") for (int e = 0; e < 2; ++e) {                                                        \
        const float bf_ = (float)b_[e];                                                                      \
        _Pragma("unroll") for (int i = 0; i < 4; ++i)                                                        \
          TGT[i] = __builtin_amdgcn_mfma_f32_16x16x4f32(bf_, a_[i][2 * hh + e], TGT[i], 0, 0, 0);           \
      }                                                                                                     \
    }                                                                                                       \
  }
#define TRF_MMA_R(TGT, AS, BS, C0, NC)                                                                      \
  {                                                                                                         \
    const float4_t a_ = *(const float4_t*)((AS) + wc0 * 16 + ofa);                                          \
    _Pragma("unroll") for (int hh = 0; hh < 2; ++hh) {                                                      \
      double2_t b_[4];                                                                                       \
      _Pragma("unroll") for (int c = 0; c < 4; ++c)                                                          \
        if (c >= (C0) && c < (NC)) b_[c] = *(const double2_t*)((BS) + c * 256 + of[hh]);                    \
      _Pragma("unroll") for (int e = 0; e < 2; ++e) {                                                        \
        _Pragma("unroll") for (int c = 0; c < 4; ++c)                                                        \
          if (c >= (C0) && c < (NC)) TGT[c] = __builtin_amdgcn_mfma_f32_16x16x4f32((float)b_[c][e], a_[2 * hh + e], TGT[c], 0, 0, 0); \
      }                                                                                                     \
    }                                                                                                       \
  }
#define TRF_STEP_C(TGT) { TRF_MMA_C(TGT, A0, Bc) TRF_MMA_C(TGT, A0 + ASL, Bc + 1024) }
#define TRF_STEP_D0(TGT) { TRF_MMA_R(TGT, At, Bc, 0, 4) TRF_MMA_R(TGT, At + ASL, Bc + 1024, 1, 4) }
#define TRF_STEP_D1(TGT) { TRF_MMA_R(TGT, At + 2 * ASL, Bc, 2, 4) TRF_MMA_R(TGT, At + 3 * ASL, Bc + 1024, 3, 4) }
#define TRF_STEP_RL(N) { TRF_MMA_R(acc0, A0, Bc, 0, N) TRF_MMA_R(acc0, A0 + ASL, Bc + 1024, 0, N) }

  __syncthreads();
  TRF_ISSUE()
  if (DP > 2) TRF_ISSUE()
  TRF_LOAD_C(0, acc0)
  if (nt > 2) TRF_LOAD_C(1, acc1) else TRF_ZERO(acc1)
  if (nt > 3) TRF_LOAD_C(2, acc2) else TRF_ZERO(acc2)
  if (nt > 4) TRF_LOAD_C(3, acc3) else TRF_ZERO(acc3)
  TRF_PARK_C(acc0)
  TRF_ZERO(acc0)
#define TRF_STEP_BEGIN()                                                                                    \
    { const int k_ = ndone % DP; vm_wait_le(vmtot - (k_ == 0 ? vmk0 : k_ == 1 ? vmk1 : vmk2)); }            \
    __builtin_amdgcn_s_barrier();                                                                           \
    TRF_ISSUE()                                                                                             \
    const double* Bc = Bs + (ndone % DP) * 2048;                                                            \
    ++ndone;
#define TRF_PAIR_C(TGT)                                                                                     \
  _Pragma("unroll 1") for (int cs = 0; cs < 2; ++cs) {                                                      \
    TRF_STEP_BEGIN()                                                                                        \
    const float* A0 = At + 2 * cs * ASL;                                                                    \
    TRF_STEP_C(TGT)                                                                                         \
  }
#define TRF_PAIR_RL(N)                                                                                      \
  _Pragma("unroll 1") for (int cs = 0; cs < 2; ++cs) {                                                      \
    TRF_STEP_BEGIN()                                                                                        \
    const float* A0 = At + 2 * cs * ASL;                                                                    \
    if (rw) TRF_STEP_RL(N)                                                                                  \
  }
#define TRF_DIAG(TGT)                                                                                       \
  {                                                                                                         \
    { TRF_STEP_BEGIN() if (rw) TRF_STEP_D0(TGT) }                                                           \
    { TRF_STEP_BEGIN() if (rw) TRF_STEP_D1(TGT) }                                                           \
    TRF_STORE_R(ci, 4, TGT)                                                                                 \
    if (ci + 1 < nt) {                                                                                      \
      __builtin_amdgcn_s_barrier();                                        \
      TRF_PARK_R(4, TGT, +)                                                                                 \
    }                                                                                                       \
  }
  for (int ci = 0; ci < ntd; ++ci) {
    const int nci = TRF_NB(ci) >> 4;
    if (nci == 4) {
      if (ci == 0 || ci == nlast) TRF_DIAG(acc0) else if (ci == 1) TRF_DIAG(acc1) else if (ci == 2) TRF_DIAG(acc2) else TRF_DIAG(acc3)
    } else {
      for (int cs = 0; cs < ((nci + 1) >> 1); ++cs) {
        TRF_STEP_BEGIN()
        const float* A0 = At + 2 * cs * ASL;
        if (rw) {
          TRF_MMA_R(acc0, A0, Bc, 2 * cs, nci)
          if (2 * cs + 1 < nci) TRF_MMA_R(acc0, A0 + ASL, Bc + 1024, 2 * cs + 1, nci)
        }
      }
      TRF_STORE_R(ci, nci, acc0)
    }
    if (ci == 0 && nt > 1) TRF_LOAD_R(nlast, ncl, acc0)
    if (ci + 1 >= nt) break;
    if (ci < 1 && 1 < nlast) TRF_PAIR_C(acc1)
    if (ci < 2 && 2 < nlast) TRF_PAIR_C(acc2)
    if (ci < 3 && 3 < nlast) TRF_PAIR_C(acc3)
    if (ncl == 3) TRF_PAIR_RL(3) else if (ncl == 4) TRF_PAIR_RL(4) else if (ncl == 2) TRF_PAIR_RL(2) else TRF_PAIR_RL(1)
    const int t = ci + 1;
    __builtin_amdgcn_s_barrier();
    if (t == nlast) { TRF_PARK_R(ncl, acc0, -) TRF_ZERO(acc0) }
    else if (t == 1) { TRF_PARK_C(acc1) TRF_ZERO(acc1) }
    else if (t == 2) { TRF_PARK_C(acc2) TRF_ZERO(acc2) }
    else { TRF_PARK_C(acc3) TRF_ZERO(acc3) }
  }
#undef TRF_DIAG
#undef TRF_PAIR_RL
#undef TRF_PAIR_C
#undef TRF_STEP_BEGIN
#undef TRF_STEP_RL
#undef TRF_STEP_D1
#undef TRF_STEP_D0
#undef TRF_STEP_C
#undef TRF_MMA_R
#undef TRF_MMA_C
#undef TRF_ISSUE
#undef TRF_ZERO
#undef TRF_PARK_R
#undef TRF_PARK_C
#undef TRF_STORE_R
#undef TRF_LOAD_R
#undef TRF_LOAD_C
#undef TRF_NB
}

__global__ void __launch_bounds__(256, 2) k_cr_trsm_dma_f32(WS w, Dims dm, CrDev cr, int eoff, int nelim, int count) {
  const int dp = dm.dp;
  const int nst = (dp + 63) / 64;
  const int per = 2 * nst;
  const int it = cr_item(count * nelim * per);
  if (it < 0) return;
  extern __shared__ __attribute__((aligned(16))) double lds[];
  const int g = it / per, r = it - g * per;
  const int b = cr.alist[g / nelim];
  if (!cr_lowp(w, b)) return;
  const int* er = cr.elim + (size_t)(eoff + g % nelim) * CR_EW;
  const int which = r / nst, strip = r - which * nst;
  const int slot = which ? er[CE_EB] : er[CE_EA];
  if (slot < 0) return;
  const int node = er[CE_NODE];
  const double* Dk = w.D + ((size_t)b * dm.p + node) * (size_t)dp * dp;
  const double* Li = w.Linv + ((size_t)b * dm.p + node) * dm.nt * TB * TB;
  const int r0 = strip * 64;
  const int ld32 = cr_ld32(dm);
  trf_strip(cr_edge(w, dm, b, slot) + (size_t)r0 * dp, Dk, Li, (dp - r0 < 64) ? dp - r0 : 64, dm.nt, dp, it, lds, cr_edge32(w, dm, b, slot) + (size_t)r0 * ld32, ld32);
}

constexpr int potrf_dma_lds_doubles() { return FACT_LDS_DOUBLES > trd_lds_doubles() ? FACT_LDS_DOUBLES : trd_lds_doubles(); }
__global__ void __launch_bounds__(256, 2) k_cr_potrf_dma(WS w, Dims dm, CrDev cr, int eoff, int nelim, int count) {
  const int it = cr_item(count * nelim);
  if (it < 0) return;
  extern __shared__ __attribute__((aligned(16))) double lds[];
  const int b = cr.alist[it / nelim];
  const int* er = cr.elim + (size_t)(eoff + it % nelim) * CR_EW;
  const int node = er[CE_NODE], dp = dm.dp;
  double* Dk = w.D + ((size_t)b * dm.p + node) * (size_t)dp * dp;
  double* Li = w.Linv + ((size_t)b * dm.p + node) * dm.nt * TB * TB;
  const double* dref = w.Ddiag + ((size_t)b * dm.p + node) * dp;
  double* stat = lds + FACT_LDS_DOUBLES - 8;
  if (threadIdx.x == 0) { stat[0] = 0.0; stat[1] = 1.0; }
  for (int r = 0; r < dm.nt; ++r) {
    const int r0 = 64 * r, nb = (dp - r0 < 64) ? dp - r0 : 64;
    if (r > 0) {
      trd_strip<true>(Dk + (size_t)r0 * dp, Dk, Li, nb, r + 1, dp, it, lds);
      __syncthreads();
    }
    wg_potrf_inv(Dk + (size_t)r0 * dp + r0, dp, Li + (size_t)r * TB * TB, dref + r0, nb, lds, nullptr, stat, (it >> 5) & 3, r > 0);
  }
  if (threadIdx.x == 0) {
    const int nbad = (int)stat[0];
    const double minr = stat[1];
    if (nbad) atomicAdd(w.iprob + (size_t)b * IS + I_NSHIFT, nbad);
    if (w.prob && minr < 1.0) atomic_min_pos(w.prob + (size_t)b * PS + P_MINPIV, minr);
  }
}

template <bool USE_MFMA, int NS>
__global__ void __launch_bounds__(256, 2) k_cr_update(WS w, Dims dm, CrDev cr, int eoff, int nelim, int uoff, int nupd, int count, int mt) {
  const int nm = (dm.dp + mt - 1) / mt;
  const int ntl = nm * (nm + 1) / 2, ntf = nm * nm;
  const int per = nupd * ntl + nelim * ntf;
  const int it = cr_item(count * per);
  if (it < 0) return;
  extern __shared__ __attribute__((aligned(16))) double lds[];
  const int b = cr.alist[it / per];
  int r = it % per;
  const int dp = dm.dp;
  const size_t bs = (size_t)dp * dp;
  const int slot_items = ntf + ntl;
  int j = r / slot_items, rr = r - j * slot_items;
  bool is_upd;
  {
    const int nmin = nelim < nupd ? nelim : nupd;
    const int full = nmin * slot_items;
    if (r < full) { is_upd = rr >= ntf; if (is_upd) rr -= ntf; }
    else if (nelim > nupd) { const int q = r - full; j = nmin + q / ntf; rr = q % ntf; is_upd = false; }
    else { const int q = r - full; j = nmin + q / ntl; rr = q % ntl; is_upd = true; }
  }
  if (is_upd) {
    const int* ur = cr.upd + (size_t)(uoff + (j + 1) % nupd) * CR_UW;
    int t = rr, tm = 0;
    while (t > tm) { t -= tm + 1; ++tm; }
    const int tn = t;
    const int m0 = tm * mt, n0 = tn * mt;
    const int M = (dp - m0 < mt) ? dp - m0 : mt, N = (dp - n0 < mt) ? dp - n0 : mt;
    double* C = w.D + ((size_t)b * dm.p + ur[CU_NODE]) * bs + (size_t)m0 * dp + n0;
    const double* O0 = cr_edge(w, dm, b, ur[CU_E0]);
    wg_gemm_nt<USE_MFMA, 2, 2, 2, NS>(C, dp, O0 + (size_t)m0 * dp, dp, O0 + (size_t)n0 * dp, dp, M, N, dp, GM_SUB, tm == tn, lds);
    if (ur[CU_E1] >= 0) {
      const double* O1 = cr_edge(w, dm, b, ur[CU_E1]);
      wg_gemm_nt<USE_MFMA, 2, 2, 2, NS>(C, dp, O1 + (size_t)m0 * dp, dp, O1 + (size_t)n0 * dp, dp, M, N, dp, GM_SUB, tm == tn, lds);
    }
  } else {
    const int* er = cr.elim + (size_t)(eoff + j) * CR_EW;
    if (er[CE_FILL] < 0) return;
    const int t = rr;
    const int tm = t / nm, tn = t - tm * nm;
    const int m0 = tm * mt, n0 = tn * mt;
    const int M = (dp - m0 < mt) ? dp - m0 : mt, N = (dp - n0 < mt) ? dp - n0 : mt;
    const double* Ox = cr_edge(w, dm, b, er[CE_FX] ? er[CE_EB] : er[CE_EA]);
    const double* Oy = cr_edge(w, dm, b, er[CE_FX] ? er[CE_EA] : er[CE_EB]);
    double* C = cr_edge(w, dm, b, er[CE_FILL]) + (size_t)m0 * dp + n0;
    wg_gemm_nt<USE_MFMA, 2, 2, 2, NS>(C, dp, Ox + (size_t)m0 * dp, dp, Oy + (size_t)n0 * dp, dp, M, N, dp, er[CE_FACC] ? GM_SUB : GM_NEG, false, lds);
  }
}

__device__ __forceinline__ int cr_nc(const WS& w, int b, int pass) {
  const int phase = w.iprob[(size_t)b * IS + I_PHASE];
// ... 187 lines not shown
```

Before: 12360.

## Pair both coupling edges per workgroup in low-precision CR triangular solve

Adds a TRSM_PAIR mode, on by default, in which one workgroup of the f32 MFMA triangular-solve kernel handles both edges (EA and EB) of an elimination node. The two edges share the staged diagonal-factor (B) tiles in LDS, so the factor is loaded once instead of twice and the grid is halved. The initial global loads are also restructured into a fetch/convert software pipeline. In exchange the kernel doubles accumulator registers and LDS use per workgroup, which can lower occupancy under the 256x2 launch bounds, and leaves fewer workgroups to fill the GPU at small batch sizes. A debug counter for paired strips is exposed as well.

Result: faster. 12580, median of 6 (+1.8%).

```diff
diff --git a/include/tunempc_hip.h b/include/tunempc_hip.h
--- a/include/tunempc_hip.h
+++ b/include/tunempc_hip.h
@@ -52,6 +52,7 @@
 #define TMPC_TUNE_LOWP_SWITCH 8
 #define TMPC_LOWP_SWITCH_DEFAULT 1e-5
 #define TMPC_TUNE_LOWP_TRSM 9
+#define TMPC_TUNE_TRSM_PAIR 10
 int tmpc_set_tuning(tmpc_handle* h, int key, double value);
 int tmpc_create_ex(tmpc_handle** out, int chunk, int p, int nx, int mb, int ng, int nc, int step3, int lanes);
 
diff --git a/include/tunempc_hip_debug.h b/include/tunempc_hip_debug.h
--- a/include/tunempc_hip_debug.h
+++ b/include/tunempc_hip_debug.h
@@ -29,6 +29,7 @@
   int32_t *nshift, *dims, *orient;
 } tmpc_debug_factor_io;
 int tmpc_debug_block_factor(tmpc_handle* h, int nb, int p, int d, int count, int mode, const tmpc_debug_factor_io* io);
+long long tmpc_debug_last_trsm_pairs(void);
 
 int tmpc_debug_cr_schedule(int p, int32_t* out, int cap);
 
diff --git a/tunempc_amd/_lib.py b/tunempc_amd/_lib.py
--- a/tunempc_amd/_lib.py
+++ b/tunempc_amd/_lib.py
@@ -29,6 +29,7 @@
 DEBUG_EXPORTS = [
     'tmpc_debug_gemm_nt', 'tmpc_debug_block_solve', 'tmpc_debug_cr_schedule', 'tmpc_debug_get_multipliers', 'tmpc_debug_get_array',
     'tmpc_debug_min_eig', 'tmpc_debug_min_eig_lane', 'tmpc_debug_factor_bench', 'tmpc_debug_block_factor',
+    'tmpc_debug_last_trsm_pairs',
 ]
 FLAG_DEBUG_NO_DMA = 32
 FACTOR_PASS1, FACTOR_FUSE_FWD1, FACTOR_LOWP_TRSM, FACTOR_DD = 1, 2, 4, 8
@@ -178,6 +179,8 @@
     lib.tmpc_debug_block_factor.argtypes = [vp, C.c_int, C.c_int, C.c_int, C.c_int, C.c_int, C.POINTER(_FactorIO)]
     lib.tmpc_debug_factor_bench.restype = C.c_int
     lib.tmpc_debug_factor_bench.argtypes = [vp, C.c_int, C.c_int, C.c_int, C.c_int, dp]
+    lib.tmpc_debug_last_trsm_pairs.restype = C.c_longlong
+    lib.tmpc_debug_last_trsm_pairs.argtypes = []
     lib.tmpc_debug_min_eig.restype = C.c_int
     lib.tmpc_debug_min_eig.argtypes = [vp, C.c_int, C.c_int, dp, dp]
     lib.tmpc_debug_min_eig_lane.restype = C.c_int
@@ -242,8 +245,8 @@
         _check(self.lib, self.lib.tmpc_set_options(self._h, float(tol or 0.0), float(center_tol or 0.0),
                                                    int(max_iter or 0), int(center_iter or 0), self.flags), 'tmpc_set_options')
 
-    def set_tuning(self, chord_step=None, small_blocks=None, eig_pretest=None, fuse_fwd=None, graph=None, persistent=None, lowp_switch=None, lowp_trsm=None):
-        for key, v in ((1, chord_step), (2, small_blocks), (3, eig_pretest), (4, fuse_fwd), (5, graph), (7, persistent), (8, lowp_switch), (9, lowp_trsm)):
+    def set_tuning(self, chord_step=None, small_blocks=None, eig_pretest=None, fuse_fwd=None, graph=None, persistent=None, lowp_switch=None, lowp_trsm=None, trsm_pair=None):
+        for key, v in ((1, chord_step), (2, small_blocks), (3, eig_pretest), (4, fuse_fwd), (5, graph), (7, persistent), (8, lowp_switch), (9, lowp_trsm), (10, trsm_pair)):
             if v is not None:
                 _check(self.lib, self.lib.tmpc_set_tuning(self._h, key, float(v)), 'tmpc_set_tuning')
 
@@ -551,6 +554,9 @@
         out = np.zeros(2)
         _check(self.lib, self.lib.tmpc_debug_factor_bench(self._h, nb, p, d, reps, _dptr(out)), 'tmpc_debug_factor_bench')
         return out
+
+    def debug_last_trsm_pairs(self):
+        return int(self.lib.tmpc_debug_last_trsm_pairs())
 
     def debug_block_solve(self, D, Ccpl, rhs):
         D = np.ascontiguousarray(D, dtype=np.float64); Ccpl = np.ascontiguousarray(Ccpl, dtype=np.float64)
diff --git a/tunempc_amd/csrc/tmpc_api.hip b/tunempc_amd/csrc/tmpc_api.hip
--- a/tunempc_amd/csrc/tmpc_api.hip
+++ b/tunempc_amd/csrc/tmpc_api.hip
@@ -133,7 +133,7 @@
   CrSched sched;
   int* d_sched;
   int rs, mt;
-  int tune_small, tune_pretest, tune_fuse, tune_graph, tune_persist, tune_lowp_trsm;
+  int tune_small, tune_pretest, tune_fuse, tune_graph, tune_persist, tune_lowp_trsm, tune_trsm_pair;
   void* dd_slab;
   size_t dd_bytes;
   int tight;
@@ -508,7 +508,7 @@
 }
 
 static void cr_factor(const WS& w, const Dims& dm, const CrSched& sc, const int* d_sched, const int* alist, int count, hipStream_t st,
-                      int rs_opt, int mt_opt, std::vector<hipEvent_t>* kev = nullptr, int* nkev = nullptr, int fuse_fwd1 = 0, int nlowp = 0) {
+                      int rs_opt, int mt_opt, std::vector<hipEvent_t>* kev = nullptr, int* nkev = nullptr, int fuse_fwd1 = 0, int nlowp = 0, long long* npairs = nullptr) {
   const CrDev cd = cr_dev(sc, d_sched, alist);
   int ke = 0;
   auto mark = [&](int cls) {
@@ -555,8 +555,13 @@
       const bool trsm32 = (dm.flags & DF_LOWP_TRSM) != 0;
       if (!trsm32 || nlowp < count)
         hipLaunchKernelGGL(k_cr_trsm_dma, dim3(cr_grid((long)count * lv.nelim * 2 * nt64)), dim3(256), trsm_lds, st, w, dm, cd, lv.eoff, lv.nelim, count);
-      if (trsm32 && nlowp > 0)
-        hipLaunchKernelGGL(k_cr_trsm_dma_f32, dim3(cr_grid((long)count * lv.nelim * 2 * nt64)), dim3(256), (size_t)trf_lds_doubles() * sizeof(double), st, w, dm, cd, lv.eoff, lv.nelim, count);
+      if (trsm32 && nlowp > 0) {
+        const bool pair = (dm.flags & DF_TRSM_PAIR) != 0;
+        hipLaunchKernelGGL(k_cr_trsm_dma_f32, dim3(cr_grid((long)count * lv.nelim * (pair ? 1 : 2) * nt64)), dim3(256), (size_t)trf_lds_doubles() * sizeof(double), st, w, dm, cd, lv.eoff, lv.nelim, count);
+        if (pair && npairs)
+          for (int e = lv.eoff; e < lv.eoff + lv.nelim; ++e)
+            if (sc.elim[(size_t)e * CR_EW + CE_EA] >= 0 && sc.elim[(size_t)e * CR_EW + CE_EB] >= 0) *npairs += (long long)nlowp * nt64;
+      }
     }
     else if (mf) hipLaunchKernelGGL((k_cr_trsm<true, 2>), dim3(cr_grid(it_trsm)), dim3(256), factor_lds(), st, w, dm, cd, lv.eoff, lv.nelim, count, rs);
     else hipLaunchKernelGGL((k_cr_trsm<false, 2>), dim3(cr_grid(it_trsm)), dim3(256), factor_lds(), st, w, dm, cd, lv.eoff, lv.nelim, count, rs);
@@ -684,7 +689,7 @@
   if ((h->flags & (TMPC_FLAG_NO_MFMA | TMPC_DEBUG_FLAG_NO_DMA)) || !w.O32 || t3 || dm.dp <= 64 || dm.nt > TRR_NT) o.lowp_switch = 0.0;
   if (o.lowp_switch > 0.0) o.lowp_switch = fmax(o.lowp_switch, 16.0 * o.tol);
   if (o.lowp_switch > 0.0) {
-    dm.flags |= DF_LOWP | (h->tune_lowp_trsm ? DF_LOWP_TRSM : 0);
+    dm.flags |= DF_LOWP | (h->tune_lowp_trsm ? DF_LOWP_TRSM : 0) | (h->tune_trsm_pair ? DF_TRSM_PAIR : 0);
     if (ln->o32_dp != 0 && ln->o32_dp != dm.dp) HIPCHK(hipMemsetAsync(w.O32, 0, 2 * (size_t)h->dm.B * h->dm.p * h->dm.dp * ((h->dm.dp + 31) & ~31) * sizeof(float), st));
     ln->o32_dp = dm.dp;
   }
@@ -1040,7 +1045,7 @@
   h->dm = make_dims(cap, p, nx, mb, ng, nc, step3);
   h->sched = cr_build(p);
   h->rs = 0; h->mt = 0;
-  h->tune_small = 1; h->tune_pretest = 1; h->tune_fuse = 1; h->tune_graph = 1; h->tune_persist = 1; h->tune_lowp_trsm = 1;
+  h->tune_small = 1; h->tune_pretest = 1; h->tune_fuse = 1; h->tune_graph = 1; h->tune_persist = 1; h->tune_lowp_trsm = 1; h->tune_trsm_pair = 1;
   h->opt.tol = 0x1p-25; h->opt.center_tol = 1e-9; h->opt.max_iter = 50; h->opt.center_iter = 12;
   h->opt.fast_exit = 0;
   h->opt.lowp_switch = TMPC_LOWP_SWITCH_DEFAULT;
@@ -1122,6 +1127,7 @@
     case TMPC_TUNE_GRAPH: h->tune_graph = value != 0.0; return TMPC_OK;
     case TMPC_TUNE_PERSISTENT: if (!(value >= 0.0 && value <= 2.0)) return TMPC_E_ARG; h->tune_persist = (int)value; return TMPC_OK;
     case TMPC_TUNE_LOWP_TRSM: h->tune_lowp_trsm = value != 0.0; return TMPC_OK;
+    case TMPC_TUNE_TRSM_PAIR: h->tune_trsm_pair = value != 0.0; return TMPC_OK;
     default: snprintf(g_err, sizeof(g_err), "tmpc_set_tuning: unknown key %d", key); return TMPC_E_ARG;
   }
 }
@@ -2485,6 +2491,8 @@
   return TMPC_OK;
 }
 
+static long long g_last_trsm_pairs = 0;
+long long tmpc_debug_last_trsm_pairs(void) { return g_last_trsm_pairs; }
 int tmpc_debug_block_factor(tmpc_handle* h, int nb, int p, int d, int count, int mode, const tmpc_debug_factor_io* io) {
   if (!h || !io || nb < 1 || p < 1 || d < 1 || count < 0 || count > nb || !io->D || !io->Ccpl || !io->rhs || (count > 0 && !io->list)) return TMPC_E_ARG;
   if (mode & ~(TMPC_DEBUG_FACTOR_PASS1 | TMPC_DEBUG_FACTOR_FUSE_FWD1 | TMPC_DEBUG_FACTOR_LOWP_TRSM | TMPC_DEBUG_FACTOR_DD)) return TMPC_E_ARG;
@@ -2518,7 +2526,7 @@
     if (O32b.alloc(n32 * sizeof(float)) != hipSuccess) return TMPC_E_NOMEM;
     HIPCHK(hipMemset(O32b.p, 0, n32 * sizeof(float)));
     w.O32 = O32b.as<float>();
-    dm.flags |= DF_LOWP | ((mode & TMPC_DEBUG_FACTOR_LOWP_TRSM) ? DF_LOWP_TRSM : 0);
+    dm.flags |= DF_LOWP | ((mode & TMPC_DEBUG_FACTOR_LOWP_TRSM) ? DF_LOWP_TRSM : 0) | (h->tune_trsm_pair ? DF_TRSM_PAIR : 0);
   }
   if (ddm) {
     if (Dlb.alloc(nb * per * 8) != hipSuccess || Olb.alloc(nb * per * 8) != hipSuccess || Flb.alloc(nb * per * 8) != hipSuccess ||
@@ -2557,6 +2565,7 @@
     for (int b = 0; b < nb; ++b) hi[(size_t)b * IS + I_LOWP] = io->lowp[b] ? 1 : 0;
     HIPCHK(hipMemcpy(w.iprob, hi.data(), hi.size() * sizeof(int), hipMemcpyHostToDevice));
   }
+  g_last_trsm_pairs = 0;
   if (count > 0) {
     const int pass = pass1 ? 1 : 2;
     if (ddm) {
@@ -2564,7 +2573,7 @@
       rc = dd_solve(w, dm, cb.sc, cb.d_sched, w.alist, count, 0, pass, nb);
       if (rc != TMPC_OK) return rc;
     } else {
-      cr_factor(w, dm, cb.sc, cb.d_sched, w.alist, count, 0, h->rs, h->mt, nullptr, nullptr, fuse ? 1 : 0, nlowp);
+      cr_factor(w, dm, cb.sc, cb.d_sched, w.alist, count, 0, h->rs, h->mt, nullptr, nullptr, fuse ? 1 : 0, nlowp, &g_last_trsm_pairs);
       cr_solve(w, dm, cb.sc, cb.d_sched, w.alist, count, 0, pass, fuse);
     }
   }
@@ -2599,6 +2608,8 @@
   cb.ablate = (int)h->opt.lowp_switch - 2;
   int rc = cb.init(nb, p, d, h->flags, h->opt.lowp_switch >= 1.0);
   if (rc != TMPC_OK) return rc;
+  if (cb.dm.flags & DF_LOWP) cb.dm.flags |= (h->tune_lowp_trsm ? DF_LOWP_TRSM : 0) | (h->tune_trsm_pair ? DF_TRSM_PAIR : 0);
+  g_last_trsm_pairs = 0;
   const int dp = cb.dm.dp;
   const size_t bs = (size_t)dp * dp, per = (size_t)p * bs;
   std::vector<double> E((size_t)p * d * d), G((size_t)p * d * d), Dd((size_t)p * d * d, 0.0), Cc((size_t)p * d * d, 0.0);
@@ -2633,7 +2644,7 @@
       HIPCHK(hipMemcpyAsync(cb.w.O + b * per, pO.p, per * 8, hipMemcpyDeviceToDevice, 0));
     }
     HIPCHK(hipEventRecord(e0, 0));
-    cr_factor(cb.w, cb.dm, cb.sc, cb.d_sched, cb.w.alist, nb, 0, h->rs, h->mt, nullptr, nullptr, 0, cb.w.O32 ? nb : 0);
+    cr_factor(cb.w, cb.dm, cb.sc, cb.d_sched, cb.w.alist, nb, 0, h->rs, h->mt, nullptr, nullptr, 0, cb.w.O32 ? nb : 0, r == reps ? &g_last_trsm_pairs : nullptr);
     HIPCHK(hipEventRecord(e1, 0));
     cr_solve(cb.w, cb.dm, cb.sc, cb.d_sched, cb.w.alist, nb, 0, 2);
     HIPCHK(hipEventRecord(e2, 0));
diff --git a/tunempc_amd/csrc/tmpc_common.h b/tunempc_amd/csrc/tmpc_common.h
--- a/tunempc_amd/csrc/tmpc_common.h
+++ b/tunempc_amd/csrc/tmpc_common.h
@@ -74,6 +74,7 @@
 };
 constexpr int DF_LOWP = 8;
 constexpr int DF_LOWP_TRSM = 16;
+constexpr int DF_TRSM_PAIR = 32;
 constexpr int NGM = 31;
 constexpr int NCM = 31;
 constexpr int NRM = NGM + NCM, NZM = NRM + 2;
diff --git a/tunempc_amd/csrc/tmpc_cr.h b/tunempc_amd/csrc/tmpc_cr.h
--- a/tunempc_amd/csrc/tmpc_cr.h
+++ b/tunempc_amd/csrc/tmpc_cr.h
@@ -519,9 +519,10 @@
                    lp ? cr_edge32(w, dm, b, slot) + (size_t)r0 * ld32 : nullptr, ld32);
 }
 
-constexpr int trf_lds_doubles() { return 2048 + TRD_DEPTH * 2048; }
-__device__ __forceinline__ void trf_strip(const double* X, const double* Dk, const double* Li, int rows, int nt, int dp, int it, double* lds, float* X32, int ld32) {
-  constexpr int ASL = 64 * 16, DP = TRD_DEPTH;
+constexpr int trf_lds_doubles() { return 2 * 2048 + TRD_DEPTH * 2048; }
+template <int NE>
+__device__ __forceinline__ void trf_strip(const double* X0, const double* X1, const double* Dk, const double* Li, int rows, int nt, int dp, int it, double* lds, float* Y0, float* Y1, int ld32) {
+  constexpr int ASL = 64 * 16, AE = 4 * ASL, DP = TRD_DEPTH;
   const int tid = threadIdx.x;
   const int lane = tid & 63, wv = __builtin_amdgcn_readfirstlane(tid >> 6);
   const int ws = (wv + it) & 3, wc0 = ws * 16;
@@ -531,77 +532,95 @@
   const int ntd = nt;
   const bool rw = ws < i1;
   float* At = (float*)lds;
-  double* Bs = lds + 2048;
-  unsigned voT[2], voL[2];
-#pragma unroll
-  for (int h = 0; h < 2; ++h) {
-    const int row = wv * 16 + 8 * h + (lane >> 3), c = lane & 7;
-    voT[h] = (unsigned)(row * TB + 2 * (c ^ dma_sw(row))) * 8u;
-    voL[h] = (unsigned)(row * dp + 2 * (c ^ dma_sw(row))) * 8u;
-  }
+  double* Bs = lds + NE * 2048;
+#define TRF_LANE(V) int V = lane; if (NE > 1) asm volatile("" : "+v"(V));
   int of[2];
 #pragma unroll
   for (int hh = 0; hh < 2; ++hh) of[hh] = fr * 16 + 2 * ((4 * hh + fk) ^ dma_sw(fr));
   const int asw = (fr >> 1) & 3, ofa = fr * 16 + 4 * (fk ^ asw);
-  const int opa0 = 4 * ((2 * fk) & 3 ^ asw) + 2 * (fk >> 1), opa1 = 4 * ((2 * fk + 1) & 3 ^ asw) + 2 * (fk >> 1);
-  float4_t acc0[4], acc1[4], acc2[4], acc3[4];
+#define TRF_OPA()                                                                                           \
+    TRF_LANE(l_)                                                                                            \
+    const int fk_ = l_ >> 4, fr_ = l_ & 15, asw_ = (fr_ >> 1) & 3;                                          \
+    const int opa0 = 4 * ((2 * fk_) & 3 ^ asw_) + 2 * (fk_ >> 1), opa1 = 4 * ((2 * fk_ + 1) & 3 ^ asw_) + 2 * (fk_ >> 1);
+  float4_t acc0[NE][4], acc1[NE][4], acc2[NE][4], acc3[NE][4];
+#define TRF_EDGES _Pragma("unroll") for (int ed = 0; ed < NE; ++ed)
   int vmtot = 0, vmk0 = 0, vmk1 = 0, vmk2 = 0;
 #define TRF_NB(T) ((dp - 64 * (T) < 64) ? dp - 64 * (T) : 64)
-#define TRF_LOAD_C(I, SET)                                                                                  \
+#define TRF_FETCH_C(I, ED, BUF)                                                                             \
   {                                                                                                         \
     const bool on_ = wc0 < TRF_NB(I);                                                                       \
+    const double* X = (ED) ? X1 : X0;                                                                       \
     _Pragma("unroll") for (int i = 0; i < 4; ++i) {                                                          \
-      double2_t u0 = (double2_t){0.0, 0.0}, u1 = u0;                                                        \
+      BUF[2 * i] = (double2_t){0.0, 0.0}; BUF[2 * i + 1] = BUF[2 * i];                                      \
       if (on_ && i < i1) {                                                                                  \
         gcptr2 cp = (gcptr2)(X + (size_t)(16 * i + fr) * dp + 64 * (I) + wc0 + 4 * fk);                     \
-        u0 = cp[0]; u1 = cp[1];                                                                             \
-      }                                                                                                     \
-      SET[i] = (float4_t){(float)-u0[0], (float)-u0[1], (float)-u1[0], (float)-u1[1]};                      \
+        BUF[2 * i] = cp[0]; BUF[2 * i + 1] = cp[1];                                                         \
+      }                                                                                                     \
     }                                                                                                       \
     if (on_) vmtot += 2 * i1;                                                                               \
   }
+#define TRF_CVT_C(SET, ED, BUF)                                                                             \
+  _Pragma("unroll") for (int i = 0; i < 4; ++i)                                                              \
+    SET[ED][i] = (float4_t){(float)-BUF[2 * i][0], (float)-BUF[2 * i][1], (float)-BUF[2 * i + 1][0], (float)-BUF[2 * i + 1][1]};
 #define TRF_LOAD_R(I, NC, SET)                                                                              \
   {                                                                                                         \
-    _Pragma("unroll") for (int c = 0; c < 4; ++c) {                                                          \
-      double2_t u0 = (double2_t){0.0, 0.0}, u1 = u0;                                                        \
-      if (rw && c < (NC)) {                                                                                 \
-        gcptr2 cp = (gcptr2)(X + (size_t)(wc0 + fr) * dp + 64 * (I) + 16 * c + 4 * fk);                     \
-        u0 = cp[0]; u1 = cp[1];                                                                             \
-      }                                                                                                     \
-      SET[c] = (float4_t){(float)-u0[0], (float)-u0[1], (float)-u1[0], (float)-u1[1]};                      \
-    }                                                                                                       \
-    if (rw) vmtot += 2 * (NC);                                                                              \
+    TRF_EDGES {                                                                                             \
+      const double* X = ed ? X1 : X0;                                                                       \
+      _Pragma("unroll") for (int c = 0; c < 4; ++c) {                                                        \
+        double2_t u0 = (double2_t){0.0, 0.0}, u1 = u0;                                                      \
+        if (rw && c < (NC)) {                                                                               \
+          gcptr2 cp = (gcptr2)(X + (size_t)(wc0 + fr) * dp + 64 * (I) + 16 * c + 4 * fk);                   \
+          u0 = cp[0]; u1 = cp[1];                                                                           \
+        }                                                                                                   \
+        SET[ed][c] = (float4_t){(float)-u0[0], (float)-u0[1], (float)-u1[0], (float)-u1[1]};                \
+      }                                                                                                     \
+      if (rw) vmtot += 2 * (NC);                                                                            \
+    }                                                                                                       \
   }
 #define TRF_STORE_R(I, NC, SET)                                                                             \
   if (rw) {                                                                                                 \
     typedef float4_t __attribute__((address_space(1)))* gptr4;                                              \
-    _Pragma("unroll") for (int c = 0; c < 4; ++c)                                                            \
-      if (c < (NC)) *(gptr4)(X32 + (size_t)(wc0 + fr) * ld32 + 64 * (I) + 16 * c + 4 * fk) = SET[c];        \
-    vmtot += (NC);                                                                                          \
+    TRF_LANE(l_)                                                                                            \
+    const int fk_ = l_ >> 4, fr_ = l_ & 15;                                                                 \
+    TRF_EDGES {                                                                                             \
+      float* X32 = ed ? Y1 : Y0;                                                                            \
+      _Pragma("unroll") for (int c = 0; c < 4; ++c)                                                          \
+        if (c < (NC)) *(gptr4)(X32 + (size_t)(wc0 + fr_) * ld32 + 64 * (I) + 16 * c + 4 * fk_) = SET[ed][c]; \
+      vmtot += (NC);                                                                                        \
+    }                                                                                                       \
   }
 #define TRF_PARK_C(SET)                                                                        \
   {                                                                                                         \
-    _Pragma("unroll") for (int i = 0; i < 4; ++i) {                                                          \
-      float* q = At + ws * ASL + (16 * i + fr) * 16;                                                        \
-      *(float2_t*)(q + opa0) = (float2_t){-SET[i][0], -SET[i][1]};                                           \
-      *(float2_t*)(q + opa1) = (float2_t){-SET[i][2], -SET[i][3]};                                           \
+    TRF_OPA()                                                                                               \
+    TRF_EDGES _Pragma("unroll") for (int i = 0; i < 4; ++i) {                                                \
+      float* q = At + ed * AE + ws * ASL + (16 * i + fr_) * 16;                                             \
+      *(float2_t*)(q + opa0) = (float2_t){-SET[ed][i][0], -SET[ed][i][1]};                                   \
+      *(float2_t*)(q + opa1) = (float2_t){-SET[ed][i][2], -SET[ed][i][3]};                                   \
     }                                                                                                       \
   }
 #define TRF_PARK_R(NC, SET, SG)                                                                             \
   if (rw) {                                                                                                 \
-    _Pragma("unroll") for (int c = 0; c < 4; ++c) {                                                          \
+    TRF_OPA()                                                                                               \
+    TRF_EDGES _Pragma("unroll") for (int c = 0; c < 4; ++c) {                                                \
       if (c < (NC)) {                                                                                       \
-        float* q = At + c * ASL + (wc0 + fr) * 16;                                                          \
-        *(float2_t*)(q + opa0) = (float2_t){SG SET[c][0], SG SET[c][1]};                                     \
-        *(float2_t*)(q + opa1) = (float2_t){SG SET[c][2], SG SET[c][3]};                                     \
-      }                                                                                                     \
-    }                                                                                                       \
-  }
-#define TRF_ZERO(SET) { _Pragma("unroll") for (int i = 0; i < 4; ++i) SET[i] = (float4_t){0.f, 0.f, 0.f, 0.f}; }
+        float* q = At + ed * AE + c * ASL + (wc0 + fr_) * 16;                                               \
+        *(float2_t*)(q + opa0) = (float2_t){SG SET[ed][c][0], SG SET[ed][c][1]};                             \
+        *(float2_t*)(q + opa1) = (float2_t){SG SET[ed][c][2], SG SET[ed][c][3]};                             \
+      }                                                                                                     \
+    }                                                                                                       \
+  }
+#define TRF_ZERO(SET) { TRF_EDGES _Pragma("unroll") for (int i = 0; i < 4; ++i) SET[ed][i] = (float4_t){0.f, 0.f, 0.f, 0.f}; }
   int ii = 0, ij = 0, is = 0, nissued = 0, ndone = 0;
 #define TRF_ISSUE()                                                       \
   {                                                                                                         \
     if (ii < ntd) {                                                                                         \
+      TRF_LANE(l_)                                                                                          \
+      unsigned voT[2], voL[2];                               \
+      _Pragma("unroll") for (int h = 0; h < 2; ++h) {                                                        \
+        const int row = wv * 16 + 8 * h + (l_ >> 3), c = l_ & 7;                                            \
+        voT[h] = (unsigned)(row * TB + 2 * (c ^ dma_sw(row))) * 8u;                                         \
+        voL[h] = (unsigned)(row * dp + 2 * (c ^ dma_sw(row))) * 8u;                                         \
+      }                                                                                                     \
       double* dst_ = Bs + (nissued % DP) * 2048 + wv * 256;                                                 \
       const int nsl_ = (ij == ii) ? (TRF_NB(ii) >> 4) : 4;                                                  \
       const bool two_ = 2 * is + 1 < nsl_;                                                                  \
@@ -630,27 +649,31 @@
   }
 #define TRF_MMA_C(TGT, AS, BS)                                                                              \
   {                                                                                                         \
-    float4_t a_[4];                                                                                          \
-    _Pragma("unroll") for (int i = 0; i < 4; ++i) a_[i] = *(const float4_t*)((AS) + i * 256 + ofa);         \
+    float4_t a_[NE][4];                                                                                      \
+    TRF_EDGES _Pragma("unroll") for (int i = 0; i < 4; ++i) a_[ed][i] = *(const float4_t*)((AS) + ed * AE + i * 256 + ofa); \
     _Pragma("unroll") for (int hh = 0; hh < 2; ++hh) {                                                      \
       const double2_t b_ = *(const double2_t*)((BS) + wc0 * 16 + of[hh]);                                   \
       _Pragma("unroll") for (int e = 0; e < 2; ++e) {                                                        \
         const float bf_ = (float)b_[e];                                                                      \
         _Pragma("unroll") for (int i = 0; i < 4; ++i)                                                        \
-          TGT[i] = __builtin_amdgcn_mfma_f32_16x16x4f32(bf_, a_[i][2 * hh + e], TGT[i], 0, 0, 0);           \
+          TRF_EDGES TGT[ed][i] = __builtin_amdgcn_mfma_f32_16x16x4f32(bf_, a_[ed][i][2 * hh + e], TGT[ed][i], 0, 0, 0); \
       }                                                                                                     \
     }                                                                                                       \
   }
 #define TRF_MMA_R(TGT, AS, BS, C0, NC)                                                                      \
   {                                                                                                         \
-    const float4_t a_ = *(const float4_t*)((AS) + wc0 * 16 + ofa);                                          \
+    float4_t a_[NE];                                                                                         \
+    TRF_EDGES a_[ed] = *(const float4_t*)((AS) + ed * AE + wc0 * 16 + ofa);                                 \
     _Pragma("unroll") for (int hh = 0; hh < 2; ++hh) {                                                      \
       double2_t b_[4];                                                                                       \
       _Pragma("unroll") for (int c = 0; c < 4; ++c)                                                          \
         if (c >= (C0) && c < (NC)) b_[c] = *(const double2_t*)((BS) + c * 256 + of[hh]);                    \
       _Pragma("unroll") for (int e = 0; e < 2; ++e) {                                                        \
         _Pragma("unroll") for (int c = 0; c < 4; ++c)                                                        \
-          if (c >= (C0) && c < (NC)) TGT[c] = __builtin_amdgcn_mfma_f32_16x16x4f32((float)b_[c][e], a_[2 * hh + e], TGT[c], 0, 0, 0); \
+          if (c >= (C0) && c < (NC)) {                                                                      \
+            const float bf_ = (float)b_[c][e];                                                               \
+            TRF_EDGES TGT[ed][c] = __builtin_amdgcn_mfma_f32_16x16x4f32(bf_, a_[ed][2 * hh + e], TGT[ed][c], 0, 0, 0); \
+          }                                                                                                 \
       }                                                                                                     \
     }                                                                                                       \
   }
@@ -662,10 +685,36 @@
   __syncthreads();
   TRF_ISSUE()
   if (DP > 2) TRF_ISSUE()
-  TRF_LOAD_C(0, acc0)
-  if (nt > 2) TRF_LOAD_C(1, acc1) else TRF_ZERO(acc1)
-  if (nt > 3) TRF_LOAD_C(2, acc2) else TRF_ZERO(acc2)
-  if (nt > 4) TRF_LOAD_C(3, acc3) else TRF_ZERO(acc3)
+  {
+    constexpr int NG = 4 * NE;
+    double2_t eb_[4][8];
+#define TRF_HAS(T) ((T) == 0 || nt > (T) + 1)
+#define TRF_FETCH_G(G) { if (TRF_HAS((G) / NE)) TRF_FETCH_C((G) / NE, (G) % NE, eb_[(G) & 3]) }
+#define TRF_CVT_G(G)                                                                                        \
+  {                                                                                                         \
+    const int t_ = (G) / NE, e_ = (G) % NE;                                                                 \
+    if (TRF_HAS(t_)) {                                                                                      \
+      if (t_ == 0) { TRF_CVT_C(acc0, e_, eb_[(G) & 3]) } else if (t_ == 1) { TRF_CVT_C(acc1, e_, eb_[(G) & 3]) }                  \
+      else if (t_ == 2) { TRF_CVT_C(acc2, e_, eb_[(G) & 3]) } else { TRF_CVT_C(acc3, e_, eb_[(G) & 3]) }                          \
+    } else {                                                                                                \
+      _Pragma("unroll") for (int i = 0; i < 4; ++i) {                                                        \
+        const float4_t z_ = (float4_t){0.f, 0.f, 0.f, 0.f};                                                  \
+        if (t_ == 1) acc1[e_][i] = z_; else if (t_ == 2) acc2[e_][i] = z_; else acc3[e_][i] = z_;            \
+      }                                                                                                     \
+    }                                                                                                       \
+  }
+#pragma unroll
+    for (int g = 0; g < 4; ++g) TRF_FETCH_G(g)
+#pragma unroll
+    for (int g = 0; g < NG; ++g) {
+      __builtin_amdgcn_sched_barrier(0);
+      TRF_CVT_G(g)
+      if (g + 4 < NG) TRF_FETCH_G(g + 4)
+    }
+#undef TRF_CVT_G
+#undef TRF_FETCH_G
+#undef TRF_HAS
+  }
   TRF_PARK_C(acc0)
   TRF_ZERO(acc0)
 #define TRF_STEP_BEGIN()                                                                                    \
@@ -740,14 +789,19 @@
 #undef TRF_PARK_C
 #undef TRF_STORE_R
 #undef TRF_LOAD_R
-#undef TRF_LOAD_C
+#undef TRF_CVT_C
+#undef TRF_FETCH_C
 #undef TRF_NB
+#undef TRF_EDGES
+#undef TRF_OPA
+#undef TRF_LANE
 }
 
 __global__ void __launch_bounds__(256, 2) k_cr_trsm_dma_f32(WS w, Dims dm, CrDev cr, int eoff, int nelim, int count) {
   const int dp = dm.dp;
   const int nst = (dp + 63) / 64;
-  const int per = 2 * nst;
+  const bool pair = (dm.flags & DF_TRSM_PAIR) != 0;
+  const int per = pair ? nst : 2 * nst;
   const int it = cr_item(count * nelim * per);
   if (it < 0) return;
   extern __shared__ __attribute__((aligned(16))) double lds[];
@@ -755,15 +809,19 @@
   const int b = cr.alist[g / nelim];
   if (!cr_lowp(w, b)) return;
   const int* er = cr.elim + (size_t)(eoff + g % nelim) * CR_EW;
-  const int which = r / nst, strip = r - which * nst;
-  const int slot = which ? er[CE_EB] : er[CE_EA];
-  if (slot < 0) return;
+  const int which = pair ? 0 : r / nst, strip = r - which * nst;
+  int s0 = which ? er[CE_EB] : er[CE_EA], s1 = pair ? er[CE_EB] : -1;
+  if (s0 < 0) { s0 = s1; s1 = -1; }
+  if (s0 < 0) return;
   const int node = er[CE_NODE];
   const double* Dk = w.D + ((size_t)b * dm.p + node) * (size_t)dp * dp;
   const double* Li = w.Linv + ((size_t)b * dm.p + node) * dm.nt * TB * TB;
-  const int r0 = strip * 64;
+  const int r0 = strip * 64, rows = (dp - r0 < 64) ? dp - r0 : 64;
   const int ld32 = cr_ld32(dm);
-  trf_strip(cr_edge(w, dm, b, slot) + (size_t)r0 * dp, Dk, Li, (dp - r0 < 64) ? dp - r0 : 64, dm.nt, dp, it, lds, cr_edge32(w, dm, b, slot) + (size_t)r0 * ld32, ld32);
+  const double* X0 = cr_edge(w, dm, b, s0) + (size_t)r0 * dp;
+  float* Y0 = cr_edge32(w, dm, b, s0) + (size_t)r0 * ld32;
+  if (s1 < 0) trf_strip<1>(X0, nullptr, Dk, Li, rows, dm.nt, dp, it, lds, Y0, nullptr, ld32);
+  else trf_strip<2>(X0, cr_edge(w, dm, b, s1) + (size_t)r0 * dp, Dk, Li, rows, dm.nt, dp, it, lds, Y0, cr_edge32(w, dm, b, s1) + (size_t)r0 * ld32, ld32);
 }
 
 constexpr int potrf_dma_lds_doubles() { return FACT_LDS_DOUBLES > trd_lds_doubles() ? FACT_LDS_DOUBLES : trd_lds_doubles(); }
```
